# nico-bohlinger/RL-X

Measured on AMD Instinct MI355X. Metric: env-steps/sec (whole node) PPO 4096 envs at 1/2/4/8 MI355X, higher is better.
Workload: dtype f32

## Files before the change

rl-x_amd/csrc/common.h:

```cpp
#pragma once
#include <hip/hip_runtime.h>
#include <hip/hip_ext.h>
#include <stdint.h>
#include <cstring>
#include <cmath>
#include <string>
#include <vector>
#include <functional>
#include "../../include/rlx_hip.h"

namespace rlx {

void set_error(const std::string& msg);

#define RLX_HIP_TRY(expr)                                                                      \
  do {                                                                                         \
    hipError_t e_ = (expr);                                                                    \
    if (e_ != hipSuccess) {                                                                    \
      ::rlx::set_error(std::string(#expr) + " failed: " + hipGetErrorString(e_) + " (" __FILE__ \
                       ":" + std::to_string(__LINE__) + ")");                                  \
      return RLX_EHIP;                                                                         \
    }                                                                                          \
  } while (0)

#define RLX_REQUIRE(cond, code, msg)                 \
  do {                                               \
    if (!(cond)) {                                   \
      ::rlx::set_error(std::string(msg));            \
      return (code);                                 \
    }                                                \
  } while (0)

#define RLX_LAUNCH_CHECK()                           \
  RLX_HIP_TRY(hipGetLastError())

constexpr int WAVE = 64;

struct Scratch {
  void* ptr = nullptr;
  size_t bytes = 0;
};

enum ScratchSlot {
  SL_SORT_KEYS_A = 0, SL_SORT_KEYS_B, SL_SORT_VALS_B, SL_SORT_TMP, SL_PERM,
  SL_MB_X, SL_MB_XC, SL_MB_AUX, SL_STATS,
  SL_ACT_P0, SL_ACT_P1, SL_ACT_P2, SL_ACT_C0, SL_ACT_C1, SL_ACT_C2,
  SL_DACT_0, SL_DACT_1, SL_LN_P, SL_LN_C,
  SL_PARTIAL, SL_HEAD_PART, SL_NORM, SL_NORM2, SL_FWD_A, SL_FWD_B, SL_KEYS, SL_GRAD_P, SL_GRAD_C, SL_MEAN, SL_VALUE, SL_RO_NETS, SL_SAC, SL_LSTM, SL_LSTM_IDX, SL_STAGE, SL_OPT_A, SL_OPT_B, SL_STATS_ALL, SL_ZEROS, SL_STAT_PART, SL_LIDX, SL_COUNTS, SL_DIST_STATS, SL_OVERFLOW, SL_SCHED, SL_NV_ROWS, SL_WFRAG, SL_WFRAG_RO, SL_XMAX, SL_MB_GROUP_X, SL_MB_GROUP_AUX, SL_DZ0, SL_WFRAG_SAC, SL_ROW_REC,
  SL_COUNT
};

enum ProfKernel { PK_GEMM_FWD = 0, PK_GEMM_DX, PK_GEMM_DW, PK_DX_L1BWD,
                  PK_L1FWD, PK_HEAD_LOSS, PK_REDUCE,
                  PK_L12FWD,
                  PK_TAIL,
                  PK_FWD2H,
                  PK_COUNT };
constexpr int PROF_ENGINE_HBM = 2;
struct ProfRec {
  int kid, row;
  double flops, bytes;
  hipEvent_t e0, e1;
};
struct ProfRow {
  int kid, engine;
  int64_t M;
  int N, K;
  int64_t launches, timed;
  double ms, flops, bytes;
};
struct Twin { const void* p[4] = {nullptr, nullptr, nullptr, nullptr}; };

}

struct AttrOnce {
  uint64_t mask = 0;
  static int dev() { int d = 0; (void)hipGetDevice(&d); return d & 63; }
  bool done() const { return (mask >> dev()) & 1; }
  void mark() { mask |= 1ull << dev(); }
};

struct rlx_ctx {
  int device = 0;
  rlx::Scratch slots[3][rlx::SL_COUNT];
  int bank = 0;
  int opt_flip = 0;
  hipStream_t side = nullptr;
  hipEvent_t ev_fork = nullptr, ev_join = nullptr;
  hipEvent_t ev_rows[2] = {nullptr, nullptr};
  hipEvent_t ev_cdone[2] = {nullptr, nullptr};
  const float* dbg_sac_eps[2] = {nullptr, nullptr};
  bool l1fwd_mfma = true;
  bool pipeline_updates = true;
  bool pf_valid = false;
  uint32_t pf_key_in[2] = {0, 0}, pf_key_out[2] = {0, 0};
  int pf_E = 0, pf_scheme = 0;
  int64_t pf_B = 0;
  hipEvent_t pf_done = nullptr;
  hipEvent_t ev_perm_free = nullptr;
  bool perm_free_recorded = false;
  bool two_streams = true;
  const uint32_t* l1_xmax = nullptr;
  const uint32_t* xmax_slot[2] = {nullptr, nullptr};
  int lf_idle_cus = 0;
  bool dw_recompute = false;
  float* l12_stats = nullptr;
  bool l12_ran = false;
  bool dw_merge = true;
  void* dbg_stamps = nullptr;
  bool fwd2h = true;
  int gather_group_rows = 524288;
  bool gather_records = true;
  bool l12_fused = true;
  int ppo_tail = -1;
  int ppo_twin = -1;
  bool fused_recurrent_act = true;
  int num_cus = 256;
  void* defer = nullptr;
  bool prof_on = false;
  int prof_sample = 1;
  hipEvent_t prof_ref = nullptr;
  double prof_union_ms = 0.0;
  std::vector<rlx::ProfRec> prof_recs;
  std::vector<rlx::ProfRow> prof_rows;
  std::vector<hipEvent_t> prof_pool;
  bool gemm_bx = true;
  float bx_gscale = 1.f;
  bool adam_emit = true;
  bool bx_keep[3] = {false, false, false};
  struct RoImages { bool valid = false; const float* params[2] = {nullptr, nullptr}; const void* img[2][3] = {}; int nt[2][3] = {}; } ro_img;
  int bx_force_mi = 0;
  int bx_debug = 0;
  struct BxImage { const float* W; int trans, K, N; const void* img; };
  BxImage bx_img[3][32];
  int bx_n[3] = {0, 0, 0};
  bool disable_l1fused = false;
  std::vector<char> ro_nets_shadow;
  int rank = 0, world = 1;
  void* comm = nullptr;
  hipStream_t comm_stream = nullptr;
  hipEvent_t comm_ev[32] = {};
  int comm_ev_pos = 0;
  rlx_allreduce_fn ar_hook = nullptr;
  void* ar_hook_user = nullptr;
  int ro_exit = 0;
  int64_t bx_window_fallbacks = 0;
  int64_t ar_calls = 0;
  hipStream_t sac_st[2] = {nullptr, nullptr};
  hipEvent_t sac_ev[6] = {nullptr, nullptr, nullptr, nullptr, nullptr, nullptr};
  struct SacImages {
    bool valid = false; const float *pp = nullptr, *qp = nullptr, *qt = nullptr; rlx_mlp_desc pd{}, qd{}; int64_t np = 0, nq2 = 0;
    void written(const float* p, int64_t n) {
      if (!valid) return;
      auto hit = [&](const float* b, int64_t m) { return b && p < b + m && b < p + n; };
      if (hit(pp, np) || hit(qp, nq2) || hit(qt, nq2)) valid = false;
    }
  } sac_img;
  const void* sac_img_arena = nullptr;
  int sac_twin = 1;
  float* sched_host[4] = {nullptr, nullptr, nullptr, nullptr};
  hipEvent_t sched_ev[4] = {nullptr, nullptr, nullptr, nullptr};
  size_t sched_cap = 0;
  int sched_pos = 0;
  bool pf_dist = false;
  int pf_T = 0, pf_nl = 0, pf_ng = 0, pf_off = 0, pf_mb = 0;
};

namespace rlx {

struct ProfScope {
  rlx_ctx* ctx;
  hipStream_t st;
  int idx = -1;
  ProfScope(rlx_ctx* c, int kid, double flops, hipStream_t s, double bytes = 0.0, int64_t M = 0, int N = 0, int K = 0,
            int engine = 0);
  hipEvent_t ev0() const;
  hipEvent_t ev1() const;
};
#define RLX_PLAUNCH(KERNEL, GRID, BLOCK, LDS, ST, ...)                                                              \
  do {                                                                                                            \
    if (prof.idx >= 0) hipExtLaunchKernelGGL(KERNEL, GRID, BLOCK, LDS, ST, prof.ev0(), prof.ev1(), 0, __VA_ARGS__); \
    else hipLaunchKernelGGL(KERNEL, GRID, BLOCK, LDS, ST, __VA_ARGS__);                                           \
  } while (0)

inline double gemm_bytes(double M, double N, double K, int c_rw = 0) { return 4.0 * (M * K + K * N + M * N * (1 + c_rw)); }

const float* zeros_f32(rlx_ctx* ctx, size_t n);
int ctx_side_stream(rlx_ctx* ctx);
int ctx_sac_streams(rlx_ctx* ctx);
__host__ __device__ __forceinline__ float x_pow2_inv(float m) {
  union { float f; uint32_t u; } c;
  c.f = m;
  const int e = (int)((c.u >> 23) & 0xffu);
  if (e == 0 || e == 0xff) return 1.f;
  int se = 254 - e;
  se = se < 27 ? 27 : (se > 227 ? 227 : se);
  c.u = (uint32_t)se << 23;
  return c.f;
}
struct GradScaleScope {
  rlx_ctx* c;
  float prev;
  GradScaleScope(rlx_ctx* ctx, float s) : c(ctx), prev(ctx->bx_gscale) { ctx->bx_gscale = s; }
  ~GradScaleScope() { c->bx_gscale = prev; }
};
void* scratch(rlx_ctx* ctx, ScratchSlot s, size_t bytes);
int x_max_update(rlx_ctx* ctx, const float* x, int64_t n, int which, hipStream_t st, const uint32_t** out);
struct XmaxScope {
  rlx_ctx* c;
  const uint32_t* prev;
  XmaxScope(rlx_ctx* ctx, const uint32_t* p) : c(ctx), prev(ctx->l1_xmax) { ctx->l1_xmax = p; }
  ~XmaxScope() { c->l1_xmax = prev; }
};
__host__ __device__ __forceinline__ float x_scale_from_max(uint32_t mbits, float fallback) {
  const int e = (int)((mbits >> 23) & 0xffu);
  if (e == 0 || e == 0xff) return fallback;
  int se = 127 + 10 - (e - 127);
  se = se < 27 ? 27 : (se > 227 ? 227 : se);
  union { uint32_t u; float f; } c;
  c.u = (uint32_t)se << 23;
  return c.f;
}

struct LayerOff {
  int in, out;
  int64_t W, b, g, be;
};
struct MlpLayout {
  int n_hidden;
  LayerOff layer[4];
  LayerOff head;
  int64_t logstd;
  int64_t n_params;
};
inline MlpLayout make_layout(const rlx_mlp_desc& d) {
  MlpLayout L{};
  L.n_hidden = d.n_hidden;
  int64_t off = 0;
  int in = d.in_dim;
  for (int l = 0; l < d.n_hidden; ++l) {
    LayerOff& o = L.layer[l];
    o.in = in;
    o.out = d.hidden[l];
    o.W = off; off += (int64_t)in * o.out;
    o.b = off; off += o.out;
    o.g = o.be = -1;
    if (d.ln_first && l == 0) {
      o.g = off; off += o.out;
      o.be = off; off += o.out;
    }
    in = o.out;
  }
  L.head.in = in;
  L.head.out = d.out_dim;
  L.head.W = off; off += (int64_t)in * d.out_dim;
  L.head.b = off; off += d.out_dim;
  L.head.g = L.head.be = -1;
  L.logstd = -1;
  if (d.has_logstd) { L.logstd = off; off += d.out_dim; }
  L.n_params = off;
  return L;
// ... 232 lines not shown
```

rl-x_amd/csrc/core.hip:

```cpp
#include "common.h"
#include <algorithm>
#include <cstdio>
#include <cstdlib>
#include <utility>

namespace rlx {

static thread_local std::string g_last_error;

void set_error(const std::string& msg) { g_last_error = msg; }

void* scratch(rlx_ctx* ctx, ScratchSlot s, size_t bytes) {
  Scratch& sl = ctx->slots[ctx->bank][s];
  if (sl.bytes >= bytes && sl.ptr) return sl.ptr;
  if (sl.ptr) {
    if (hipDeviceSynchronize() != hipSuccess) { set_error("hipDeviceSynchronize failed in scratch()"); return nullptr; }
    (void)hipFree(sl.ptr);
    sl.ptr = nullptr;
    sl.bytes = 0;
  }
  size_t want = ((bytes > (size_t(1) << 20) ? bytes + bytes / 8 : bytes) + 255) & ~size_t(255);
  void* p = nullptr;
  hipError_t e = hipMalloc(&p, want);
  if (e != hipSuccess) {
// ... 48 lines not shown
  hipEvent_t e = nullptr;
  (void)hipEventCreate(&e);
  return e;
}

ProfScope::ProfScope(rlx_ctx* c, int kid, double flops, hipStream_t s, double bytes, int64_t M, int N, int K, int engine)
    : ctx(c), st(s) {
  if (!c || !c->prof_on) return;
  int row = -1;
  for (size_t i = 0; i < c->prof_rows.size(); ++i) {
    const ProfRow& q = c->prof_rows[i];
    if (q.kid == kid && q.engine == engine && q.M == M && q.N == N && q.K == K) { row = (int)i; break; }
  }
  if (row < 0) {
    row = (int)c->prof_rows.size();
    c->prof_rows.push_back(ProfRow{kid, engine, M, N, K, 0, 0, 0.0, 0.0, 0.0});
  }
  const int64_t seq = c->prof_rows[row].launches++;
  if (c->prof_sample > 1 && (seq % c->prof_sample) != 0) return;
  ProfRec r{kid, row, flops, bytes, prof_event(c), prof_event(c)};
  idx = (int)c->prof_recs.size();
  c->prof_recs.push_back(r);
}

__global__ __launch_bounds__(256) void k_abs_max(const float* __restrict__ x, int64_t n, uint32_t* __restrict__ out) {
  __shared__ float s_m[4];
  float m = 0.f;
  const int64_t stride = (int64_t)gridDim.x * 256 * 4;
  for (int64_t i = ((int64_t)blockIdx.x * 256 + threadIdx.x) * 4; i < n; i += stride) {
    if (i + 4 <= n && (reinterpret_cast<uintptr_t>(x + i) & 15) == 0) {
      const float4 v = *reinterpret_cast<const float4*>(x + i);
      m = fmaxf(fmaxf(m, fabsf(v.x)), fmaxf(fabsf(v.y), fmaxf(fabsf(v.z), fabsf(v.w))));
    } else {
      for (int j = 0; j < 4 && i + j < n; ++j) m = fmaxf(m, fabsf(x[i + j]));
    }
  }
  m = wave_max(m);
  if ((threadIdx.x & 63) == 0) s_m[threadIdx.x >> 6] = m;
  __syncthreads();
  if (threadIdx.x == 0) {
    m = fmaxf(fmaxf(s_m[0], s_m[1]), fmaxf(s_m[2], s_m[3]));
    if (m > 0.f) atomicMax(out, __float_as_uint(m));
  }
}

int x_max_update(rlx_ctx* ctx, const float* x, int64_t n, int which, hipStream_t st, const uint32_t** out) {
  const int bank = ctx->bank;
  ctx->bank = 0;
  uint32_t* slot = (uint32_t*)scratch(ctx, SL_XMAX, 4 * sizeof(uint32_t));
  ctx->bank = bank;
  if (!slot) return RLX_ENOMEM;
  slot += which & 3;
  RLX_HIP_TRY(hipMemsetAsync(slot, 0, sizeof(uint32_t), st));
  int grid = div_up(n, 256 * 4 * 8);
  grid = grid < 1 ? 1 : (grid > 512 ? 512 : grid);
  hipLaunchKernelGGL(k_abs_max, dim3(grid), dim3(256), 0, st, x, n, slot);
  RLX_LAUNCH_CHECK();
  *out = slot;
  return RLX_OK;
}

hipEvent_t ProfScope::ev0() const { return idx >= 0 ? ctx->prof_recs[idx].e0 : nullptr; }
hipEvent_t ProfScope::ev1() const { return idx >= 0 ? ctx->prof_recs[idx].e1 : nullptr; }

}

extern "C" {

int rlx_prof_begin(rlx_ctx* ctx) {
  RLX_REQUIRE(ctx, RLX_EINVAL, "rlx_prof_begin: ctx is NULL");
  if (!ctx->prof_ref) RLX_HIP_TRY(hipEventCreate(&ctx->prof_ref));
  RLX_HIP_TRY(hipDeviceSynchronize());
  RLX_HIP_TRY(hipEventRecord(ctx->prof_ref, 0));
  ctx->prof_rows.clear();
  ctx->prof_on = true;
  return RLX_OK;
}

int rlx_prof_kernel_count(void) { return rlx::PK_COUNT; }

const char* rlx_prof_kernel_name(int k) {
  static const char* names[rlx::PK_COUNT] = {"k_gemm_fwd", "k_gemm_dx", "k_gemm_dw", "k_dx_l1bwd",
                                              "k_l1fwd_mfma", "k_head_loss", "k_reduce_segments", "k_l12fwd", "k_tail", "k_fwd2h"};
  return (k >= 0 && k < rlx::PK_COUNT) ? names[k] : nullptr;
}

int rlx_prof_end(rlx_ctx* ctx, double* ms_out, double* flops_out, double* bytes_out, int64_t* count_out) {
  RLX_REQUIRE(ctx && ms_out && flops_out && bytes_out && count_out, RLX_EINVAL, "rlx_prof_end: NULL pointer");
  ctx->prof_on = false;
  RLX_HIP_TRY(hipDeviceSynchronize());
  for (int k = 0; k < rlx::PK_COUNT; ++k) { ms_out[k] = 0.0; flops_out[k] = 0.0; bytes_out[k] = 0.0; count_out[k] = 0; }
  std::vector<std::pair<float, float>> iv;
  iv.reserve(ctx->prof_recs.size());
  for (auto& r : ctx->prof_recs) {
    float ms = 0.f, t0 = 0.f;
    if (hipEventElapsedTime(&ms, r.e0, r.e1) == hipSuccess) {
      ms_out[r.kid] += ms;
      flops_out[r.kid] += r.flops;
      bytes_out[r.kid] += r.bytes;
      count_out[r.kid] += 1;
      rlx::ProfRow& q = ctx->prof_rows[r.row];
      q.timed += 1;
      q.ms += ms;
      q.flops += r.flops;
      q.bytes += r.bytes;
      if (q.engine != rlx::PROF_ENGINE_HBM && ctx->prof_ref && hipEventElapsedTime(&t0, ctx->prof_ref, r.e0) == hipSuccess)
        iv.emplace_back(t0, t0 + ms);
    }
    ctx->prof_pool.push_back(r.e0);
    ctx->prof_pool.push_back(r.e1);
  }
  ctx->prof_recs.clear();
  std::sort(iv.begin(), iv.end());
  double uni = 0.0;
  float cs = 0.f, ce = -1.f;
  for (auto& p : iv) {
    if (ce < 0.f || p.first > ce) { if (ce >= 0.f) uni += ce - cs; cs = p.first; ce = p.second; }
    else if (p.second > ce) ce = p.second;
  }
  if (ce >= 0.f) uni += ce - cs;
  ctx->prof_union_ms = uni;
  return RLX_OK;
}

int rlx_prof_rows(rlx_ctx* ctx, rlx_prof_row* rows, int capacity, int* n_out) {
  RLX_REQUIRE(ctx && n_out && (rows || capacity == 0), RLX_EINVAL, "rlx_prof_rows: NULL pointer");
  const int n = (int)ctx->prof_rows.size();
  *n_out = n;
  for (int i = 0; i < n && i < capacity; ++i) {
    const rlx::ProfRow& q = ctx->prof_rows[i];
    rows[i] = rlx_prof_row{q.kid, q.engine, q.N, q.K, q.M, q.launches, q.timed, q.ms, q.flops, q.bytes};
  }
  return RLX_OK;
}

int rlx_prof_union_ms(rlx_ctx* ctx, double* out) {
  RLX_REQUIRE(ctx && out, RLX_EINVAL, "rlx_prof_union_ms: NULL pointer");
  *out = ctx->prof_union_ms;
  return RLX_OK;
}

int rlx_dbg_set_option(rlx_ctx* ctx, const char* name, int value) {
  RLX_REQUIRE(ctx && name, RLX_EINVAL, "rlx_dbg_set_option: NULL");
  if (std::string(name) == "sac_twin") { ctx->sac_twin = value; return RLX_OK; }
  if (std::string(name) == "disable_l1fused") { ctx->disable_l1fused = value != 0; return RLX_OK; }
  if (std::string(name) == "l1fwd_mfma") { ctx->l1fwd_mfma = value != 0; return RLX_OK; }
  if (std::string(name) == "pipeline_updates") { ctx->pipeline_updates = value != 0; return RLX_OK; }
  if (std::string(name) == "two_streams") { ctx->two_streams = value != 0; return RLX_OK; }
  if (std::string(name) == "ppo_twin") { ctx->ppo_twin = value; return RLX_OK; }
  if (std::string(name) == "ro_exit") { ctx->ro_exit = value; return RLX_OK; }
  if (std::string(name) == "lf_idle_cus") { ctx->lf_idle_cus = value < 0 ? 0 : value; return RLX_OK; }
  if (std::string(name) == "dw_recompute") { ctx->dw_recompute = value != 0; return RLX_OK; }
  if (std::string(name) == "dw_merge") { ctx->dw_merge = value != 0; return RLX_OK; }
  if (std::string(name) == "fwd2h") { ctx->fwd2h = value != 0; return RLX_OK; }
  if (std::string(name) == "l12_fused") { ctx->l12_fused = value != 0; return RLX_OK; }
  if (std::string(name) == "gather_group_rows") { ctx->gather_group_rows = value; return RLX_OK; }
  if (std::string(name) == "gather_records") { ctx->gather_records = value != 0; return RLX_OK; }
  if (std::string(name) == "ppo_tail") { ctx->ppo_tail = value < 0 ? -1 : (value > 2 ? 2 : value); return RLX_OK; }
  if (std::string(name) == "bx_force_mi") { ctx->bx_force_mi = value; return RLX_OK; }
  if (std::string(name) == "adam_emit") { ctx->adam_emit = value != 0; return RLX_OK; }
  if (std::string(name) == "bx_debug") { ctx->bx_debug = value; return RLX_OK; }
  if (std::string(name) == "bx_gscale_log2") { ctx->bx_gscale = ldexpf(1.f, value < 0 ? 0 : (value > 40 ? 40 : value)); return RLX_OK; }
  if (std::string(name) == "gemm_bx") { ctx->gemm_bx = value != 0; return RLX_OK; }
  if (std::string(name) == "prof_sample") { ctx->prof_sample = value < 1 ? 1 : value; return RLX_OK; }
  if (std::string(name) == "fused_recurrent_act") { ctx->fused_recurrent_act = value != 0; return RLX_OK; }
  RLX_REQUIRE(false, RLX_EINVAL, "rlx_dbg_set_option: unknown option");
}

int rlx_dbg_get_counter(rlx_ctx* ctx, const char* name, int64_t* out) {
  RLX_REQUIRE(ctx && name && out, RLX_EINVAL, "rlx_dbg_get_counter: NULL");
  int bank = 0, slot = 0;
  if (sscanf(name, "scratch_ptr:%d:%d", &bank, &slot) == 2 && bank >= 0 && bank < 3 && slot >= 0 && slot < rlx::SL_COUNT) {
    *out = (int64_t)reinterpret_cast<uintptr_t>(ctx->slots[bank][slot].ptr);
    return RLX_OK;
  }
  if (sscanf(name, "scratch_bytes:%d:%d", &bank, &slot) == 2 && bank >= 0 && bank < 3 && slot >= 0 && slot < rlx::SL_COUNT) {
    *out = (int64_t)ctx->slots[bank][slot].bytes;
    return RLX_OK;
  }
  if (std::string(name) == "allreduce_calls") { *out = ctx->ar_calls; return RLX_OK; }
  if (std::string(name) == "bx_window_fallbacks") { *out = ctx->bx_window_fallbacks; return RLX_OK; }
  if (std::string(name) == "gemm_bx") { *out = ctx->gemm_bx ? 1 : 0; return RLX_OK; }
  RLX_REQUIRE(false, RLX_EINVAL, "rlx_dbg_get_counter: unknown counter");
}

int rlx_version(void) { return 200; }

const char* rlx_last_error(void) { return rlx::g_last_error.c_str(); }

int rlx_ctx_create(int device, rlx_ctx** out) {
  RLX_REQUIRE(out != nullptr, RLX_EINVAL, "rlx_ctx_create: out is NULL");
  int count = 0;
  RLX_HIP_TRY(hipGetDeviceCount(&count));
  RLX_REQUIRE(device >= 0 && device < count, RLX_EINVAL, "rlx_ctx_create: no such HIP device");
  RLX_HIP_TRY(hipSetDevice(device));
  hipDeviceProp_t prop;
  RLX_HIP_TRY(hipGetDeviceProperties(&prop, device));
  rlx_ctx* c = new rlx_ctx();
  c->device = device;
  c->num_cus = prop.multiProcessorCount;
  if (const char* e = getenv("RLX_GEMM_BX")) c->gemm_bx = atoi(e) != 0;
  if (const char* e = getenv("RLX_BX_DEBUG")) c->bx_debug = atoi(e);
  *out = c;
  return RLX_OK;
}

int rlx_dist_release(rlx_ctx* ctx);

int rlx_ctx_destroy(rlx_ctx* ctx) {
  if (!ctx) return RLX_OK;
  (void)hipSetDevice(ctx->device);
  (void)hipDeviceSynchronize();
  (void)rlx_dist_release(ctx);
  for (int i = 0; i < 2; ++i)
    if (ctx->sac_st[i]) (void)hipStreamDestroy(ctx->sac_st[i]);
  for (int i = 0; i < 6; ++i)
    if (ctx->sac_ev[i]) (void)hipEventDestroy(ctx->sac_ev[i]);
  for (int i = 0; i < 4; ++i) {
    if (ctx->sched_host[i]) (void)hipHostFree(ctx->sched_host[i]);
    if (ctx->sched_ev[i]) (void)hipEventDestroy(ctx->sched_ev[i]);
  }
  for (int b = 0; b < 3; ++b)
    for (int i = 0; i < rlx::SL_COUNT; ++i)
      if (ctx->slots[b][i].ptr) (void)hipFree(ctx->slots[b][i].ptr);
  if (ctx->ev_fork) (void)hipEventDestroy(ctx->ev_fork);
  if (ctx->ev_join) (void)hipEventDestroy(ctx->ev_join);
  for (int p = 0; p < 2; ++p) {
    if (ctx->ev_rows[p]) (void)hipEventDestroy(ctx->ev_rows[p]);
    if (ctx->ev_cdone[p]) (void)hipEventDestroy(ctx->ev_cdone[p]);
  }
  if (ctx->side) (void)hipStreamDestroy(ctx->side);
  for (auto& r : ctx->prof_recs) { (void)hipEventDestroy(r.e0); (void)hipEventDestroy(r.e1); }
  for (auto e : ctx->prof_pool) (void)hipEventDestroy(e);
  if (ctx->prof_ref) (void)hipEventDestroy(ctx->prof_ref);
  if (ctx->pf_done) (void)hipEventDestroy(ctx->pf_done);
  if (ctx->ev_perm_free) (void)hipEventDestroy(ctx->ev_perm_free);
  delete ctx;
  return RLX_OK;
}

int64_t rlx_mlp_param_count(const rlx_mlp_desc* desc) {
  if (!desc || desc->n_hidden < 1 || desc->n_hidden > 3) return -1;
  return rlx::make_layout(*desc).n_params;
}

}
```

rl-x_amd/csrc/gemm_bx.hip:

```cpp
#include "gemm_bx.h"
#ifndef RLX_WS_MIN_WAVES
#define RLX_WS_MIN_WAVES 2
#endif
#include "mlp.h"

namespace rlx {

__global__ __launch_bounds__(256) void k_bx_wfrag(BxJobs jobs) {
  int ji = 0;
#pragma unroll
  for (int q = 1; q < BX_MAX_JOBS; ++q)
    if (q < jobs.n && (int)blockIdx.x >= jobs.job[q].first_block) ji = q;
  const BxJob& jb = jobs.job[ji];
  const int idx = ((int)blockIdx.x - jb.first_block) * 256 + threadIdx.x;
  if (idx >= jb.KB * jb.NT * 64) return;
  const int lane = idx & 63, blk = idx >> 6, nt = blk % jb.NT, kb = blk / jb.NT;
  const int j = nt * 32 + (lane & 31), k0 = kb * 16 + 8 * (lane >> 5);
  float v[8];
#pragma unroll
  for (int e = 0; e < 8; ++e) {
    const int k = k0 + e;
    v[e] = (k < jb.K && j < jb.N) ? (jb.trans ? jb.W[(int64_t)j * jb.ldw + k] : jb.W[(int64_t)k * jb.ldw + j]) : 0.f;
  }
  u32x4 pl[X_NP];
#pragma unroll
  for (int e = 0; e < 4; ++e) {
    uint32_t p0, p1;
    bx_split2(v[2 * e] * X_WSCALE, v[2 * e + 1] * X_WSCALE, p0, p1);
    pl[0][e] = p0;
    pl[1][e] = p1;
  }
  u32x4* o = jb.out + ((int64_t)blk * X_NP) * 64 + lane;
  o[0] = pl[0];
  o[64] = pl[1];
}

template <int MODE, int ACT, bool APPLY, int MI, bool WS = false, bool TWIN = false>
__global__ __launch_bounds__(WS ? 2 * G_THREADS : G_THREADS, WS ? RLX_WS_MIN_WAVES : 2) void k_gemm_bx(const float* __restrict__ A, const u32x4* __restrict__ Wf,
                                                          const float* __restrict__ bias, float* __restrict__ C,
                                                          int64_t M, int N, int K, int lda, int ldc, int ntn,
                                                          const int32_t* __restrict__ m_dev, Twin tw, float sa, float so,
                                                          const float* __restrict__ Hsrc) {
  constexpr int BM = 64 * MI;
  if (TWIN && blockIdx.y) {
    A = static_cast<const float*>(tw.p[0]);
    Wf = static_cast<const u32x4*>(tw.p[1]);
    bias = static_cast<const float*>(tw.p[2]);
    C = const_cast<float*>(static_cast<const float*>(tw.p[3]));
    if (MODE == 1) Hsrc = Hsrc ? static_cast<const float*>(tw.p[2]) : nullptr;
  }
  __shared__ __attribute__((aligned(16))) char lds[2 * X_OPER];
  const int tile = xcd_remap(blockIdx.x, gridDim.x);
  const int64_t m0 = (int64_t)(tile / ntn) * BM;
  if (m_dev) {
    const int64_t mv = *m_dev;
    if (mv < M) M = mv;
    if (m0 >= M) return;
  }
  const int n0 = (tile % ntn) * G_BN;
  const int t = threadIdx.x, lane = t & 63, wv = t >> 6, wm = (wv >> 1) & 1, wn = wv & 1;
  const int a_r = (t & 255) >> 3, a_c = (t & 7) * 4;
  const int NT = ntn * 4, nt0 = (n0 >> 5) + wn * 2;
  if (WS && wv >= 4) {
    const int nkp = (K + X_BK - 1) / X_BK;
    const bool plain = m0 + BM <= M && K % X_BK == 0;
    const float* ap = A + (m0 + a_r) * lda + a_c;
    float4 ra[2 * MI];
    auto load = [&](int kt) {
      const int kk = kt * X_BK;
#pragma unroll
      for (int p = 0; p < 2 * MI; ++p)
        ra[p] = plain ? *reinterpret_cast<const float4*>(ap + (int64_t)(32 * p) * lda + kk)
                      : ld4(A, m0 + a_r + 32 * p, kk + a_c, M, K, lda);
    };
    load(0);
#pragma unroll
    for (int p = 0; p < 2 * MI; ++p) bx_stage_k4(lds, a_r + 32 * p, a_c, ra[p], sa);
    if (nkp > 1) load(1);
    __syncthreads();
    for (int kt = 0; kt < nkp; ++kt) {
      if (kt + 1 < nkp) {
        char* nxt = lds + ((kt + 1) & 1) * X_OPER;
#pragma unroll
        for (int p = 0; p < 2 * MI; ++p) bx_stage_k4(nxt, a_r + 32 * p, a_c, ra[p], sa);
        if (kt + 2 < nkp) load(kt + 2);
      }
      __syncthreads();
    }
    return;
  }
  f32x16 acc[MI][2];
#pragma unroll
  for (int i = 0; i < MI; ++i)
#pragma unroll
    for (int j = 0; j < 2; ++j)
#pragma unroll
      for (int r = 0; r < 16; ++r) acc[i][j][r] = 0.f;
  const int nk = (K + X_BK - 1) / X_BK;
  float bv[2] = {0.f, 0.f};
  if (MODE == 0) {
#pragma unroll
    for (int j = 0; j < 2; ++j) {
      const int col = n0 + acc_col(wn, j, lane);
      bv[j] = col < N ? bias[col] : 0.f;
    }
  }
  if (WS) {
    u32x4 fb0[2][X_NP], fb1[2][X_NP], fa0[MI][X_NP], fa1[MI][X_NP];
    bx_load_b(Wf, 0, NT, nt0, lane, fb0);
    __syncthreads();
    for (int kt = 0; kt < nk; ++kt) {
      const char* cur = lds + (kt & 1) * X_OPER;
      bx_load_frag<MI>(cur, wm * 32 * MI, lane, 0, fa0);
      bx_load_b(Wf, 2 * kt + 1, NT, nt0, lane, fb1);
      bx_load_frag<MI>(cur, wm * 32 * MI, lane, 1, fa1);
      bx_mma<MI>(fa0, fb0, acc);
      bx_load_b(Wf, 2 * kt + 2 < 2 * nk ? 2 * kt + 2 : 2 * nk - 1, NT, nt0, lane, fb0);
      bx_mma<MI>(fa1, fb1, acc);
      __syncthreads();
    }
  } else
  if (m0 + BM <= M && K % X_BK == 0) {
    const float* ap = A + (m0 + a_r) * lda + a_c;
    auto load = [&](int kt, float4 (&r)[2 * MI]) {
      const int kk = (kt < nk ? kt : nk - 1) * X_BK;
#pragma unroll
      for (int p = 0; p < 2 * MI; ++p) r[p] = *reinterpret_cast<const float4*>(ap + (int64_t)(32 * p) * lda + kk);
    };
    bx_kloop<MI>(lds, Wf, nk, NT, nt0, wm, lane, a_r, a_c, load, acc, sa);
  } else {
    auto load = [&](int kt, float4 (&r)[2 * MI]) {
      const int kk = (kt < nk ? kt : nk - 1) * X_BK;
#pragma unroll
      for (int p = 0; p < 2 * MI; ++p) r[p] = ld4(A, m0 + a_r + 32 * p, kk + a_c, M, K, lda);
    };
    bx_kloop<MI>(lds, Wf, nk, NT, nt0, wm, lane, a_r, a_c, load, acc, sa);
  }
  if (m0 + BM <= M && n0 + G_BN <= N) {
    float* cb = C + (m0 + wm * 32 * MI + 4 * (lane >> 5)) * ldc + n0 + wn * 64 + (lane & 31);
    if (MODE == 0) {
#pragma unroll
      for (int i = 0; i < MI; ++i)
#pragma unroll
        for (int j = 0; j < 2; ++j)
#pragma unroll
          for (int r = 0; r < 16; ++r)
            cb[(i * 32 + (r & 3) + 8 * (r >> 2)) * ldc + j * 32] = act_fwd_t<ACT>(fmaf(acc[i][j][r], so, bv[j]));
    } else if (APPLY) {
      const float* hsb = (Hsrc ? Hsrc : C) + (m0 + wm * 32 * MI + 4 * (lane >> 5)) * ldc + n0 + wn * 64 + (lane & 31);
#pragma unroll
      for (int i = 0; i < MI; ++i) {
        float h[2][16];
#pragma unroll
        for (int j = 0; j < 2; ++j)
#pragma unroll
          for (int r = 0; r < 16; ++r) h[j][r] = hsb[(i * 32 + (r & 3) + 8 * (r >> 2)) * ldc + j * 32];
#pragma unroll
        for (int j = 0; j < 2; ++j)
#pragma unroll
          for (int r = 0; r < 16; ++r)
            cb[(i * 32 + (r & 3) + 8 * (r >> 2)) * ldc + j * 32] = acc[i][j][r] * so * act_grad_t<ACT>(h[j][r]);
      }
    } else {
#pragma unroll
      for (int i = 0; i < MI; ++i)
#pragma unroll
        for (int j = 0; j < 2; ++j)
#pragma unroll
          for (int r = 0; r < 16; ++r) cb[(i * 32 + (r & 3) + 8 * (r >> 2)) * ldc + j * 32] = acc[i][j][r] * so;
    }
    return;
  }
#pragma unroll
  for (int j = 0; j < 2; ++j) {
    const int col = n0 + acc_col(wn, j, lane);
    if (col >= N) continue;
#pragma unroll
    for (int i = 0; i < MI; ++i)
#pragma unroll
      for (int r = 0; r < 16; ++r) {
        const int64_t row = m0 + wm * 32 * MI + i * 32 + (r & 3) + 8 * (r >> 2) + 4 * (lane >> 5);
        if (row < M) {
          const int64_t o = row * ldc + col;
          float v = acc[i][j][r] * so;
          if (MODE == 0) v = act_fwd_t<ACT>(v + bv[j]);
          else if (APPLY) v *= act_grad_t<ACT>((Hsrc ? Hsrc : C)[o]);
          C[o] = v;
        }
      }
  }
}

constexpr int XW_THREADS = 512;
struct DwArgs {
  const float* Hp;
  const float* dZ;
  float* partW;
  float* partB;
  const float *Hp1, *dZ1;
  float *partW1, *partB1;
  int64_t M, Mc;
  int Kd, ldh, N, ntk, ntn;
  BxDwRecompute rc;
};
template <bool TWIN, bool REC = false>
__global__ __launch_bounds__(XW_THREADS, 2) void k_gemm_dw_bx(DwArgs a, DwArgs b, int nb0, float sg, float so) {
  extern __shared__ __attribute__((aligned(16))) char lds[];
  int bid = blockIdx.x, nblk = nb0;
  if (bid >= nb0) {
    a = b;
    bid -= nb0;
    nblk = gridDim.x - nb0;
  }
  const float* __restrict__ Hp = a.Hp;
  const float* __restrict__ dZ = a.dZ;
  float* __restrict__ partW = a.partW;
  float* __restrict__ partB = a.partB;
  if (TWIN && blockIdx.y) {
    Hp = a.Hp1;
    dZ = a.dZ1;
    partW = a.partW1;
    partB = a.partB1;
  }
  const int64_t M = a.M, Mc = a.Mc;
  const int Kd = a.Kd, ldh = a.ldh, N = a.N, ntk = a.ntk, ntn = a.ntn;
  const int ntiles = ntk * ntn;
  const int lb = xcd_remap(bid, nblk);
  const int s = lb / ntiles, tile = lb % ntiles;
  const int k0d = (tile / ntn) * G_BM;
  const int n0 = (tile % ntn) * G_BN;
  const int64_t mbeg = (int64_t)s * Mc;
  int64_t mend = mbeg + Mc;
  if (mend > M) mend = M;
  const int t = threadIdx.x, lane = t & 63, wv = t >> 6;
  const int nk = (int)((mend - mbeg + X_BK - 1) / X_BK);
  const bool interior = k0d + G_BM <= Kd && n0 + G_BN <= N;
  float colsum[4] = {0.f, 0.f, 0.f, 0.f};
  const int pt = t & 255, op = pt >> 7, tt = pt & 127, cg = tt & 31, mg = tt >> 5;
  const bool rec = REC && a.rc.X != nullptr;
  if (REC && wv >= 4 && rec && op == 0) {
    const BxDwRecompute& R = a.rc;
    const int wh = wv - 4, li = lane & 31, lh = lane >> 5;
    const int O = R.O;
    const int64_t pdelta = (TWIN && blockIdx.y) ? R.pdelta1 : 0;
    const float* __restrict__ stats = (TWIN && blockIdx.y) ? R.stats1 : R.stats;
    const u32x4* __restrict__ W1x = reinterpret_cast<const u32x4*>((TWIN && blockIdx.y) ? R.W1x1 : R.W1x);
    const float xs = R.xmax ? x_scale_from_max(*R.xmax, X_ASCALE) : X_ASCALE;
    const float xinv = 1.0f / xs;
    u32x4 w1f[2][2][X_NP];
    float bias[2], gam[2], bet[2];
#pragma unroll
    for (int j = 0; j < 2; ++j) {
      const int ctg = (k0d >> 5) + 2 * wh + j;
#pragma unroll
      for (int kb = 0; kb < 2; ++kb)
#pragma unroll
        for (int p = 0; p < X_NP; ++p) w1f[kb][j][p] = W1x[((int64_t)(kb * R.NT1 + ctg) * X_NP + p) * 64 + lane];
      const int col = k0d + 32 * (2 * wh + j) + li;
      bias[j] = R.b1[pdelta + col];
      gam[j] = R.g[pdelta + col];
      bet[j] = R.be[pdelta + col];
    }
    char* xa = lds + 4 * X_OPER + wh * (X_NP * 2048 + 256);
    float* st_l = reinterpret_cast<float*>(xa + X_NP * 2048);
    for (int i = lane; i < X_NP * 2048 / 16; i += 64) reinterpret_cast<u32x4*>(xa)[i] = u32x4{0u, 0u, 0u, 0u};
    constexpr int XC = 9;
    int xr_[XC], xk_[XC];
#pragma unroll
    for (int c = 0; c < XC; ++c) {
      const int e = lane + 64 * c;
      xr_[c] = e / O;
      xk_[c] = e - xr_[c] * O;
    }
    float xv[XC], smean = 0.f, srstd = 0.f;
    auto xload = [&](int kt) {
      const int64_t m0 = mbeg + (int64_t)kt * X_BK;
      const float* xb = R.X + m0 * O;
      const int nvalid = (int)((mend - m0 < X_BK ? mend - m0 : X_BK)) * O;
#pragma unroll
      for (int c = 0; c < XC; ++c) {
        const int e = lane + 64 * c;
        xv[c] = e < nvalid ? xb[e] : 0.f;
      }
      const bool rv = lane < 32 && m0 + lane < mend;
      smean = rv ? stats[m0 + lane] : 0.f;
      srstd = rv ? stats[M + m0 + lane] : 0.f;
    };
    auto produce = [&](int buf) {
#pragma unroll
      for (int c = 0; c < XC; ++c) {
        if (lane + 64 * c < 32 * O) {
          uint32_t p0, p1;
          bx_split2(xv[c] * xs, 0.f, p0, p1);
          char* da = xa + bx_off(xr_[c], xk_[c] >> 3) + (xk_[c] & 7) * 2;
          *reinterpret_cast<uint16_t*>(da) = (uint16_t)p0;
          *reinterpret_cast<uint16_t*>(da + 2048) = (uint16_t)p1;
        }
      }
      if (lane < 32) { st_l[lane] = smean; st_l[32 + lane] = srstd; }
      f32x16 z[2];
#pragma unroll
      for (int j = 0; j < 2; ++j)
#pragma unroll
        for (int r = 0; r < 16; ++r) z[j][r] = bias[j] * (xs * X_WSCALE);
      const int nks = O > 16 ? 2 : 1;
      for (int kb = 0; kb < nks; ++kb) {
        u32x4 xf[X_NP];
#pragma unroll
        for (int p = 0; p < X_NP; ++p) xf[p] = *reinterpret_cast<const u32x4*>(xa + p * 2048 + bx_off(li, 2 * kb + lh));
#pragma unroll
        for (int j = 0; j < 2; ++j) {
          z[j] = __builtin_amdgcn_mfma_f32_32x32x16_f16(__builtin_bit_cast(f16x8, xf[0]), __builtin_bit_cast(f16x8, w1f[kb][j][1]), z[j], 0, 0, 0);
          z[j] = __builtin_amdgcn_mfma_f32_32x32x16_f16(__builtin_bit_cast(f16x8, xf[1]), __builtin_bit_cast(f16x8, w1f[kb][j][0]), z[j], 0, 0, 0);
          z[j] = __builtin_amdgcn_mfma_f32_32x32x16_f16(__builtin_bit_cast(f16x8, xf[0]), __builtin_bit_cast(f16x8, w1f[kb][j][0]), z[j], 0, 0, 0);
        }
      }
      const float zs = xinv * X_WINV;
      char* dst = lds + buf * 2 * X_OPER;
#pragma unroll
      for (int s8 = 0; s8 < 2; ++s8) {
        float4 mv[2], rv[2];
#pragma unroll
        for (int h2 = 0; h2 < 2; ++h2) {
          mv[h2] = *reinterpret_cast<const float4*>(st_l + 16 * s8 + 8 * h2 + 4 * lh);
          rv[h2] = *reinterpret_cast<const float4*>(st_l + 32 + 16 * s8 + 8 * h2 + 4 * lh);
        }
#pragma unroll
        for (int j = 0; j < 2; ++j) {
          float v[8];
#pragma unroll
          for (int e = 0; e < 8; ++e) {
            const float mean = e < 4 ? (&mv[0].x)[e & 3] : (&mv[1].x)[e & 3];
            const float rs = e < 4 ? (&rv[0].x)[e & 3] : (&rv[1].x)[e & 3];
            const float y = fmaf((z[j][8 * s8 + e] * zs - mean) * rs, gam[j], bet[j]);
            v[e] = y > 0.f ? y : __expf(fminf(y, 0.f)) - 1.0f;
          }
          bx_stage_k8<true>(dst, 32 * (2 * wh + j) + li, 2 * s8 + lh, v, X_ASCALE);
        }
      }
    };
    xload(0);
    produce(0);
    if (nk > 1) xload(1);
    __syncthreads();
    for (int kt = 0; kt < nk; ++kt) {
      if (kt + 1 < nk) {
        produce((kt + 1) & 1);
        if (kt + 2 < nk) xload(kt + 2);
      }
      __syncthreads();
    }
    if (k0d == 0 && partB) {
      const float* red = reinterpret_cast<const float*>(lds);
      __syncthreads();
      if (pt < 128 && n0 + pt < N) partB[(int64_t)s * N + n0 + pt] = (red[pt] + red[128 + pt]) + (red[256 + pt] + red[384 + pt]);
    }
    return;
  }
  if (wv >= 4) {
    const float* __restrict__ src = op ? dZ : Hp;
    const int ld = op ? N : ldh, c0 = (op ? n0 : k0d) + cg * 4, ncols = op ? N : Kd;
    const bool plain = interior && (mend - mbeg) % X_BK == 0;
    float4 rra[8];
    const int rbase = rec ? 16 * (mg >> 1) + 4 * (mg & 1) : mg * 8;
    const float* sp = src + (mbeg + rbase) * ld + c0;
// ... 303 lines not shown
  }

#define RLX_BX_LAUNCH_WS_TWIN(MODE, ACTV, APPLYV, GRID, ST, ...)                                                                          \
  if ((MODE) == 0) {                                                                                                              \
    switch (ACTV) {                                                                                                               \
      case RLX_ACT_TANH: RLX_PLAUNCH((k_gemm_bx<0, RLX_ACT_TANH, false, 2, true, true>), GRID, dim3(2 * G_THREADS), 0, ST, __VA_ARGS__); break; \
      case RLX_ACT_ELU: RLX_PLAUNCH((k_gemm_bx<0, RLX_ACT_ELU, false, 2, true, true>), GRID, dim3(2 * G_THREADS), 0, ST, __VA_ARGS__); break;   \
      case RLX_ACT_RELU: RLX_PLAUNCH((k_gemm_bx<0, RLX_ACT_RELU, false, 2, true, true>), GRID, dim3(2 * G_THREADS), 0, ST, __VA_ARGS__); break; \
      default: RLX_PLAUNCH((k_gemm_bx<0, RLX_ACT_NONE, false, 2, true, true>), GRID, dim3(2 * G_THREADS), 0, ST, __VA_ARGS__); break;           \
    }                                                                                                                             \
  } else if (!(APPLYV)) {                                                                                                         \
    RLX_PLAUNCH((k_gemm_bx<1, RLX_ACT_NONE, false, 2, true, true>), GRID, dim3(2 * G_THREADS), 0, ST, __VA_ARGS__);                     \
  } else {                                                                                                                        \
    switch (ACTV) {                                                                                                               \
      case RLX_ACT_TANH: RLX_PLAUNCH((k_gemm_bx<1, RLX_ACT_TANH, true, 2, true, true>), GRID, dim3(2 * G_THREADS), 0, ST, __VA_ARGS__); break;  \
      case RLX_ACT_ELU: RLX_PLAUNCH((k_gemm_bx<1, RLX_ACT_ELU, true, 2, true, true>), GRID, dim3(2 * G_THREADS), 0, ST, __VA_ARGS__); break;    \
      case RLX_ACT_RELU: RLX_PLAUNCH((k_gemm_bx<1, RLX_ACT_RELU, true, 2, true, true>), GRID, dim3(2 * G_THREADS), 0, ST, __VA_ARGS__); break;  \
      default: RLX_PLAUNCH((k_gemm_bx<1, RLX_ACT_NONE, false, 2, true, true>), GRID, dim3(2 * G_THREADS), 0, ST, __VA_ARGS__); break;           \
    }                                                                                                                             \
  }

#define RLX_BX_LAUNCH_MI(MIV, MODE, ACTV, APPLYV, GRID, ST, ...)                                                                   \
  if ((MODE) == 0) {                                                                                                              \
    switch (ACTV) {                                                                                                               \
      case RLX_ACT_TANH: RLX_PLAUNCH((k_gemm_bx<0, RLX_ACT_TANH, false, MIV>), GRID, dim3(G_THREADS), 0, ST, __VA_ARGS__); break; \
      case RLX_ACT_ELU: RLX_PLAUNCH((k_gemm_bx<0, RLX_ACT_ELU, false, MIV>), GRID, dim3(G_THREADS), 0, ST, __VA_ARGS__); break;   \
      case RLX_ACT_RELU: RLX_PLAUNCH((k_gemm_bx<0, RLX_ACT_RELU, false, MIV>), GRID, dim3(G_THREADS), 0, ST, __VA_ARGS__); break; \
      default: RLX_PLAUNCH((k_gemm_bx<0, RLX_ACT_NONE, false, MIV>), GRID, dim3(G_THREADS), 0, ST, __VA_ARGS__); break;           \
    }                                                                                                                             \
  } else if (!(APPLYV)) {                                                                                                         \
    RLX_PLAUNCH((k_gemm_bx<1, RLX_ACT_NONE, false, MIV>), GRID, dim3(G_THREADS), 0, ST, __VA_ARGS__);                             \
  } else {                                                                                                                        \
    switch (ACTV) {                                                                                                               \
      case RLX_ACT_TANH: RLX_PLAUNCH((k_gemm_bx<1, RLX_ACT_TANH, true, MIV>), GRID, dim3(G_THREADS), 0, ST, __VA_ARGS__); break;  \
      case RLX_ACT_ELU: RLX_PLAUNCH((k_gemm_bx<1, RLX_ACT_ELU, true, MIV>), GRID, dim3(G_THREADS), 0, ST, __VA_ARGS__); break;    \
      case RLX_ACT_RELU: RLX_PLAUNCH((k_gemm_bx<1, RLX_ACT_RELU, true, MIV>), GRID, dim3(G_THREADS), 0, ST, __VA_ARGS__); break;  \
      default: RLX_PLAUNCH((k_gemm_bx<1, RLX_ACT_NONE, false, MIV>), GRID, dim3(G_THREADS), 0, ST, __VA_ARGS__); break;           \
    }                                                                                                                             \
  }

#define RLX_BX_LAUNCH_TWIN(MODE, ACTV, APPLYV, GRID, ST, ...)                                                                       \
  if ((MODE) == 0) {                                                                                                              \
    switch (ACTV) {                                                                                                               \
      case RLX_ACT_TANH: RLX_PLAUNCH((k_gemm_bx<0, RLX_ACT_TANH, false, 1, false, true>), GRID, dim3(G_THREADS), 0, ST, __VA_ARGS__); break; \
      case RLX_ACT_ELU: RLX_PLAUNCH((k_gemm_bx<0, RLX_ACT_ELU, false, 1, false, true>), GRID, dim3(G_THREADS), 0, ST, __VA_ARGS__); break;   \
      case RLX_ACT_RELU: RLX_PLAUNCH((k_gemm_bx<0, RLX_ACT_RELU, false, 1, false, true>), GRID, dim3(G_THREADS), 0, ST, __VA_ARGS__); break; \
      default: RLX_PLAUNCH((k_gemm_bx<0, RLX_ACT_NONE, false, 1, false, true>), GRID, dim3(G_THREADS), 0, ST, __VA_ARGS__); break;           \
    }                                                                                                                             \
  } else if (!(APPLYV)) {                                                                                                         \
    RLX_PLAUNCH((k_gemm_bx<1, RLX_ACT_NONE, false, 1, false, true>), GRID, dim3(G_THREADS), 0, ST, __VA_ARGS__);                  \
  } else {                                                                                                                        \
    switch (ACTV) {                                                                                                               \
      case RLX_ACT_TANH: RLX_PLAUNCH((k_gemm_bx<1, RLX_ACT_TANH, true, 1, false, true>), GRID, dim3(G_THREADS), 0, ST, __VA_ARGS__); break;  \
      case RLX_ACT_ELU: RLX_PLAUNCH((k_gemm_bx<1, RLX_ACT_ELU, true, 1, false, true>), GRID, dim3(G_THREADS), 0, ST, __VA_ARGS__); break;    \
      case RLX_ACT_RELU: RLX_PLAUNCH((k_gemm_bx<1, RLX_ACT_RELU, true, 1, false, true>), GRID, dim3(G_THREADS), 0, ST, __VA_ARGS__); break;  \
      default: RLX_PLAUNCH((k_gemm_bx<1, RLX_ACT_NONE, false, 1, false, true>), GRID, dim3(G_THREADS), 0, ST, __VA_ARGS__); break;           \
    }                                                                                                                             \
  }

static inline int bx_row_tiles(const rlx_ctx* ctx, int64_t M, int ntn) {
  if (ctx->bx_force_mi == 1 || ctx->bx_force_mi == 2) return ctx->bx_force_mi;
  return (div_up(M, G_BM) * ntn < 2 * ctx->num_cus) ? 1 : 2;
}

bool bx_twin_usable(const rlx_ctx* ctx, int64_t M, int N) { return bx_row_tiles(ctx, M, div_up(N, G_BN)) == 1; }

int bx_launch_fwd(rlx_ctx* ctx, const float* A, const void* img, const float* bias, float* C, int64_t M, int N, int K,
                  int act, hipStream_t st, int lda, const int32_t* m_dev, const Twin* tw) {
  ProfScope prof(m_dev ? nullptr : ctx, PK_GEMM_FWD, (tw ? 4.0 : 2.0) * (double)M * N * K, st, (tw ? 2.0 : 1.0) * gemm_bytes(M, N, K), M, N, K, 1);
  const int ntn = div_up(N, G_BN);
  if (tw && bx_row_tiles(ctx, M, ntn) != 1) {
    RLX_BX_LAUNCH_WS_TWIN(0, act, 0, dim3(div_up(M, G_BM) * ntn, 2), st, A, (const u32x4*)img, bias, C, M, N, K, lda > 0 ? lda : K, N,
                          ntn, m_dev, *tw, X_ASCALE, X_AINV * X_WINV, (const float*)nullptr);
  } else if (tw) {
    RLX_BX_LAUNCH_TWIN(0, act, 0, dim3(div_up(M, 64) * ntn, 2), st, A, (const u32x4*)img, bias, C, M, N, K, lda > 0 ? lda : K, N,
                       ntn, m_dev, *tw, X_ASCALE, X_AINV * X_WINV, (const float*)nullptr);
  } else if (bx_row_tiles(ctx, M, ntn) == 1) {
    RLX_BX_LAUNCH_MI(1, 0, act, 0, dim3(div_up(M, 64) * ntn), st, A, (const u32x4*)img, bias, C, M, N, K, lda > 0 ? lda : K, N,
                     ntn, m_dev, Twin{}, X_ASCALE, X_AINV * X_WINV, (const float*)nullptr);
  } else {
    RLX_BX_LAUNCH_WS(0, act, 0, dim3(div_up(M, G_BM) * ntn), st, A, (const u32x4*)img, bias, C, M, N, K, lda > 0 ? lda : K, N,
                     ntn, m_dev, Twin{}, X_ASCALE, X_AINV * X_WINV, (const float*)nullptr);
  }
  RLX_LAUNCH_CHECK();
  return RLX_OK;
}

int bx_launch_dx(rlx_ctx* ctx, const float* dZ, const void* img, float* HD, int64_t M, int N, int Kd, int ldo, int act,
                 int apply, hipStream_t st, const Twin* tw, const float* hsrc) {
  RLX_REQUIRE(!tw || (hsrc != nullptr) == (tw->p[2] != nullptr), RLX_EINVAL, "bx_launch_dx: a twin launch is out of place for both problems or for neither");
  const float gs = ctx->bx_gscale;
  ProfScope prof(ctx, PK_GEMM_DX, (tw ? 4.0 : 2.0) * (double)M * N * Kd, st, (tw ? 2.0 : 1.0) * gemm_bytes(M, Kd, N, apply), M, Kd, N, 1);
  const int ntn = div_up(Kd, G_BN);
  if (tw && bx_row_tiles(ctx, M, ntn) != 1) {
    RLX_BX_LAUNCH_WS_TWIN(1, act, apply, dim3(div_up(M, G_BM) * ntn, 2), st, dZ, (const u32x4*)img, (const float*)nullptr, HD, M, Kd,
                          N, N, ldo, ntn, (const int32_t*)nullptr, *tw, gs, X_WINV / gs, hsrc);
  } else if (tw) {
    RLX_BX_LAUNCH_TWIN(1, act, apply, dim3(div_up(M, 64) * ntn, 2), st, dZ, (const u32x4*)img, (const float*)nullptr, HD, M, Kd,
                       N, N, ldo, ntn, (const int32_t*)nullptr, *tw, gs, X_WINV / gs, hsrc);
  } else if (bx_row_tiles(ctx, M, ntn) == 1) {
    RLX_BX_LAUNCH_MI(1, 1, act, apply, dim3(div_up(M, 64) * ntn), st, dZ, (const u32x4*)img, (const float*)nullptr, HD, M, Kd, N,
                     N, ldo, ntn, (const int32_t*)nullptr, Twin{}, gs, X_WINV / gs, hsrc);
  } else {
    RLX_BX_LAUNCH_WS(1, act, apply, dim3(div_up(M, G_BM) * ntn), st, dZ, (const u32x4*)img, (const float*)nullptr, HD, M, Kd,
                     N, N, ldo, ntn, (const int32_t*)nullptr, Twin{}, gs, X_WINV / gs, hsrc);
  }
  RLX_LAUNCH_CHECK();
  return RLX_OK;
}

bool bx_dw_usable(const rlx_ctx* ctx, int64_t M, int Kd, int ldh, int N) {
  return !(ctx->bx_debug & 64) && ctx->gemm_bx && M >= 4096 && N % 4 == 0 && ldh % 4 == 0 && ldh >= ((Kd + 3) & ~3);
}

static int dw_attr() {
  static AttrOnce attr_set;      
  if (!attr_set.done()) {
    RLX_HIP_TRY(hipFuncSetAttribute(reinterpret_cast<const void*>(k_gemm_dw_bx<false>), hipFuncAttributeMaxDynamicSharedMemorySize,
                                    4 * X_OPER + 16384));
    RLX_HIP_TRY(hipFuncSetAttribute(reinterpret_cast<const void*>(k_gemm_dw_bx<true>), hipFuncAttributeMaxDynamicSharedMemorySize,
                                    4 * X_OPER + 16384));
    RLX_HIP_TRY(hipFuncSetAttribute(reinterpret_cast<const void*>(k_gemm_dw_bx<false, true>), hipFuncAttributeMaxDynamicSharedMemorySize,
                                    4 * X_OPER + 16384));
    RLX_HIP_TRY(hipFuncSetAttribute(reinterpret_cast<const void*>(k_gemm_dw_bx<true, true>), hipFuncAttributeMaxDynamicSharedMemorySize,
                                    4 * X_OPER + 16384));
    attr_set.mark();  
  }
  return RLX_OK;
}

static DwArgs dw_args(const float* Hp, const float* dZ, float* pW, float* pB, int64_t M, int Kd, int ldh, int N, int64_t Mc, int ntk,
                      int ntn, const Twin* tw) {
  DwArgs a;
  a.Hp = Hp; a.dZ = dZ; a.partW = pW; a.partB = pB;
  a.Hp1 = tw ? static_cast<const float*>(tw->p[0]) : nullptr;
  a.dZ1 = tw ? static_cast<const float*>(tw->p[1]) : nullptr;
  a.partW1 = tw ? const_cast<float*>(static_cast<const float*>(tw->p[2])) : nullptr;
  a.partB1 = tw ? const_cast<float*>(static_cast<const float*>(tw->p[3])) : nullptr;
  a.M = M; a.Mc = Mc; a.Kd = Kd; a.ldh = ldh; a.N = N; a.ntk = ntk; a.ntn = ntn;
  a.rc = BxDwRecompute{};
  return a;
}
constexpr size_t DW_REC_LDS = 2 * (X_NP * 2048 + 256);

int bx_launch_dw(rlx_ctx* ctx, const float* Hp, const float* dZ, float* pW, float* pB, int64_t M, int Kd, int ldh, int N,
                 int64_t Mc, int S, int ntk, int ntn, hipStream_t st, const Twin* tw) {
  int rc = dw_attr();
  if (rc) return rc;
  const float gs = ctx->bx_gscale;
  ProfScope prof(ctx, PK_GEMM_DW, (tw ? 4.0 : 2.0) * (double)M * Kd * N, st, (tw ? 2.0 : 1.0) * gemm_bytes(Kd, N, M), Kd, N, (int)M, 1);
  const DwArgs a = dw_args(Hp, dZ, pW, pB, M, Kd, ldh, N, Mc, ntk, ntn, tw);
  const int nb = S * ntk * ntn;
  if (tw) {
    RLX_PLAUNCH(k_gemm_dw_bx<true>, dim3(nb, 2), dim3(XW_THREADS), 4 * X_OPER, st, a, a, nb, gs, X_AINV / gs);
  } else {
    RLX_PLAUNCH(k_gemm_dw_bx<false>, dim3(nb), dim3(XW_THREADS), 4 * X_OPER, st, a, a, nb, gs, X_AINV / gs);
  }
  RLX_LAUNCH_CHECK();
  return RLX_OK;
}

int bx_launch_dw2(rlx_ctx* ctx, const BxDwJob& j0, const BxDwJob& j1, int64_t M, hipStream_t st, const Twin* tw0, const Twin* tw1) {
  int rc = dw_attr();
  if (rc) return rc;
  RLX_REQUIRE((tw0 == nullptr) == (tw1 == nullptr), RLX_EINVAL, "bx_launch_dw2: both jobs or neither must have a twin");
  const float gs = ctx->bx_gscale;
  const double nets = tw0 ? 2.0 : 1.0;
  ProfScope prof(ctx, PK_GEMM_DW, nets * 2.0 * (double)M * ((double)j0.Kd * j0.N + (double)j1.Kd * j1.N), st,
                 nets * (gemm_bytes(j0.Kd, j0.N, M) + gemm_bytes(j1.Kd, j1.N, M)), j0.Kd + j1.Kd, j0.N + j1.N, (int)M, 1);
  DwArgs a = dw_args(j0.Hp, j0.dZ, j0.pW, j0.pB, M, j0.Kd, j0.ldh, j0.N, j0.Mc, j0.ntk, j0.ntn, tw0);
  const DwArgs b = dw_args(j1.Hp, j1.dZ, j1.pW, j1.pB, M, j1.Kd, j1.ldh, j1.N, j1.Mc, j1.ntk, j1.ntn, tw1);
  if (j0.rc) {
    RLX_REQUIRE(j0.rc->X && j0.rc->W1x && j0.rc->stats && j0.Kd == 512 && j0.rc->O <= 32 && (!tw0 || (j0.rc->W1x1 && j0.rc->stats1)),
                RLX_EINVAL, "bx_launch_dw2: incomplete recompute description");
    a.rc = *j0.rc;
  }
  const int nb0 = j0.S * j0.ntk * j0.ntn, nb1 = j1.S * j1.ntk * j1.ntn;
  const size_t lds = 4 * X_OPER + (j0.rc ? DW_REC_LDS : 0);
  if (j0.rc) {
    if (tw0) { RLX_PLAUNCH((k_gemm_dw_bx<true, true>), dim3(nb0 + nb1, 2), dim3(XW_THREADS), lds, st, a, b, nb0, gs, X_AINV / gs); }
    else { RLX_PLAUNCH((k_gemm_dw_bx<false, true>), dim3(nb0 + nb1), dim3(XW_THREADS), lds, st, a, b, nb0, gs, X_AINV / gs); }
  } else if (tw0) {
    RLX_PLAUNCH(k_gemm_dw_bx<true>, dim3(nb0 + nb1, 2), dim3(XW_THREADS), lds, st, a, b, nb0, gs, X_AINV / gs);
  } else {
    RLX_PLAUNCH(k_gemm_dw_bx<false>, dim3(nb0 + nb1), dim3(XW_THREADS), lds, st, a, b, nb0, gs, X_AINV / gs);
  }
  RLX_LAUNCH_CHECK();
  return RLX_OK;
}

}
```

rl-x_amd/csrc/mlp.h:

```cpp
#pragma once
#include "gemm.h"

namespace rlx {

constexpr int REDUCE_MAX_SEGS = 48;
constexpr int REDUCE_MAX_BLOCKS = 4096;

struct ReduceSeg {
  const float* src;
  float* dst;
  int64_t len;
  int64_t stride;
  int S;
  int nblocks;
  float scale;
  float bias;
  int in_norm;
  int vec;
};
struct ReduceTable {
  int n;
  ReduceSeg seg[REDUCE_MAX_SEGS];
};

struct TrunkOpts {
  int ldx = 0;
  bool gemm_l0 = false;
  float* dx_out = nullptr;
  int dx_c0 = 0, dx_nc = 0, dx_ld = 0;
  const float* dz_below_last = nullptr;
};

int mlp_check_desc(const rlx_mlp_desc& d);
int launch_gemm_fwd(rlx_ctx* ctx, const float* A, const float* W, const float* bias, float* C, int64_t M, int N, int K,
                    int act, hipStream_t st, int lda, const int32_t* m_dev = nullptr);
int launch_head_fwd(const float* H, const float* W, const float* b, float* out, int64_t M, int K, int A,
                    hipStream_t st, const int32_t* m_dev = nullptr, const Twin* tw = nullptr);
bool dx_cols_ok(int K, int nc);
int launch_dx_cols(const float* dZ, const float* Wblk, float* dX, int64_t M, int K, int nc, int ldo, hipStream_t st,
                   const Twin* tw = nullptr);
int64_t choose_mc(int64_t M, int tiles, int num_cus, int* S_out);
int64_t choose_mc_fit(int64_t M, int tiles, int num_cus, int* S_out);
int launch_reduce_segments(ReduceTable& tab, float* sumsq_partials, int* n_blocks_out, hipStream_t st, rlx_ctx* prof_ctx = nullptr);
int mlp_trunk_fwd(rlx_ctx* ctx, const rlx_mlp_desc& d, const MlpLayout& L, const float* params, const float* x,
                  float* const* acts, int64_t M, hipStream_t st, int ldx = 0, bool gemm_l0 = false,
                  const int32_t* m_dev = nullptr, int n_layers = -1);
int mlp_trunk_bwd(rlx_ctx* ctx, const rlx_mlp_desc& d, const MlpLayout& L, const float* params, const float* x,
                  float* const* acts, float* grads, int64_t M, const ReduceSeg* extra, int n_extra,
                  float* sumsq_partials, int* n_sumsq_blocks, hipStream_t st, const TrunkOpts* opt = nullptr);

int stage_reduce(rlx_ctx* ctx, ReduceTable& tab, float* sumsq, int* nsq, hipStream_t st);
int stage_l1_fwd2(rlx_ctx* ctx, const float* x, const float* W, const float* b, const float* g, const float* be, float* H,
                  const float* W2, const float* b2, const float* g2, const float* be2, float* H2, int64_t M, int O, int Hd,
                  int act, int ln, hipStream_t st);
int stage_l1_bwd2(rlx_ctx* ctx, const float* x, const float* W, const float* b, const float* g, const float* be, float* H,
                  const float* W2, const float* b2, const float* g2, const float* be2, float* H2, int64_t M, int O, int Hd, int act,
                  int ln, float* gW, float* gb, float* gg, float* gbe, float* gW2, float* gb2, float* gg2, float* gbe2, float* sumsq,
                  int* nsq, hipStream_t st);
struct ReduceDefer {
  ReduceTable tab;
  float* base = nullptr;
  size_t cap = 0, off = 0;
};
float* stage_alloc(rlx_ctx* ctx, size_t floats);
size_t stage_dw_floats(const rlx_ctx* ctx, int64_t M, int Kd, int N);
size_t stage_l1_bwd_floats(const rlx_ctx* ctx, int64_t M, int O, int Hd);
int stage_reduce_flush(rlx_ctx* ctx, float* sumsq, int* nsq, hipStream_t st);
int stage_dw(rlx_ctx* ctx, const float* Hp, int ldh, const float* dZ, int64_t M, int Kd, int N, float* gW, float* gB,
             float* sumsq, int* nsq, hipStream_t st);
int stage_dx(rlx_ctx* ctx, const float* dZ, const float* W, float* out, int64_t M, int N, int Kd, int ldo, int act,
             int apply_act, hipStream_t st, const float* hsrc = nullptr);
int stage_l1_fwd(rlx_ctx* ctx, const float* x, const float* W, const float* b, const float* g, const float* be, float* H,
                 int64_t M, int O, int Hd, int act, int ln, hipStream_t st);
int stage_l1_bwd(rlx_ctx* ctx, const float* x, const float* W, const float* b, const float* g, const float* be, float* H,
                 int64_t M, int O, int Hd, int act, int ln, float* gW, float* gb, float* gg, float* gbe, float* sumsq,
                 int* nsq, hipStream_t st);

bool l1fused_supported(const rlx_mlp_desc& d);
bool l1fwd_mfma_supported(const rlx_mlp_desc& d);
int launch_l1fwd_mfma(const rlx_mlp_desc& d, const MlpLayout& L, const float* params, const float* x, float* h1, int64_t M,
                      int num_cus, hipStream_t st, const int32_t* m_dev = nullptr, rlx_ctx* prof_ctx = nullptr,
                      const float* params1 = nullptr, float* h1_1 = nullptr);
struct L12Twin {
  const float* params;
  float *h1, *h2;
  const void *w1x, *w2x;
  float* stats = nullptr;
};
bool l12fwd_supported(const rlx_mlp_desc& d);
int launch_l12fwd(rlx_ctx* ctx, const rlx_mlp_desc& d, const MlpLayout& L, const float* params, const float* x, float* h1, float* h2,
                  const void* w1x, const void* w2x, int64_t M, hipStream_t st, const L12Twin* tw = nullptr, float* stats = nullptr);
struct Fwd2hTwin {
  const float* params;
  const void *w1x, *w2x;
  float *h1, *h2, *out;
};
bool fwd2h_supported(const rlx_ctx* ctx, const rlx_mlp_desc& d, const MlpLayout& L, const float* params, int64_t M, int ldx,
                     const void** w1x, const void** w2x);
int launch_fwd2h(rlx_ctx* ctx, const rlx_mlp_desc& d, const MlpLayout& L, const float* params, const void* w1x, const void* w2x,
                 const float* x, int ldx, float* h1, float* h2, float* out, int64_t M, hipStream_t st, const Fwd2hTwin* tw = nullptr);
struct Fwd3hTwin {
  const float* params;
  const void* wx[3];
  float *z1, *h1, *h2, *h3, *out;
};
bool fwd3h_supported(const rlx_ctx* ctx, const rlx_mlp_desc& d, const MlpLayout& L, const float* params, int64_t M, int ldx, const void** wx);
int launch_fwd3h(rlx_ctx* ctx, const rlx_mlp_desc& d, const MlpLayout& L, const float* params, const void* const* wx, const float* x, int ldx,
                 float* z1, float* h1, float* h2, float* h3, float* out, int64_t M, hipStream_t st, const Fwd3hTwin* tw = nullptr);
struct Dxa2hTwin {
  const float* params;
  const void* w2t;
  const float *h1, *h2, *dq;
  float* da;
};
bool dxa2h_supported(const rlx_ctx* ctx, const rlx_mlp_desc& d, int64_t M, int nc);
int launch_dxa2h(rlx_ctx* ctx, const rlx_mlp_desc& d, const MlpLayout& L, const float* params, const void* w2t, const float* h1,
                 const float* h2, const float* dq, float* da, int c0, int nc, int ld_da, int64_t M, hipStream_t st,
                 const Dxa2hTwin* tw = nullptr);
bool dw_merge_ok(const rlx_ctx* ctx, const rlx_mlp_desc& d, const MlpLayout& L, int64_t M);
size_t l1fused_partial_floats(const rlx_mlp_desc& d, int grid);
int l1fused_grid(int64_t M, int num_cus);
struct L1FusedTwin {
  const float* params;
  const float* dZ2;
  float* arena;
  float* grads;
  const void *w2x, *w1x;
  ReduceTable* tab;
};
bool l1fused_bx_images(const rlx_ctx* ctx, const MlpLayout& L, const float* params, const void** w2x, const void** w1x);
int launch_l1fused(rlx_ctx* ctx, const rlx_mlp_desc& d, const MlpLayout& L, const float* params, const float* x,
                   const float* dZ2, float* arena, int grid, float* grads, int64_t M, ReduceTable* tab, hipStream_t st,
                   const L1FusedTwin* tw = nullptr);

int bx_prepare_mlp(rlx_ctx* ctx, const rlx_mlp_desc& d, const MlpLayout& L, const float* params, bool with_bwd, hipStream_t st);
void bx_release(rlx_ctx* ctx);
struct BxNetSpec {
  const rlx_mlp_desc* d;
  const float* params;
  bool with_bwd;
  bool first_layer;
};
int bx_prepare_nets(rlx_ctx* ctx, const BxNetSpec* nets, int n_nets, hipStream_t st, ScratchSlot slot = SL_WFRAG, bool launch = true);
struct BxMat {
  const float* W;
  int K, N;
  bool fwd, trans;
};
int bx_prepare_mats(rlx_ctx* ctx, const BxMat* mats, int n, hipStream_t st);
void bx_release_all(rlx_ctx* ctx);
const void* bx_lookup(const rlx_ctx* ctx, const float* W, int trans, int K, int N);
bool bx_twin_usable(const rlx_ctx* ctx, int64_t M, int N);
int bx_launch_fwd(rlx_ctx* ctx, const float* A, const void* img, const float* bias, float* C, int64_t M, int N, int K, int act,
                  hipStream_t st, int lda, const int32_t* m_dev, const Twin* tw = nullptr);
int bx_launch_dx(rlx_ctx* ctx, const float* dZ, const void* img, float* HD, int64_t M, int N, int Kd, int ldo, int act, int apply,
                 hipStream_t st, const Twin* tw = nullptr, const float* hsrc = nullptr);
bool bx_dw_usable(const rlx_ctx* ctx, int64_t M, int Kd, int ldh, int N);
int bx_launch_dw(rlx_ctx* ctx, const float* Hp, const float* dZ, float* pW, float* pB, int64_t M, int Kd, int ldh, int N,
                 int64_t Mc, int S, int ntk, int ntn, hipStream_t st, const Twin* tw = nullptr);
struct BxDwRecompute {
  const float* X = nullptr;
  const void* W1x = nullptr;
  const float* b1 = nullptr;
  const float* g = nullptr;
  const float* be = nullptr;
  const float* stats = nullptr;
  const uint32_t* xmax = nullptr;
  const void* W1x1 = nullptr;
  const float* stats1 = nullptr;
  int64_t pdelta1 = 0;
  int O = 0, NT1 = 16;
};
struct BxDwJob {
  const float* Hp;
  const float* dZ;
  float *pW, *pB;
  int Kd, ldh, N;
  int64_t Mc;
  int S, ntk, ntn;
  const BxDwRecompute* rc = nullptr;
};
int bx_launch_dw2(rlx_ctx* ctx, const BxDwJob& j0, const BxDwJob& j1, int64_t M, hipStream_t st, const Twin* tw0 = nullptr,
                  const Twin* tw1 = nullptr);


struct BxEmitLayer {
  int64_t w_off;
  int in, out;
  void* nn;
  void* tt;
  int nt_nn, nt_tt;
};
struct BxEmit {
  int n;
  BxEmitLayer l[3];
};
BxEmit bx_emit_table(const rlx_ctx* ctx, const rlx_mlp_desc& d, const float* params);
int launch_clip_adam(float* params, const float* grads, float* m, float* v, int64_t n, const float* sumsq_partials,
                     int n_partials, int64_t step, float lr, float max_norm, float b1, float b2, float eps,
                     float* norm_out, hipStream_t st, const float* sched_dev = nullptr, const BxEmit* emit = nullptr,
                     float* polyak_target = nullptr, float tau = 0.f,
                     float weight_decay = 0.f,
                     int clip_mode = 0);
int launch_clip_adam2(float* p0, const float* g0, float* m0, float* v0, int64_t n0, const float* part0, int np0, float* norm0,
                      const BxEmit* e0, float* p1, const float* g1, float* m1, float* v1, int64_t n1, const float* part1, int np1,
                      float* norm1, const BxEmit* e1, int64_t step, float lr, float max_norm, float b1, float b2, float eps,
                      hipStream_t st, const float* sched_dev = nullptr);
int launch_sumsq_partials2(const float* g0, int64_t n0, float* part0, int* np0, const float* g1, int64_t n1, float* part1, int* np1,
                           hipStream_t st);
int clip_adam_step(rlx_ctx* ctx, float* params, const float* grads, float* m, float* v, int64_t n_params, int64_t step, float lr,
                   float max_grad_norm, float b1, float b2, float eps, float* grad_norm_out, hipStream_t st, const BxEmit* emit);
void adam_schedule_entry(float* out3, int64_t step, float lr, float b1, float b2);
int launch_sumsq_partials(const float* g, int64_t n, float* partials, hipStream_t st);

}
```

rl-x_amd/csrc/mlp.hip:

```cpp
#include "mlp.h"
#include "ln_kernels.h"

namespace rlx {

constexpr int L1_R_FWD = 4, L1_R_BWD = 2;
constexpr int L1_MAXJ = 8;
constexpr int L1_THREADS = 512;

__device__ __forceinline__ float readlane_f(float v, int lane) {
  return __int_as_float(__builtin_amdgcn_readlane(__float_as_int(v), lane));
}

struct L1Args {
  const float* X;
  float* H;
  int64_t M;
  int O, Hd, NJ;
};

template <bool BWD, int ACT, bool LN, int L1R>
__device__ __forceinline__ void l1_rows(const L1Args& a, const float* __restrict__ Ws, const float* __restrict__ bs,
                                        const float* __restrict__ gs, const float* __restrict__ bes,
                                        float (&dg)[L1_MAXJ], float (&dbe)[L1_MAXJ], int lane, int64_t wave_g,
                                        int64_t nwaves) {
  const float invH = 1.0f / (float)a.Hd;
  const int NJ = a.NJ;
  float xv[L1R], dh[L1R][L1_MAXJ];
  int64_t row0 = wave_g * L1R;
#pragma unroll
  for (int r = 0; r < L1R; ++r) {
    xv[r] = (lane < a.O && row0 + r < a.M) ? a.X[(row0 + r) * a.O + lane] : 0.f;
    if (BWD) {
#pragma unroll
      for (int j = 0; j < L1_MAXJ; ++j)
        dh[r][j] = (j < NJ && row0 + r < a.M) ? a.H[(row0 + r) * a.Hd + lane + 64 * j] : 0.f;
    }
  }
  for (; row0 < a.M; row0 += nwaves * L1R) {
    float xc[L1R], dc[L1R][L1_MAXJ];
#pragma unroll
    for (int r = 0; r < L1R; ++r) {
      xc[r] = xv[r];
      if (BWD) {
#pragma unroll
        for (int j = 0; j < L1_MAXJ; ++j) dc[r][j] = dh[r][j];
      }
    }
    const int64_t nrow0 = row0 + nwaves * L1R;
#pragma unroll
    for (int r = 0; r < L1R; ++r) {
      xv[r] = (lane < a.O && nrow0 + r < a.M) ? a.X[(nrow0 + r) * a.O + lane] : 0.f;
      if (BWD) {
#pragma unroll
        for (int j = 0; j < L1_MAXJ; ++j)
          dh[r][j] = (j < NJ && nrow0 + r < a.M) ? a.H[(nrow0 + r) * a.Hd + lane + 64 * j] : 0.f;
      }
    }
    float z[L1R][L1_MAXJ];
#pragma unroll
    for (int r = 0; r < L1R; ++r)
#pragma unroll
      for (int j = 0; j < L1_MAXJ; ++j) z[r][j] = 0.f;
    for (int k = 0; k < a.O; ++k) {
      float xs[L1R];
#pragma unroll
      for (int r = 0; r < L1R; ++r) xs[r] = readlane_f(xc[r], k);
#pragma unroll
      for (int j = 0; j < L1_MAXJ; ++j) {
        if (j < NJ) {
          const float wv = Ws[k * a.Hd + lane + 64 * j];
#pragma unroll
          for (int r = 0; r < L1R; ++r) z[r][j] = fmaf(xs[r], wv, z[r][j]);
        }
      }
    }
#pragma unroll
    for (int r = 0; r < L1R; ++r) {
      const int64_t row = row0 + r;
      if (row >= a.M) break;
      float s = 0.f, ss = 0.f;
#pragma unroll
      for (int j = 0; j < L1_MAXJ; ++j)
        if (j < NJ) {
          z[r][j] += bs[lane + 64 * j];
          s += z[r][j];
          ss += z[r][j] * z[r][j];
        }
      float mean = 0.f, rstd = 1.f;
      if (LN) {
        s = wave_sum(s);
        ss = wave_sum(ss);
        mean = s * invH;
        const float var = fmaxf(0.f, ss * invH - mean * mean);
        rstd = rsqrtf(var + 1e-6f);
      }
      if (!BWD) {
#pragma unroll
        for (int j = 0; j < L1_MAXJ; ++j)
          if (j < NJ) {
            const int c = lane + 64 * j;
            float y = z[r][j];
            if (LN) y = (y - mean) * rstd * gs[c] + bes[c];
            a.H[row * a.Hd + c] = act_fwd_t<ACT>(y);
          }
      } else {
        float m1 = 0.f, m2 = 0.f;
#pragma unroll
        for (int j = 0; j < L1_MAXJ; ++j)
          if (j < NJ) {
            const int c = lane + 64 * j;
            const float gam = LN ? gs[c] : 1.f;
            const float xh = (z[r][j] - mean) * rstd;
            const float y = LN ? xh * gam + bes[c] : z[r][j];
            const float h = act_fwd_t<ACT>(y);
            const float dy = dc[r][j] * act_grad_t<ACT>(h);
            dg[j] += dy * xh;
            dbe[j] += dy;
            const float dxh = dy * gam;
            z[r][j] = xh;
            dc[r][j] = dxh;
            m1 += dxh;
            m2 += dxh * xh;
          }
        if (LN) {
          m1 = wave_sum(m1) * invH;
          m2 = wave_sum(m2) * invH;
        }
#pragma unroll
        for (int j = 0; j < L1_MAXJ; ++j)
          if (j < NJ) a.H[row * a.Hd + lane + 64 * j] = LN ? rstd * (dc[r][j] - m1 - z[r][j] * m2) : dc[r][j];
      }
    }
  }
}

struct L1Twin { const float *W = nullptr, *b = nullptr, *g = nullptr, *be = nullptr; float *H = nullptr, *lnp = nullptr; };

template <bool BWD>
__global__ __launch_bounds__(L1_THREADS) void k_l1(const float* __restrict__ X, const float* __restrict__ W,
                                                   const float* __restrict__ b, const float* __restrict__ g,
                                                   const float* __restrict__ be, float* __restrict__ H,
                                                   float* __restrict__ ln_partials ,
                                                   int64_t M, int O, int Hd, int act, int ln,
                                                   const int32_t* __restrict__ m_dev ,
                                                   L1Twin tw = L1Twin()) {
  extern __shared__ __attribute__((aligned(16))) float smem[];
  if (m_dev && (int64_t)*m_dev < M) M = *m_dev;
  if (blockIdx.y) { W = tw.W; b = tw.b; g = tw.g; be = tw.be; H = tw.H; ln_partials = tw.lnp; }
  float* Ws = smem;
  float* bs = Ws + O * Hd;
  float* gs = bs + Hd;
  float* bes = gs + Hd;
  lds_stage<L1_THREADS>(Ws, W, O * Hd);
// ... 415 lines not shown
    red[b_r * 128 + b_c + 3] = colsum[3];
    __syncthreads();
    if (t < 128 && n0 + t < N) {
      float v = 0.f;
#pragma unroll
      for (int q = 0; q < 8; ++q) v += red[q * 128 + t];
      partB[(int64_t)s * N + n0 + t] = v;
    }
  }
}

constexpr int head_fwd_lds_floats(int rows, int K, int A) { return rows * (K + 4) + K * A; }
template <int ROWS, int NQA>
__global__ __launch_bounds__(256) void k_head_fwd(const float* __restrict__ H, const float* __restrict__ W,
                                                  const float* __restrict__ b, float* __restrict__ out, int64_t M,
                                                  int K, int A, const int32_t* __restrict__ m_dev, int w_trans, int ldo,
                                                  Twin tw) {
  extern __shared__ __attribute__((aligned(16))) float smem[];
  constexpr int NG = 256 / ROWS;
  static_assert(NQA >= 1 && NQA * NG <= 64, "at most 64 output columns");
  if (blockIdx.y) {
    H = static_cast<const float*>(tw.p[0]);
    W = static_cast<const float*>(tw.p[1]);
    b = static_cast<const float*>(tw.p[2]);
    out = const_cast<float*>(static_cast<const float*>(tw.p[3]));
  }
  const int HS = K + 4;
  float* Hs = smem;
  float* Ws = Hs + ROWS * HS;
  const int64_t r0 = (int64_t)blockIdx.x * ROWS;
  if (m_dev) {
    const int64_t mv = *m_dev;
    if (mv < M) M = mv;
    if (r0 >= M) return;
  }
  const int K4 = K >> 2, KA = K * A;
  constexpr int HB = ROWS / 16;
  constexpr int WB = 36;
  float4 hreg[HB][4];
  {
    const int c4 = threadIdx.x & 15;
#pragma unroll
    for (int q = 0; q < HB; ++q) {
      const int r = (threadIdx.x >> 4) + 16 * q;
      const float4* src = reinterpret_cast<const float4*>(H + (r0 + r) * K);
#pragma unroll
      for (int j = 0; j < 4; ++j)
        hreg[q][j] = (r0 + r < M && c4 + 16 * j < K4) ? src[c4 + 16 * j] : make_float4(0.f, 0.f, 0.f, 0.f);
    }
  }
  float wreg[WB];
#pragma unroll
  for (int j = 0; j < WB; ++j) {
    const int i = threadIdx.x + 256 * j;
    wreg[j] = i < KA ? W[i] : 0.f;
  }
  {
    const int c4 = threadIdx.x & 15;
#pragma unroll
    for (int q = 0; q < HB; ++q) {
      const int r = (threadIdx.x >> 4) + 16 * q;
#pragma unroll
      for (int j = 0; j < 4; ++j)
        if (c4 + 16 * j < K4) *reinterpret_cast<float4*>(&Hs[r * HS + 4 * (c4 + 16 * j)]) = hreg[q][j];
    }
    for (int c = c4 + 64; c < K4; c += 16) {
#pragma unroll
      for (int q = 0; q < HB; ++q) {
        const int r = (threadIdx.x >> 4) + 16 * q;
        *reinterpret_cast<float4*>(&Hs[r * HS + 4 * c]) =
            r0 + r < M ? reinterpret_cast<const float4*>(H + (r0 + r) * K)[c] : make_float4(0.f, 0.f, 0.f, 0.f);
      }
    }
  }
  for (int base = 0; base < KA; base += 256 * WB) {
    if (base) {
#pragma unroll
      for (int j = 0; j < WB; ++j) {
        const int i = base + threadIdx.x + 256 * j;
        wreg[j] = i < KA ? W[i] : 0.f;
      }
    }
#pragma unroll
    for (int j = 0; j < WB; ++j) {
      const int i = base + threadIdx.x + 256 * j;
      if (i < KA) {
        if (w_trans) {
          const int a = i / K, k = i - a * K;
          Ws[k * A + a] = wreg[j];
        } else {
          Ws[i] = wreg[j];
        }
      }
    }
  }
  __syncthreads();
  const int r = threadIdx.x % ROWS, g = threadIdx.x / ROWS;
  float acc[NQA];
  int ac[NQA];
#pragma unroll
  for (int q = 0; q < NQA; ++q) {
    acc[q] = 0.f;
    ac[q] = g + q * NG < A ? g + q * NG : A - 1;
  }
#pragma unroll 2
  for (int k = 0; k < K; k += 4) {
    const float4 h = *reinterpret_cast<const float4*>(&Hs[r * HS + k]);
    const float* wk = Ws + k * A;
#pragma unroll
    for (int q = 0; q < NQA; ++q) {
      acc[q] = fmaf(h.x, wk[ac[q]], acc[q]);
      acc[q] = fmaf(h.y, wk[A + ac[q]], acc[q]);
      acc[q] = fmaf(h.z, wk[2 * A + ac[q]], acc[q]);
      acc[q] = fmaf(h.w, wk[3 * A + ac[q]], acc[q]);
    }
  }
  if (r0 + r < M) {
#pragma unroll
    for (int q = 0; q < NQA; ++q) {
      const int a = g + q * NG;
      if (a < A) out[(r0 + r) * ldo + a] = acc[q] + (b ? b[a] : 0.f);
    }
  }
}

constexpr size_t HEAD_FWD_MAX_LDS = 128 * 1024;
static void head_fwd16_allow_large_lds() {
  static AttrOnce done;
  if (done.done()) return;
  (void)hipFuncSetAttribute(reinterpret_cast<const void*>(k_head_fwd<16, 1>), hipFuncAttributeMaxDynamicSharedMemorySize, (int)HEAD_FWD_MAX_LDS);
  (void)hipFuncSetAttribute(reinterpret_cast<const void*>(k_head_fwd<16, 2>), hipFuncAttributeMaxDynamicSharedMemorySize, (int)HEAD_FWD_MAX_LDS);
  (void)hipFuncSetAttribute(reinterpret_cast<const void*>(k_head_fwd<16, 3>), hipFuncAttributeMaxDynamicSharedMemorySize, (int)HEAD_FWD_MAX_LDS);
  (void)hipFuncSetAttribute(reinterpret_cast<const void*>(k_head_fwd<16, 4>), hipFuncAttributeMaxDynamicSharedMemorySize, (int)HEAD_FWD_MAX_LDS);
  done.mark();
}
#define RLX_HEAD_FWD_16(A_, GRID, LDS, ST, ...)                                                                   \
  if ((LDS) > 64 * 1024) head_fwd16_allow_large_lds();                                                            \
  switch (div_up((A_), 16)) {                                                                                     \
    case 1: hipLaunchKernelGGL((k_head_fwd<16, 1>), GRID, dim3(256), LDS, ST, __VA_ARGS__); break;                \
    case 2: hipLaunchKernelGGL((k_head_fwd<16, 2>), GRID, dim3(256), LDS, ST, __VA_ARGS__); break;                \
    case 3: hipLaunchKernelGGL((k_head_fwd<16, 3>), GRID, dim3(256), LDS, ST, __VA_ARGS__); break;                \
    default: hipLaunchKernelGGL((k_head_fwd<16, 4>), GRID, dim3(256), LDS, ST, __VA_ARGS__); break;               \
  }
#define RLX_HEAD_FWD_64(A_, GRID, LDS, ST, ...)                                                                   \
  do {                                                                                                            \
    const int nq_ = div_up((A_), 4);                                                                              \
    if (nq_ <= 2) hipLaunchKernelGGL((k_head_fwd<64, 2>), GRID, dim3(256), LDS, ST, __VA_ARGS__);                 \
    else if (nq_ <= 4) hipLaunchKernelGGL((k_head_fwd<64, 4>), GRID, dim3(256), LDS, ST, __VA_ARGS__);            \
    else if (nq_ <= 8) hipLaunchKernelGGL((k_head_fwd<64, 8>), GRID, dim3(256), LDS, ST, __VA_ARGS__);            \
    else hipLaunchKernelGGL((k_head_fwd<64, 16>), GRID, dim3(256), LDS, ST, __VA_ARGS__);                         \
  } while (0)

__global__ __launch_bounds__(256) void k_reduce_segments(ReduceTable tab, float* __restrict__ sumsq_partials) {
  __shared__ float4 s_acc[4][64];
  __shared__ float s_buf[4];
  int seg = 0;
  int blk = blockIdx.x;
  while (seg < tab.n - 1 && blk >= tab.seg[seg].nblocks) {
    blk -= tab.seg[seg].nblocks;
    ++seg;
  }
  const ReduceSeg sg = tab.seg[seg];
  float sq = 0.f;
  if (sg.vec == 2) {
    const int x = threadIdx.x & 15, y = threadIdx.x >> 4;
    const int64_t i = (int64_t)blk * 64 + 4 * x;
    float4 a = make_float4(0.f, 0.f, 0.f, 0.f);
    if (i < sg.len) {
      const float* p = sg.src + i;
      int sidx = y;
      for (; sidx + 240 < sg.S; sidx += 256) {
        float4 v[16];
#pragma unroll
        for (int q = 0; q < 16; ++q) v[q] = *reinterpret_cast<const float4*>(p + (int64_t)(sidx + 16 * q) * sg.stride);
#pragma unroll
        for (int q = 0; q < 16; q += 4) {
          a.x += (v[q].x + v[q + 1].x) + (v[q + 2].x + v[q + 3].x);
          a.y += (v[q].y + v[q + 1].y) + (v[q + 2].y + v[q + 3].y);
          a.z += (v[q].z + v[q + 1].z) + (v[q + 2].z + v[q + 3].z);
          a.w += (v[q].w + v[q + 1].w) + (v[q + 2].w + v[q + 3].w);
        }
      }
      for (; sidx < sg.S; sidx += 64) {
        float4 r[4];
#pragma unroll
        for (int q = 0; q < 4; ++q) {
          const int si = sidx + 16 * q;
          r[q] = *reinterpret_cast<const float4*>(p + (int64_t)(si < sg.S ? si : sg.S - 1) * sg.stride);
        }
#pragma unroll
        for (int q = 0; q < 4; ++q)
          if (sidx + 16 * q < sg.S) { a.x += r[q].x; a.y += r[q].y; a.z += r[q].z; a.w += r[q].w; }
      }
    }
    float4* sred4 = &s_acc[0][0];
    sred4[y * 16 + x] = a;
    __syncthreads();
    if (y == 0 && i < sg.len) {
      float4 v = a;
#pragma unroll
      for (int q = 1; q < 16; ++q) {
        const float4 b = sred4[q * 16 + x];
        v.x += b.x; v.y += b.y; v.z += b.z; v.w += b.w;
      }
      v.x = v.x * sg.scale + sg.bias;
      v.y = v.y * sg.scale + sg.bias;
      v.z = v.z * sg.scale + sg.bias;
      v.w = v.w * sg.scale + sg.bias;
      sg.dst[i] = v.x; sg.dst[i + 1] = v.y; sg.dst[i + 2] = v.z; sg.dst[i + 3] = v.w;
      if (sg.in_norm) sq = v.x * v.x + v.y * v.y + v.z * v.z + v.w * v.w;
    }
  } else if (sg.vec) {
    const int x = threadIdx.x & 63, y = threadIdx.x >> 6;
    const int64_t i = (int64_t)blk * 256 + 4 * x;
    float4 a = make_float4(0.f, 0.f, 0.f, 0.f);
    if (i < sg.len) {
      const float* p = sg.src + i;
      int sidx = y;
      for (; sidx + 60 < sg.S; sidx += 64) {
        float4 v[16];
#pragma unroll
        for (int q = 0; q < 16; ++q) v[q] = *reinterpret_cast<const float4*>(p + (int64_t)(sidx + 4 * q) * sg.stride);
#pragma unroll
        for (int q = 0; q < 16; q += 4) {
          a.x += (v[q].x + v[q + 1].x) + (v[q + 2].x + v[q + 3].x);
          a.y += (v[q].y + v[q + 1].y) + (v[q + 2].y + v[q + 3].y);
          a.z += (v[q].z + v[q + 1].z) + (v[q + 2].z + v[q + 3].z);
          a.w += (v[q].w + v[q + 1].w) + (v[q + 2].w + v[q + 3].w);
        }
      }
      for (; sidx + 12 < sg.S; sidx += 16) {
        const float4 v0 = *reinterpret_cast<const float4*>(p + (int64_t)sidx * sg.stride);
        const float4 v1 = *reinterpret_cast<const float4*>(p + (int64_t)(sidx + 4) * sg.stride);
        const float4 v2 = *reinterpret_cast<const float4*>(p + (int64_t)(sidx + 8) * sg.stride);
        const float4 v3 = *reinterpret_cast<const float4*>(p + (int64_t)(sidx + 12) * sg.stride);
        a.x += (v0.x + v1.x) + (v2.x + v3.x);
        a.y += (v0.y + v1.y) + (v2.y + v3.y);
        a.z += (v0.z + v1.z) + (v2.z + v3.z);
        a.w += (v0.w + v1.w) + (v2.w + v3.w);
      }
      {
        float4 r[3];
#pragma unroll
        for (int q = 0; q < 3; ++q) {
          const int si = sidx + 4 * q;
          r[q] = *reinterpret_cast<const float4*>(p + (int64_t)(si < sg.S ? si : sg.S - 1) * sg.stride);
        }
#pragma unroll
        for (int q = 0; q < 3; ++q) {
          if (sidx + 4 * q < sg.S) { a.x += r[q].x; a.y += r[q].y; a.z += r[q].z; a.w += r[q].w; }
        }
      }
    }
    s_acc[y][x] = a;
    __syncthreads();
    if (y == 0 && i < sg.len) {
      const float4 b1 = s_acc[1][x], b2 = s_acc[2][x], b3 = s_acc[3][x];
      float4 v;
      v.x = ((a.x + b1.x) + (b2.x + b3.x)) * sg.scale + sg.bias;
      v.y = ((a.y + b1.y) + (b2.y + b3.y)) * sg.scale + sg.bias;
      v.z = ((a.z + b1.z) + (b2.z + b3.z)) * sg.scale + sg.bias;
      v.w = ((a.w + b1.w) + (b2.w + b3.w)) * sg.scale + sg.bias;
      sg.dst[i] = v.x; sg.dst[i + 1] = v.y; sg.dst[i + 2] = v.z; sg.dst[i + 3] = v.w;
      if (sg.in_norm) sq = v.x * v.x + v.y * v.y + v.z * v.z + v.w * v.w;
    }
  } else {
    const int x = threadIdx.x & 15, y = threadIdx.x >> 4;
    const int64_t i = (int64_t)blk * 16 + x;
    float a = 0.f;
    if (i < sg.len) {
      const float* p = sg.src + i;
      int sidx = y;
      for (; sidx + 48 < sg.S; sidx += 64) {
        const float v0 = p[(int64_t)sidx * sg.stride], v1 = p[(int64_t)(sidx + 16) * sg.stride];
        const float v2 = p[(int64_t)(sidx + 32) * sg.stride], v3 = p[(int64_t)(sidx + 48) * sg.stride];
        a += (v0 + v1) + (v2 + v3);
      }
      for (; sidx < sg.S; sidx += 16) a += p[(int64_t)sidx * sg.stride];
    }
    float* sred = reinterpret_cast<float*>(&s_acc[0][0]);
    sred[y * 16 + x] = a;
    __syncthreads();
    if (y == 0 && i < sg.len) {
      float v = 0.f;
#pragma unroll
      for (int q = 0; q < 16; ++q) v += sred[q * 16 + x];
      v = v * sg.scale + sg.bias;
      sg.dst[i] = v;
      if (sg.in_norm) sq = v * v;
    }
  }
  sq = wave_sum(sq);
  if ((threadIdx.x & 63) == 0) s_buf[threadIdx.x >> 6] = sq;
  __syncthreads();
  if (threadIdx.x == 0 && sumsq_partials) sumsq_partials[blockIdx.x] = s_buf[0] + s_buf[1] + s_buf[2] + s_buf[3];
}

static int check_desc(const rlx_mlp_desc& d) {
  RLX_REQUIRE(d.n_hidden >= 1 && d.n_hidden <= 3, RLX_EUNSUP, "mlp: n_hidden must be 1..3");
  RLX_REQUIRE(d.in_dim >= 1 && d.in_dim <= 8192, RLX_EUNSUP, "mlp: in_dim must be 1..8192");
  RLX_REQUIRE(d.in_dim <= 32 || !d.ln_first || d.n_hidden >= 2, RLX_EUNSUP,
              "mlp: LayerNorm after a wide first layer needs at least two hidden layers");
  RLX_REQUIRE(d.hidden[0] % 64 == 0 && d.hidden[0] >= 64 && d.hidden[0] <= 512, RLX_EUNSUP,
              "mlp: hidden[0] must be a multiple of 64 in [64, 512]");
  for (int l = 1; l < d.n_hidden; ++l)
    RLX_REQUIRE(d.hidden[l] % 4 == 0 && d.hidden[l] >= 4, RLX_EUNSUP, "mlp: hidden dims must be multiples of 4");
  RLX_REQUIRE(d.out_dim >= 1 && d.out_dim <= 64, RLX_EUNSUP, "mlp: out_dim must be 1..64");
  RLX_REQUIRE(d.act >= 0 && d.act <= 2, RLX_EINVAL, "mlp: unknown activation");
  return RLX_OK;
}

int mlp_check_desc(const rlx_mlp_desc& d) { return check_desc(d); }

int launch_l1_fwd(const rlx_mlp_desc& d, const MlpLayout& L, const float* params, const float* x, float* h1,
                  int64_t M, int num_cus, hipStream_t st, bool allow_mfma, const int32_t* m_dev = nullptr, rlx_ctx* prof_ctx = nullptr) {
  if (allow_mfma && M >= 1024 && l1fwd_mfma_supported(d)) return launch_l1fwd_mfma(d, L, params, x, h1, M, num_cus, st, m_dev, prof_ctx);
  const LayerOff& o = L.layer[0];
  const int grid = l1_grid(M, num_cus);
  return launch_l1<false>(x, params + o.W, params + o.b, o.g >= 0 ? params + o.g : nullptr,
                          o.be >= 0 ? params + o.be : nullptr, h1, nullptr, M, o.in, o.out, d.act,
                          d.ln_first ? 1 : 0, grid, st, m_dev);
}

int launch_gemm_fwd(rlx_ctx* ctx, const float* A, const float* W, const float* bias, float* C, int64_t M, int N, int K,
                    int act, hipStream_t st, int lda, const int32_t* m_dev) {
  if (const void* img = bx_lookup(ctx, W, 0, K, N)) return bx_launch_fwd(ctx, A, img, bias, C, M, N, K, act, st, lda, m_dev);
  ProfScope prof(m_dev ? nullptr : ctx, PK_GEMM_FWD, 2.0 * (double)M * N * K, st, gemm_bytes(M, N, K), M, N, K);
  const int ntn = div_up(N, G_BN);
  const int grid = div_up(M, G_BM) * ntn;
  RLX_GEMM_FWD_LAUNCH(act, dim3(grid), st, A, W, bias, C, M, N, K, lda > 0 ? lda : K, ntn, m_dev);
  RLX_LAUNCH_CHECK();
  return RLX_OK;
}


__global__ __launch_bounds__(256) void k_head_fwd_narrow(const float* __restrict__ H, const float* __restrict__ W,
                                                         const float* __restrict__ b, float* __restrict__ out, int64_t M,
                                                         int K, int A, const int32_t* __restrict__ m_dev, Twin tw) {
  if (blockIdx.y) {
    H = static_cast<const float*>(tw.p[0]);
    W = static_cast<const float*>(tw.p[1]);
    b = static_cast<const float*>(tw.p[2]);
    out = const_cast<float*>(static_cast<const float*>(tw.p[3]));
  }
  if (m_dev) {
    const int64_t mv = *m_dev;
    if (mv < M) M = mv;
  }
  const int lane = threadIdx.x & 63, wv = threadIdx.x >> 6;
  const int64_t nw = (int64_t)gridDim.x * 4;
  for (int64_t row = (int64_t)blockIdx.x * 4 + wv; row < M; row += nw) {
    float acc[4] = {0.f, 0.f, 0.f, 0.f};
    for (int k = lane; k < K; k += 64) {
      const float h = H[row * K + k];
#pragma unroll
      for (int a = 0; a < 4; ++a)
        if (a < A) acc[a] = fmaf(h, W[k * A + a], acc[a]);
    }
#pragma unroll
    for (int a = 0; a < 4; ++a)
      if (a < A) {
        const float v = wave_sum(acc[a]);
        if (lane == 0) out[row * A + a] = v + b[a];
      }
  }
}

int launch_head_fwd(const float* H, const float* W, const float* b, float* out, int64_t M, int K, int A,
                    hipStream_t st, const int32_t* m_dev, const Twin* tw) {
  const unsigned gy = tw ? 2 : 1;
  const Twin t2 = tw ? *tw : Twin{};
  static AttrOnce lds_opt_in;
  if (!lds_opt_in.done()) {
#define RLX_HEAD_ATTR(R, Q)                                                                                                     \
  RLX_HIP_TRY(hipFuncSetAttribute(reinterpret_cast<const void*>(k_head_fwd<R, Q>), hipFuncAttributeMaxDynamicSharedMemorySize, 160 * 1024))
    RLX_HEAD_ATTR(16, 1); RLX_HEAD_ATTR(16, 2); RLX_HEAD_ATTR(16, 3); RLX_HEAD_ATTR(16, 4);
    RLX_HEAD_ATTR(64, 2); RLX_HEAD_ATTR(64, 4); RLX_HEAD_ATTR(64, 8); RLX_HEAD_ATTR(64, 16);
#undef RLX_HEAD_ATTR
    lds_opt_in.mark();
  }
  if (A <= 4) {
    int grid = div_up(M, 4);
    if (grid > 4096) grid = 4096;
    hipLaunchKernelGGL(k_head_fwd_narrow, dim3(grid, gy), dim3(256), 0, st, H, W, b, out, M, K, A, m_dev, t2);
  } else if (M < 65536) {
    const size_t lds = (size_t)head_fwd_lds_floats(16, K, A) * sizeof(float);
    RLX_REQUIRE(K % 4 == 0 && A <= 64 && lds <= 160 * 1024, RLX_EUNSUP, "head forward: K % 4 == 0, A <= 64, tile within the LDS");
    RLX_HEAD_FWD_16(A, dim3(div_up(M, 16), gy), lds, st, H, W, b, out, M, K, A, m_dev, 0, A, t2);
  } else {
    const size_t lds = (size_t)head_fwd_lds_floats(64, K, A) * sizeof(float);
    RLX_REQUIRE(K % 4 == 0 && A <= 64 && lds <= 160 * 1024, RLX_EUNSUP, "head forward: K % 4 == 0, A <= 64, tile within the LDS");
    RLX_HEAD_FWD_64(A, dim3(div_up(M, 64), gy), lds, st, H, W, b, out, M, K, A, m_dev, 0, A, t2);
  }
  RLX_LAUNCH_CHECK();
  return RLX_OK;
}

bool dx_cols_ok(int K, int nc) {
  return nc >= 1 && nc <= 64 && K % 4 == 0 && (size_t)head_fwd_lds_floats(16, K, nc) * sizeof(float) <= HEAD_FWD_MAX_LDS;
}

int launch_dx_cols(const float* dZ, const float* Wblk, float* dX, int64_t M, int K, int nc, int ldo, hipStream_t st,
                   const Twin* tw) {
  const size_t lds = (size_t)head_fwd_lds_floats(16, K, nc) * sizeof(float);
  RLX_REQUIRE(nc <= 64 && K % 4 == 0 && lds <= HEAD_FWD_MAX_LDS, RLX_EUNSUP, "launch_dx_cols: at most 64 columns, tile within 128 KB of LDS");
  RLX_HEAD_FWD_16(nc, dim3(div_up(M, 16), tw ? 2 : 1), lds, st, dZ, Wblk, (const float*)nullptr, dX, M, K, nc,
                  (const int32_t*)nullptr, 1, ldo, tw ? *tw : Twin{});
  RLX_LAUNCH_CHECK();
  return RLX_OK;
}

int mlp_trunk_fwd(rlx_ctx* ctx, const rlx_mlp_desc& d, const MlpLayout& L, const float* params, const float* x,
                  float* const* acts, int64_t M, hipStream_t st, int ldx, bool gemm_l0, const int32_t* m_dev, int n_layers) {
  int rc;
  const int nl = (n_layers >= 1 && n_layers <= d.n_hidden) ? n_layers : d.n_hidden;
  int l_next = 1;
  if (ctx->l12_fused && d.in_dim <= 32 && !gemm_l0 && !m_dev && nl >= 2 && M >= 4096 && (ldx <= 0 || ldx == d.in_dim) &&
      l12fwd_supported(d)) {
    const LayerOff &o0 = L.layer[0], &o1 = L.layer[1];
    const void* w1x = bx_lookup(ctx, params + o0.W, 0, o0.in, o0.out);
    const void* w2x = w1x ? bx_lookup(ctx, params + o1.W, 0, o1.in, o1.out) : nullptr;
    if (w1x && w2x) {
      rc = launch_l12fwd(ctx, d, L, params, x, acts[0], acts[1], w1x, w2x, M, st, nullptr, ctx->l12_stats);
      if (rc) return rc;
      l_next = 2;
      ctx->l12_ran = ctx->l12_stats != nullptr;
    }
  }
  if (l_next == 2) {
  } else if (d.in_dim <= 32 && !gemm_l0) {
    RLX_REQUIRE(ldx <= 0 || ldx == d.in_dim, RLX_EUNSUP, "mlp: padded input rows need in_dim > 32");
    rc = launch_l1_fwd(d, L, params, x, acts[0], M, ctx->num_cus, st, ctx->l1fwd_mfma, m_dev, ctx);
  } else {
    const LayerOff& o = L.layer[0];
    const int ld = ldx > 0 ? ldx : d.in_dim;
    RLX_REQUIRE(ld % 4 == 0 && ld >= d.in_dim, RLX_EUNSUP, "mlp: wide inputs need a row stride that is a multiple of 4");
    if (d.ln_first) {
      RLX_REQUIRE(acts[3] != nullptr && d.n_hidden >= 2, RLX_EUNSUP, "mlp: wide LayerNorm layer without its pre-activation buffer");
      rc = launch_gemm_fwd(ctx, x, params + o.W, params + o.b, acts[3], M, o.out, o.in, RLX_ACT_NONE, st, ld, m_dev);
      if (rc) return rc;
      int grid = div_up(M, 4);
      if (grid > ctx->num_cus * 8) grid = ctx->num_cus * 8;
      hipLaunchKernelGGL(k_ln_act<false>, dim3(grid), dim3(256), 0, st, acts[3], acts[0], params + o.g, params + o.be,
                         (float*)nullptr, M, o.out, d.act);
      RLX_LAUNCH_CHECK();
      rc = RLX_OK;
    } else {
      rc = launch_gemm_fwd(ctx, x, params + o.W, params + o.b, acts[0], M, o.out, o.in, d.act, st, ld, m_dev);
    }
  }
  if (rc) return rc;
  for (int l = l_next; l < nl; ++l) {
    const LayerOff& o = L.layer[l];
    rc = launch_gemm_fwd(ctx, acts[l - 1], params + o.W, params + o.b, acts[l], M, o.out, o.in, d.act, st, 0, m_dev);
    if (rc) return rc;
  }
  return RLX_OK;
}

int64_t choose_mc(int64_t M, int tiles, int num_cus, int* S_out) {
  int S = (num_cus + tiles - 1) / tiles;
  if (S < 1) S = 1;
  int64_t Mc = (M + S - 1) / S;
  Mc = ((Mc + G_BK - 1) / G_BK) * G_BK;
  if (Mc < G_BK) Mc = G_BK;
  S = (int)((M + Mc - 1) / Mc);
  if (S < 1) S = 1;
  *S_out = S;
  return Mc;
}

bool dw_merge_ok(const rlx_ctx* ctx, const rlx_mlp_desc& d, const MlpLayout& L, int64_t M) {
  return ctx->dw_merge && d.n_hidden == 3 && bx_dw_usable(ctx, M, L.layer[2].in, L.layer[2].in, L.layer[2].out) &&
         bx_dw_usable(ctx, M, L.layer[1].in, L.layer[1].in, L.layer[1].out);
}

int64_t choose_mc_fit(int64_t M, int tiles, int num_cus, int* S_out) {
  int S = num_cus / tiles;
  if (S < 1) S = 1;
  int64_t Mc = (M + S - 1) / S;
  Mc = ((Mc + G_BK - 1) / G_BK) * G_BK;
  if (Mc < G_BK) Mc = G_BK;
  S = (int)((M + Mc - 1) / Mc);
  *S_out = S < 1 ? 1 : S;
  return Mc;
}

int mlp_trunk_bwd(rlx_ctx* ctx, const rlx_mlp_desc& d, const MlpLayout& L, const float* params, const float* x,
                  float* const* acts, float* grads, int64_t M, const ReduceSeg* extra, int n_extra,
                  float* sumsq_partials, int* n_sumsq_blocks, hipStream_t st, const TrunkOpts* opt) {
  ReduceTable tab;
  tab.n = 0;
  const bool wide = d.in_dim > 32 || (opt && opt->gemm_l0);
  const bool wide_ln = wide && d.ln_first;
  RLX_REQUIRE(!wide_ln || (d.n_hidden >= 2 && acts[3] != nullptr), RLX_EUNSUP,
              "mlp: wide LayerNorm layer needs two hidden layers and its pre-activation buffer");
  const bool pgrads = grads != nullptr;
  const int ldx = (opt && opt->ldx > 0) ? opt->ldx : d.in_dim;
  size_t need = 0;
  int S_l[4];
  int64_t Mc_l[4];
  for (int l = d.n_hidden - 1; l >= 0; --l) {
    const LayerOff& o = L.layer[l];
    const int tiles = (l == 0 && !wide) ? div_up(o.out, G_BN) : div_up(o.in, G_BM) * div_up(o.out, G_BN);
    Mc_l[l] = choose_mc(M, tiles, ctx->num_cus, &S_l[l]);
  }
  const bool dw_merge = pgrads && opt && opt->dz_below_last && dw_merge_ok(ctx, d, L, M);
  RLX_REQUIRE(dw_merge || !ctx->l12_ran, RLX_EUNSUP, "mlp bwd: the first-layer activations were not stored but cannot be recomputed here");
  if (dw_merge) {
    const int tiles = div_up(L.layer[2].in, G_BM) * div_up(L.layer[2].out, G_BN) + div_up(L.layer[1].in, G_BM) * div_up(L.layer[1].out, G_BN);
    Mc_l[2] = Mc_l[1] = choose_mc_fit(M, tiles, ctx->num_cus, &S_l[2]);
    S_l[1] = S_l[2];
  }
  for (int l = d.n_hidden - 1; l >= 0; --l) need += (size_t)S_l[l] * ((size_t)L.layer[l].in * L.layer[l].out + L.layer[l].out);
  const LayerOff& o0 = L.layer[0];
  const int l1_grid = rlx::l1_grid(M, ctx->num_cus);
  int ln_grid = div_up(M, 16);
  if (ln_grid > ctx->num_cus * 4) ln_grid = ctx->num_cus * 4;
  if (d.ln_first) need += (size_t)(wide_ln ? ln_grid : l1_grid) * 2 * o0.out;
  const bool fuse_l1 = pgrads && !wide && l1fused_supported(d) && !ctx->disable_l1fused;
  const int lf_grid = l1fused_grid(M, ctx->num_cus - ctx->lf_idle_cus > 8 ? ctx->num_cus - ctx->lf_idle_cus : 8);
  if (fuse_l1) need += l1fused_partial_floats(d, lf_grid);
  float* arena = (float*)scratch(ctx, SL_PARTIAL, need * sizeof(float));
  if (!arena) return RLX_ENOMEM;
  float* cur = arena;
  const float* dz[4] = {acts[0], acts[1], acts[2], acts[3]};
  const int pre = d.n_hidden - 2;
  const bool dz_ready = opt && opt->dz_below_last && pre >= 1;
  if (dz_ready) dz[pre] = opt->dz_below_last;

  const bool merge2 = pgrads && ctx->dw_merge && d.n_hidden == 2 && wide && !d.ln_first && !dz_ready && !fuse_l1 &&
                      bx_lookup(ctx, params + L.layer[1].W, 1, L.layer[1].out, L.layer[1].in) != nullptr &&
                      bx_dw_usable(ctx, M, L.layer[1].in, L.layer[1].in, L.layer[1].out) && bx_dw_usable(ctx, M, o0.in, ldx, o0.out);
  if (merge2) {
    const LayerOff& o1 = L.layer[1];
    float* dz0 = (float*)scratch(ctx, SL_DZ0, (size_t)M * o0.out * sizeof(float));
    if (!dz0) return RLX_ENOMEM;
    int rcm = bx_launch_dx(ctx, acts[1], bx_lookup(ctx, params + o1.W, 1, o1.out, o1.in), dz0, M, o1.out, o1.in, o1.in, d.act, 1, st,
                           nullptr, acts[0]);
    if (rcm) return rcm;
    const int tiles = div_up(o1.in, G_BM) * div_up(o1.out, G_BN) + div_up(o0.in, G_BM) * div_up(o0.out, G_BN);
    int Sm = 0;
    const int64_t Mcm = choose_mc_fit(M, tiles, ctx->num_cus, &Sm);
    RLX_REQUIRE(Sm <= S_l[0] && Sm <= S_l[1], RLX_EUNSUP, "mlp bwd: merged weight-gradient slabs exceed the arena");
    float* pW1 = cur; cur += (size_t)S_l[1] * o1.in * o1.out;
    float* pB1 = cur; cur += (size_t)S_l[1] * o1.out;
    float* pW0 = cur; cur += (size_t)S_l[0] * o0.in * o0.out;
    float* pB0 = cur; cur += (size_t)S_l[0] * o0.out;
    const BxDwJob j0{x, dz0, pW0, pB0, o0.in, ldx, o0.out, Mcm, Sm, div_up(o0.in, G_BM), div_up(o0.out, G_BN)};
    const BxDwJob j1{acts[0], acts[1], pW1, pB1, o1.in, o1.in, o1.out, Mcm, Sm, div_up(o1.in, G_BM), div_up(o1.out, G_BN)};
    rcm = bx_launch_dw2(ctx, j0, j1, M, st);
    if (rcm) return rcm;
    tab.seg[tab.n++] = ReduceSeg{pW1, grads + o1.W, (int64_t)o1.in * o1.out, (int64_t)o1.in * o1.out, Sm, 0, 1.f, 0.f, 1};
    tab.seg[tab.n++] = ReduceSeg{pB1, grads + o1.b, (int64_t)o1.out, (int64_t)o1.out, Sm, 0, 1.f, 0.f, 1};
    tab.seg[tab.n++] = ReduceSeg{pW0, grads + o0.W, (int64_t)o0.in * o0.out, (int64_t)o0.in * o0.out, Sm, 0, 1.f, 0.f, 1};
    tab.seg[tab.n++] = ReduceSeg{pB0, grads + o0.b, (int64_t)o0.out, (int64_t)o0.out, Sm, 0, 1.f, 0.f, 1};
    if (opt && opt->dx_out) RLX_REQUIRE(false, RLX_EUNSUP, "mlp bwd: input-gradient columns with parameter gradients");
    for (int e = 0; e < n_extra; ++e) tab.seg[tab.n++] = extra[e];
    return launch_reduce_segments(tab, sumsq_partials, n_sumsq_blocks, st, ctx);
  }
  BxDwJob dw_job3{};
  bool l1_done = false;
  if (dw_merge && fuse_l1 && dz_ready) {
    float* lf_arena = arena + need - l1fused_partial_floats(d, lf_grid);
    const int rcf = launch_l1fused(ctx, d, L, params, x, dz[1], lf_arena, lf_grid, grads, M, &tab, st);
    if (rcf) return rcf;
    l1_done = true;
  }
  for (int l = d.n_hidden - 1; l >= 1; --l) {
    const LayerOff& o = L.layer[l];
    float* pW = cur; cur += (size_t)S_l[l] * o.in * o.out;
    float* pB = cur; cur += (size_t)S_l[l] * o.out;
    const int ntk = div_up(o.in, G_BM), ntn = div_up(o.out, G_BN);
    if (dw_merge) {
      BxDwJob job{acts[l - 1], dz[l], pW, pB, o.in, o.in, o.out, Mc_l[l], S_l[l], ntk, ntn};
      if (l == 2) dw_job3 = job;
      else {
        BxDwRecompute rcd;
        if (ctx->l12_ran) {
          rcd.X = x; rcd.W1x = bx_lookup(ctx, params + o0.W, 0, o0.in, o0.out); rcd.b1 = params + o0.b; rcd.g = params + o0.g;
          rcd.be = params + o0.be; rcd.stats = ctx->l12_stats; rcd.xmax = ctx->l1_xmax; rcd.O = o0.in; rcd.NT1 = o0.out / 32;
          job.rc = &rcd;
        }
        const int rcw = bx_launch_dw2(ctx, job, dw_job3, M, st);
        if (rcw) return rcw;
      }
      tab.seg[tab.n++] = ReduceSeg{pW, grads + o.W, (int64_t)o.in * o.out, (int64_t)o.in * o.out, S_l[l], 0, 1.f, 0.f, 1};
      tab.seg[tab.n++] = ReduceSeg{pB, grads + o.b, (int64_t)o.out, (int64_t)o.out, S_l[l], 0, 1.f, 0.f, 1};
    } else if (pgrads) {
      hipStream_t sw = st;
      if (bx_dw_usable(ctx, M, o.in, o.in, o.out)) {
        const int rcw = bx_launch_dw(ctx, acts[l - 1], dz[l], pW, pB, M, o.in, o.in, o.out, Mc_l[l], S_l[l], ntk, ntn, sw);
        if (rcw) return rcw;
      } else {
        ProfScope prof(ctx, PK_GEMM_DW, 2.0 * (double)M * o.in * o.out, sw, gemm_bytes(o.in, o.out, M), o.in, o.out, (int)M);
        RLX_PLAUNCH(k_gemm_dw, dim3(S_l[l] * ntk * ntn), dim3(G_THREADS), 0, sw, (const float*)acts[l - 1], dz[l], pW, pB, M,
                           o.in, o.in, o.out, Mc_l[l], ntk, ntn);
      }
      RLX_LAUNCH_CHECK();
      tab.seg[tab.n++] = ReduceSeg{pW, grads + o.W, (int64_t)o.in * o.out, (int64_t)o.in * o.out, S_l[l], 0, 1.f, 0.f, 1};
      tab.seg[tab.n++] = ReduceSeg{pB, grads + o.b, (int64_t)o.out, (int64_t)o.out, S_l[l], 0, 1.f, 0.f, 1};
    }
    if (l == 1 && fuse_l1) continue;
    if (dz_ready && l == d.n_hidden - 1) continue;
    const int ntn2 = div_up(o.in, G_BN);
    const int apply = (l - 1 == 0 && (!wide || wide_ln)) ? 0 : 1;
    if (const void* img = bx_lookup(ctx, params + o.W, 1, o.out, o.in)) {
      const int rcx = bx_launch_dx(ctx, dz[l], img, acts[l - 1], M, o.out, o.in, o.in, d.act, apply, st);
      if (rcx) return rcx;
    } else {
      ProfScope prof(ctx, PK_GEMM_DX, 2.0 * (double)M * o.in * o.out, st, gemm_bytes(M, o.in, o.out, apply), M, o.in, o.out);
      RLX_GEMM_DX_LAUNCH(d.act, apply, dim3(div_up(M, G_BM) * ntn2), st, dz[l], params + o.W, acts[l - 1], M, o.out, o.in,
                         o.in, ntn2, (const float*)nullptr);
      RLX_LAUNCH_CHECK();
    }
  }
  if (fuse_l1 && !l1_done) {
    float* lf_arena = cur; cur += l1fused_partial_floats(d, lf_grid);
    const int rcf = launch_l1fused(ctx, d, L, params, x, dz[1], lf_arena, lf_grid, grads, M, &tab, st);
    if (rcf) return rcf;
  }
  if (wide_ln) {
    float* pLNw = cur; cur += (size_t)ln_grid * 2 * o0.out;
    hipLaunchKernelGGL(k_ln_act<true>, dim3(ln_grid), dim3(256), (size_t)8 * o0.out * sizeof(float), st, acts[3], acts[0],
                       params + o0.g, params + o0.be, pLNw, M, o0.out, d.act);
    RLX_LAUNCH_CHECK();
    if (pgrads) {
      tab.seg[tab.n++] = ReduceSeg{pLNw, grads + o0.g, (int64_t)o0.out, (int64_t)2 * o0.out, ln_grid, 0, 1.f, 0.f, 1};
      tab.seg[tab.n++] = ReduceSeg{pLNw + o0.out, grads + o0.be, (int64_t)o0.out, (int64_t)2 * o0.out, ln_grid, 0, 1.f, 0.f, 1};
    }
  }
  if (wide) {
    if (pgrads) {
      float* pW = cur; cur += (size_t)S_l[0] * o0.in * o0.out;
      float* pB = cur; cur += (size_t)S_l[0] * o0.out;
      const int ntk = div_up(o0.in, G_BM), ntn = div_up(o0.out, G_BN);
      if (bx_dw_usable(ctx, M, o0.in, ldx, o0.out)) {
        const int rcw = bx_launch_dw(ctx, x, acts[0], pW, pB, M, o0.in, ldx, o0.out, Mc_l[0], S_l[0], ntk, ntn, st);
        if (rcw) return rcw;
      } else {
        ProfScope prof(ctx, PK_GEMM_DW, 2.0 * (double)M * o0.in * o0.out, st, gemm_bytes(o0.in, o0.out, M), o0.in, o0.out, (int)M);
        RLX_PLAUNCH(k_gemm_dw, dim3(S_l[0] * ntk * ntn), dim3(G_THREADS), 0, st, x, acts[0], pW, pB, M, o0.in, ldx,
                           o0.out, Mc_l[0], ntk, ntn);
      }
      RLX_LAUNCH_CHECK();
      tab.seg[tab.n++] = ReduceSeg{pW, grads + o0.W, (int64_t)o0.in * o0.out, (int64_t)o0.in * o0.out, S_l[0], 0, 1.f, 0.f, 1};
      tab.seg[tab.n++] = ReduceSeg{pB, grads + o0.b, (int64_t)o0.out, (int64_t)o0.out, S_l[0], 0, 1.f, 0.f, 1};
    }
    if (opt && opt->dx_out) {
      RLX_REQUIRE(opt->dx_nc > 0 && opt->dx_c0 >= 0 && opt->dx_c0 + opt->dx_nc <= o0.in && opt->dx_ld >= opt->dx_nc,
                  RLX_EINVAL, "mlp bwd: bad input-gradient column range");
      if (opt->dx_nc <= 64 && (size_t)head_fwd_lds_floats(16, o0.out, opt->dx_nc) * sizeof(float) <= HEAD_FWD_MAX_LDS) {
        const size_t lds = (size_t)head_fwd_lds_floats(16, o0.out, opt->dx_nc) * sizeof(float);
        RLX_HEAD_FWD_16(opt->dx_nc, dim3(div_up(M, 16)), lds, st, (const float*)acts[0],
                        params + o0.W + (int64_t)opt->dx_c0 * o0.out, (const float*)nullptr, opt->dx_out, M, o0.out,
                        opt->dx_nc, (const int32_t*)nullptr, 1, opt->dx_ld, Twin{});
        RLX_LAUNCH_CHECK();
      } else {
      const int ntn2 = div_up(opt->dx_nc, G_BN);
      ProfScope prof(ctx, PK_GEMM_DX, 2.0 * (double)M * opt->dx_nc * o0.out, st, gemm_bytes(M, opt->dx_nc, o0.out), M, opt->dx_nc, o0.out);
      RLX_GEMM_DX_LAUNCH(d.act, 0, dim3(div_up(M, G_BM) * ntn2), st, acts[0],
                         params + o0.W + (int64_t)opt->dx_c0 * o0.out, opt->dx_out, M, o0.out, opt->dx_nc, opt->dx_ld, ntn2,
                         (const float*)nullptr);
      RLX_LAUNCH_CHECK();
      }
    }
  }
  float* pLN = nullptr;
  if (!fuse_l1 && !wide) {
    RLX_REQUIRE(pgrads, RLX_EUNSUP, "mlp bwd: input-gradient-only mode needs in_dim > 32");
    if (d.ln_first) { pLN = cur; cur += (size_t)l1_grid * 2 * o0.out; }
    int rc1 = launch_l1<true>(x, params + o0.W, params + o0.b, o0.g >= 0 ? params + o0.g : nullptr,
                              o0.be >= 0 ? params + o0.be : nullptr, acts[0], pLN, M, o0.in, o0.out, d.act,
                              d.ln_first ? 1 : 0, l1_grid, st);
    if (rc1) return rc1;
    if (d.ln_first) {
      tab.seg[tab.n++] = ReduceSeg{pLN, grads + o0.g, (int64_t)o0.out, (int64_t)2 * o0.out, l1_grid, 0, 1.f, 0.f, 1};
      tab.seg[tab.n++] = ReduceSeg{pLN + o0.out, grads + o0.be, (int64_t)o0.out, (int64_t)2 * o0.out, l1_grid, 0, 1.f, 0.f, 1};
    }
    float* pW = cur; cur += (size_t)S_l[0] * o0.in * o0.out;
    float* pB = cur; cur += (size_t)S_l[0] * o0.out;
    const int ntn = div_up(o0.out, G_BN);
    RLX_REQUIRE(o0.in <= 32, RLX_EUNSUP, "mlp bwd: in_dim > 32 not supported by the skinny dW1 kernel yet");
    hipLaunchKernelGGL(k_gemm_dw_skinny, dim3(S_l[0] * ntn), dim3(G_THREADS), 0, st, x, acts[0], pW, pB, M, o0.in,
                       o0.out, Mc_l[0], ntn);
    RLX_LAUNCH_CHECK();
    tab.seg[tab.n++] = ReduceSeg{pW, grads + o0.W, (int64_t)o0.in * o0.out, (int64_t)o0.in * o0.out, S_l[0], 0, 1.f, 0.f, 1};
    tab.seg[tab.n++] = ReduceSeg{pB, grads + o0.b, (int64_t)o0.out, (int64_t)o0.out, S_l[0], 0, 1.f, 0.f, 1};
  }
  if (!pgrads) {
    if (n_sumsq_blocks) *n_sumsq_blocks = 0;
    return RLX_OK;
  }
  for (int e = 0; e < n_extra; ++e) tab.seg[tab.n++] = extra[e];
  return launch_reduce_segments(tab, sumsq_partials, n_sumsq_blocks, st, ctx);
}

int launch_reduce_segments(ReduceTable& tab, float* sumsq_partials, int* n_blocks_out, hipStream_t st, rlx_ctx* prof_ctx) {
  int total_blocks = 0;
  double bytes = 0.0;
  int64_t outputs = 0;
  for (int i = 0; i < tab.n; ++i) {
    bytes += 4.0 * (double)tab.seg[i].len * (tab.seg[i].S + 1);
    outputs += tab.seg[i].len;
  }
  ProfScope prof(prof_ctx, PK_REDUCE, 0.0, st, bytes, outputs, tab.n, 0, PROF_ENGINE_HBM);
  for (int i = 0; i < tab.n; ++i) {
    ReduceSeg& g = tab.seg[i];
    g.vec = (g.len % 4 == 0 && g.stride % 4 == 0 && (reinterpret_cast<uintptr_t>(g.src) & 15) == 0 && g.len >= 256)
                ? 1 : 0;
    if (g.vec && g.S >= 128) g.vec = 2;
    g.nblocks = g.vec == 2 ? div_up(g.len, 64) : (g.vec ? div_up(g.len, 256) : div_up(g.len, 16));
    total_blocks += g.nblocks;
  }
  RLX_REQUIRE(total_blocks <= REDUCE_MAX_BLOCKS, RLX_EUNSUP, "mlp bwd: too many reduction blocks");
  RLX_PLAUNCH(k_reduce_segments, dim3(total_blocks), dim3(256), 0, st, tab, sumsq_partials);
  RLX_LAUNCH_CHECK();
  if (n_blocks_out) *n_blocks_out = total_blocks;
  return RLX_OK;
}

static inline size_t align64(size_t n) { return (n + 63) & ~size_t(63); }

float* stage_alloc(rlx_ctx* ctx, size_t floats) {
  ReduceDefer* D = static_cast<ReduceDefer*>(ctx->defer);
  if (!D) return (float*)scratch(ctx, SL_STAGE, floats * sizeof(float));
  if (D->off + align64(floats) > D->cap) {
    set_error("stage_alloc: the deferred-reduction arena is too small (stage_*_floats out of step with the stages)");
    return nullptr;
  }
  float* p = D->base + D->off;
  D->off += align64(floats);
  return p;
}

size_t stage_dw_floats(const rlx_ctx* ctx, int64_t M, int Kd, int N) {
  int S = 1;
  (void)choose_mc(M, div_up(Kd, G_BM) * div_up(N, G_BN), ctx->num_cus, &S);
  return align64((size_t)S * Kd * N + (size_t)S * N);
}

size_t stage_l1_bwd_floats(const rlx_ctx* ctx, int64_t M, int O, int Hd) {
  int S = 1;
  (void)choose_mc(M, div_up(Hd, G_BN), ctx->num_cus, &S);
  return align64((size_t)l1_grid(M, ctx->num_cus) * 2 * Hd + (size_t)S * (O + 1) * Hd);
}

static int reduce_launch(rlx_ctx* ctx, ReduceTable& tab, float* sumsq, int* nsq, hipStream_t st);

int stage_reduce_flush(rlx_ctx* ctx, float* sumsq, int* nsq, hipStream_t st) {
  ReduceDefer* D = static_cast<ReduceDefer*>(ctx->defer);
  ctx->defer = nullptr;
  if (!D || D->tab.n == 0) return RLX_OK;
  return reduce_launch(ctx, D->tab, sumsq, nsq, st);
}

static int reduce_now(rlx_ctx* ctx, ReduceTable& tab, float* sumsq, int* nsq, hipStream_t st) {
  if (ReduceDefer* D = static_cast<ReduceDefer*>(ctx->defer)) {
    RLX_REQUIRE(D->tab.n + tab.n <= REDUCE_MAX_SEGS, RLX_EUNSUP, "deferred reduction: too many segments");
    for (int i = 0; i < tab.n; ++i) D->tab.seg[D->tab.n++] = tab.seg[i];
    return RLX_OK;
  }
  return reduce_launch(ctx, tab, sumsq, nsq, st);
}

static int reduce_launch(rlx_ctx* ctx, ReduceTable& tab, float* sumsq, int* nsq, hipStream_t st) {
  int total = 0;
  for (int i = 0; i < tab.n; ++i) {
    ReduceSeg& g = tab.seg[i];
    g.vec = (g.len % 4 == 0 && g.stride % 4 == 0 && (reinterpret_cast<uintptr_t>(g.src) & 15) == 0 && g.len >= 256) ? 1 : 0;
    if (g.vec && g.S >= 128) g.vec = 2;
    g.nblocks = g.vec == 2 ? div_up(g.len, 64) : (g.vec ? div_up(g.len, 256) : div_up(g.len, 16));
    total += g.nblocks;
  }
  RLX_REQUIRE(!nsq || *nsq + total <= REDUCE_MAX_BLOCKS, RLX_EUNSUP, "stage reduce: norm partial array exhausted");
  hipLaunchKernelGGL(k_reduce_segments, dim3(total), dim3(256), 0, st, tab, sumsq ? sumsq + (nsq ? *nsq : 0) : nullptr);
  RLX_LAUNCH_CHECK();
  if (nsq) *nsq += total;
  return RLX_OK;
}

int stage_reduce(rlx_ctx* ctx, ReduceTable& tab, float* sumsq, int* nsq, hipStream_t st) {
  return reduce_now(ctx, tab, sumsq, nsq, st);
}

int stage_dw(rlx_ctx* ctx, const float* Hp, int ldh, const float* dZ, int64_t M, int Kd, int N, float* gW, float* gB,
             float* sumsq, int* nsq, hipStream_t st) {
  const int ntk = div_up(Kd, G_BM), ntn = div_up(N, G_BN);
  int S = 1;
  const int64_t Mc = choose_mc(M, ntk * ntn, ctx->num_cus, &S);
  float* pW = stage_alloc(ctx, (size_t)S * Kd * N + (size_t)S * N);
  if (!pW) return RLX_ENOMEM;
  float* pB = pW + (size_t)S * Kd * N;
  if (bx_dw_usable(ctx, M, Kd, ldh, N)) {
    const int rcw = bx_launch_dw(ctx, Hp, dZ, pW, pB, M, Kd, ldh, N, Mc, S, ntk, ntn, st);
    if (rcw) return rcw;
  } else {
    ProfScope prof(ctx, PK_GEMM_DW, 2.0 * (double)M * Kd * N, st, gemm_bytes(Kd, N, M), Kd, N, (int)M);
    RLX_PLAUNCH(k_gemm_dw, dim3(S * ntk * ntn), dim3(G_THREADS), 0, st, Hp, dZ, pW, pB, M, Kd, ldh, N, Mc, ntk, ntn);
  }
  RLX_LAUNCH_CHECK();
  ReduceTable tab;
  tab.n = 0;
  tab.seg[tab.n++] = ReduceSeg{pW, gW, (int64_t)Kd * N, (int64_t)Kd * N, S, 0, 1.f, 0.f, 1};
  if (gB) tab.seg[tab.n++] = ReduceSeg{pB, gB, (int64_t)N, (int64_t)N, S, 0, 1.f, 0.f, 1};
  return reduce_now(ctx, tab, sumsq, nsq, st);
}

int stage_dx(rlx_ctx* ctx, const float* dZ, const float* W, float* out, int64_t M, int N, int Kd, int ldo, int act,
             int apply_act, hipStream_t st, const float* hsrc) {
  if (const void* img = bx_lookup(ctx, W, 1, N, Kd)) return bx_launch_dx(ctx, dZ, img, out, M, N, Kd, ldo, act, apply_act, st, nullptr, hsrc);
  const int ntn = div_up(Kd, G_BN);
  ProfScope prof(ctx, PK_GEMM_DX, 2.0 * (double)M * N * Kd, st, gemm_bytes(M, Kd, N, apply_act), M, Kd, N);
  RLX_GEMM_DX_LAUNCH(act, apply_act, dim3(div_up(M, G_BM) * ntn), st, dZ, W, out, M, N, Kd, ldo, ntn, hsrc);
  RLX_LAUNCH_CHECK();
  return RLX_OK;
}

int stage_l1_fwd(rlx_ctx* ctx, const float* x, const float* W, const float* b, const float* g, const float* be, float* H,
                 int64_t M, int O, int Hd, int act, int ln, hipStream_t st) {
  return launch_l1<false>(x, W, b, g, be, H, nullptr, M, O, Hd, act, ln, l1_grid(M, ctx->num_cus), st);
}

int stage_l1_fwd2(rlx_ctx* ctx, const float* x, const float* W, const float* b, const float* g, const float* be, float* H,
                  const float* W2, const float* b2, const float* g2, const float* be2, float* H2, int64_t M, int O, int Hd,
                  int act, int ln, hipStream_t st) {
  L1Twin tw;
  tw.W = W2; tw.b = b2; tw.g = g2; tw.be = be2; tw.H = H2;
  return launch_l1<false>(x, W, b, g, be, H, nullptr, M, O, Hd, act, ln, l1_grid(M, ctx->num_cus), st, nullptr, &tw);
}

int stage_l1_bwd(rlx_ctx* ctx, const float* x, const float* W, const float* b, const float* g, const float* be, float* H,
                 int64_t M, int O, int Hd, int act, int ln, float* gW, float* gb, float* gg, float* gbe, float* sumsq,
                 int* nsq, hipStream_t st) {
  RLX_REQUIRE(O <= 32, RLX_EUNSUP, "stage_l1_bwd: in_dim must be <= 32");
  const int grid = l1_grid(M, ctx->num_cus);
  const int ntn = div_up(Hd, G_BN);
  int S = 1;
  const int64_t Mc = choose_mc(M, ntn, ctx->num_cus, &S);
  float* arena = stage_alloc(ctx, (size_t)grid * 2 * Hd + (size_t)S * (O + 1) * Hd);
  if (!arena) return RLX_ENOMEM;
  float* pLN = arena;
  float* pW = arena + (size_t)grid * 2 * Hd;
  float* pB = pW + (size_t)S * O * Hd;
  int rc = launch_l1<true>(x, W, b, g, be, H, ln ? pLN : nullptr, M, O, Hd, act, ln, grid, st);
  if (rc) return rc;
  hipLaunchKernelGGL(k_gemm_dw_skinny, dim3(S * ntn), dim3(G_THREADS), 0, st, x, H, pW, pB, M, O, Hd, Mc, ntn);
  RLX_LAUNCH_CHECK();
  ReduceTable tab;
  tab.n = 0;
  tab.seg[tab.n++] = ReduceSeg{pW, gW, (int64_t)O * Hd, (int64_t)O * Hd, S, 0, 1.f, 0.f, 1};
  tab.seg[tab.n++] = ReduceSeg{pB, gb, (int64_t)Hd, (int64_t)Hd, S, 0, 1.f, 0.f, 1};
  if (ln) {
    tab.seg[tab.n++] = ReduceSeg{pLN, gg, (int64_t)Hd, (int64_t)2 * Hd, grid, 0, 1.f, 0.f, 1};
    tab.seg[tab.n++] = ReduceSeg{pLN + Hd, gbe, (int64_t)Hd, (int64_t)2 * Hd, grid, 0, 1.f, 0.f, 1};
  }
  return reduce_now(ctx, tab, sumsq, nsq, st);
}

int stage_l1_bwd2(rlx_ctx* ctx, const float* x, const float* W, const float* b, const float* g, const float* be, float* H,
                  const float* W2, const float* b2, const float* g2, const float* be2, float* H2, int64_t M, int O, int Hd, int act,
                  int ln, float* gW, float* gb, float* gg, float* gbe, float* gW2, float* gb2, float* gg2, float* gbe2, float* sumsq,
                  int* nsq, hipStream_t st) {
  RLX_REQUIRE(O <= 32, RLX_EUNSUP, "stage_l1_bwd2: in_dim must be <= 32");
  const int grid = l1_grid(M, ctx->num_cus);
  const int ntn = div_up(Hd, G_BN);
  int S = 1;
  const int64_t Mc = choose_mc(M, ntn, ctx->num_cus, &S);
  float* arena[2];
  for (int k = 0; k < 2; ++k) {
    arena[k] = stage_alloc(ctx, (size_t)grid * 2 * Hd + (size_t)S * (O + 1) * Hd);
    if (!arena[k]) return RLX_ENOMEM;
  }
  RLX_REQUIRE(ctx->defer || arena[0] != arena[1], RLX_EUNSUP, "stage_l1_bwd2 needs the deferred-reduction arena (two live partial sets)");
  L1Twin tw;
  tw.W = W2; tw.b = b2; tw.g = g2; tw.be = be2; tw.H = H2; tw.lnp = ln ? arena[1] : nullptr;
  int rc = launch_l1<true>(x, W, b, g, be, H, ln ? arena[0] : nullptr, M, O, Hd, act, ln, grid, st, nullptr, &tw);
  if (rc) return rc;
  ReduceTable tab;
  tab.n = 0;
  float* Hs[2] = {H, H2};
  float* gWs[2] = {gW, gW2};
  float* gbs[2] = {gb, gb2};
  float* ggs[2] = {gg, gg2};
  float* gbes[2] = {gbe, gbe2};
  for (int k = 0; k < 2; ++k) {
    float* pLN = arena[k];
    float* pW = arena[k] + (size_t)grid * 2 * Hd;
    float* pB = pW + (size_t)S * O * Hd;
    hipLaunchKernelGGL(k_gemm_dw_skinny, dim3(S * ntn), dim3(G_THREADS), 0, st, x, Hs[k], pW, pB, M, O, Hd, Mc, ntn);
    RLX_LAUNCH_CHECK();
    tab.seg[tab.n++] = ReduceSeg{pW, gWs[k], (int64_t)O * Hd, (int64_t)O * Hd, S, 0, 1.f, 0.f, 1};
    tab.seg[tab.n++] = ReduceSeg{pB, gbs[k], (int64_t)Hd, (int64_t)Hd, S, 0, 1.f, 0.f, 1};
    if (ln) {
      tab.seg[tab.n++] = ReduceSeg{pLN, ggs[k], (int64_t)Hd, (int64_t)2 * Hd, grid, 0, 1.f, 0.f, 1};
      tab.seg[tab.n++] = ReduceSeg{pLN + Hd, gbes[k], (int64_t)Hd, (int64_t)2 * Hd, grid, 0, 1.f, 0.f, 1};
    }
  }
  return reduce_now(ctx, tab, sumsq, nsq, st);
}

}

using namespace rlx;

extern "C" int rlx_dbg_gemm_f32(rlx_ctx* ctx, int mode, const float* A, const float* B, float* C, float* aux,
                                int64_t M, int N, int K, int act, void* stream) {
  RLX_REQUIRE(ctx && A && B && C && M > 0 && N > 0 && K > 0, RLX_EINVAL, "rlx_dbg_gemm_f32: bad args");
  RLX_REQUIRE(N % 4 == 0 && K % 4 == 0, RLX_EUNSUP, "rlx_dbg_gemm_f32: N and K must be multiples of 4");
  hipStream_t st = (hipStream_t)stream;
  if (mode == 0) {
    RLX_REQUIRE(aux, RLX_EINVAL, "rlx_dbg_gemm_f32: mode 0 needs bias");
    return launch_gemm_fwd(ctx, A, B, aux, C, M, N, K, act, st, 0, nullptr);
  }
  if (mode == 1) {
    const int ntn = div_up(K, G_BN);
    ProfScope prof(ctx, PK_GEMM_DX, 2.0 * (double)M * N * K, st, gemm_bytes(M, K, N, act >= 0 ? 1 : 0));
    RLX_GEMM_DX_LAUNCH(act >= 0 ? act : 0, act >= 0 ? 1 : 0, dim3(div_up(M, G_BM) * ntn), st, A, B, C, M, N, K, K, ntn, (const float*)nullptr);
    RLX_LAUNCH_CHECK();
    return RLX_OK;
  }
  if (mode == 2 || mode == 5) {
    const int ntk = div_up(K, G_BM), ntn = div_up(N, G_BN);
    int S = 1;
    const int64_t Mc = choose_mc(M, ntk * ntn, ctx->num_cus, &S);
    float* pW = (float*)scratch(ctx, SL_PARTIAL, ((size_t)S * K * N + (size_t)S * N) * sizeof(float));
    if (!pW) return RLX_ENOMEM;
    float* pB = pW + (size_t)S * K * N;
    if (mode == 5) {
      const int rcw = bx_launch_dw(ctx, A, B, pW, pB, M, K, K, N, Mc, S, ntk, ntn, st);
      if (rcw) return rcw;
    } else {
      ProfScope prof(ctx, PK_GEMM_DW, 2.0 * (double)M * N * K, st, gemm_bytes(K, N, M));
      RLX_PLAUNCH(k_gemm_dw, dim3(S * ntk * ntn), dim3(G_THREADS), 0, st, A, B, pW, pB, M, K, K, N, Mc, ntk, ntn);
    }
    RLX_LAUNCH_CHECK();
    ReduceTable tab;
    tab.n = 0;
    tab.seg[tab.n++] = ReduceSeg{pW, C, (int64_t)K * N, (int64_t)K * N, S, 0, 1.f, 0.f, 0};
    if (aux) tab.seg[tab.n++] = ReduceSeg{pB, aux, (int64_t)N, (int64_t)N, S, 0, 1.f, 0.f, 0};
    int total = 0;
    for (int i = 0; i < tab.n; ++i) {
      ReduceSeg& g = tab.seg[i];
      g.vec = (g.len % 4 == 0 && g.stride % 4 == 0 && (reinterpret_cast<uintptr_t>(g.src) & 15) == 0 && g.len >= 256) ? 1 : 0;
      if (g.vec && g.S >= 128) g.vec = 2;
      g.nblocks = g.vec == 2 ? div_up(g.len, 64) : (g.vec ? div_up(g.len, 256) : div_up(g.len, 16));
      total += g.nblocks;
    }
    hipLaunchKernelGGL(k_reduce_segments, dim3(total), dim3(256), 0, st, tab, (float*)nullptr);
    RLX_LAUNCH_CHECK();
    return RLX_OK;
  }
  if (mode == 3 || mode == 4) {
    rlx_mlp_desc d{};
    MlpLayout L{};
    d.n_hidden = 2;
    L.n_hidden = 2;
    LayerOff& o = L.layer[1];
    o.W = 0;
    o.in = K;
    o.out = N;
    const bool was = ctx->gemm_bx;
    ctx->gemm_bx = true;
    int rc = bx_prepare_mlp(ctx, d, L, B, mode == 4, st);
    if (!rc) {
      if (mode == 3) {
        RLX_REQUIRE(aux, RLX_EINVAL, "rlx_dbg_gemm_f32: mode 3 needs bias");
        const void* img = bx_lookup(ctx, B, 0, K, N);
        rc = img ? bx_launch_fwd(ctx, A, img, aux, C, M, N, K, act, st, 0, nullptr) : RLX_EUNSUP;
      } else {
        const void* img = bx_lookup(ctx, B, 1, N, K);
        rc = img ? bx_launch_dx(ctx, A, img, C, M, N, K, K, act >= 0 ? act : 0, act >= 0 ? 1 : 0, st) : RLX_EUNSUP;
      }
    }
    bx_release(ctx);
    ctx->gemm_bx = was;
    return rc;
  }
  RLX_REQUIRE(false, RLX_EINVAL, "rlx_dbg_gemm_f32: mode must be 0 .. 5");
}

extern "C" int rlx_dbg_l1_f32(rlx_ctx* ctx, int bwd, const float* X, const float* W, const float* b, const float* g,
                              const float* be, float* H, float* ln_partials, int64_t M, int O, int Hd, int act, int ln,
                              int grid, void* stream) {
  RLX_REQUIRE(ctx && X && W && b && H && M > 0 && O >= 1 && O <= 32 && Hd % 64 == 0 && Hd <= 512 && grid > 0,
              RLX_EINVAL, "rlx_dbg_l1_f32: bad args");
  if (bwd) return launch_l1<true>(X, W, b, g, be, H, ln_partials, M, O, Hd, act, ln, grid, (hipStream_t)stream);
  return launch_l1<false>(X, W, b, g, be, H, nullptr, M, O, Hd, act, ln, grid, (hipStream_t)stream);
}

extern "C" int rlx_mlp_fwd_f32(rlx_ctx* ctx, const rlx_mlp_desc* desc, const float* params, const float* x, float* out,
                               int64_t n, void* stream) {
  RLX_REQUIRE(ctx && desc && params && x && out && n >= 0, RLX_EINVAL, "rlx_mlp_fwd_f32: bad args");
  if (n == 0) return RLX_OK;
  int rc = mlp_check_desc(*desc);
  if (rc) return rc;
  const MlpLayout L = make_layout(*desc);
  hipStream_t st = (hipStream_t)stream;
  int maxh = 0;
  for (int l = 0; l < desc->n_hidden; ++l) maxh = desc->hidden[l] > maxh ? desc->hidden[l] : maxh;
  float* bufA = (float*)scratch(ctx, SL_FWD_A, (size_t)n * maxh * sizeof(float));
  float* bufB = (float*)scratch(ctx, SL_FWD_B, (size_t)n * maxh * sizeof(float));
  if (!bufA || !bufB) return RLX_ENOMEM;
  float* acts[4] = {bufA, bufB, bufA, bufB};
  int ldx = 0;
  if (desc->in_dim > 32 && desc->in_dim % 4 != 0) {
    ldx = (desc->in_dim + 3) & ~3;
    float* xp = (float*)scratch(ctx, SL_STAGE, (size_t)n * ldx * sizeof(float));
    if (!xp) return RLX_ENOMEM;
    RLX_HIP_TRY(hipMemcpy2DAsync(xp, (size_t)ldx * sizeof(float), x, (size_t)desc->in_dim * sizeof(float),
                                 (size_t)desc->in_dim * sizeof(float), (size_t)n, hipMemcpyDeviceToDevice, st));
    x = xp;
  }
  const bool own_images = n >= 4096 && ctx->gemm_bx && ctx->bx_n[0] == 0 && ctx->bx_n[1] == 0;
  struct BxOwn { rlx_ctx* c; bool on; ~BxOwn() { if (on) bx_release_all(c); } } bx_own{ctx, own_images};
  if (own_images) {
    const BxNetSpec net = {desc, params, false, desc->in_dim > 32};
    rc = bx_prepare_nets(ctx, &net, 1, st);
    if (rc) return rc;
  }
  {
    const void *w1x = nullptr, *w2x = nullptr;
    if (fwd2h_supported(ctx, *desc, L, params, n, ldx, &w1x, &w2x))
      return launch_fwd2h(ctx, *desc, L, params, w1x, w2x, x, ldx, nullptr, nullptr, out, n, st);
    const void* wx[3];
    if (fwd3h_supported(ctx, *desc, L, params, n, ldx, wx))
      return launch_fwd3h(ctx, *desc, L, params, wx, x, ldx, nullptr, nullptr, nullptr, nullptr, out, n, st);
  }
  rc = mlp_trunk_fwd(ctx, *desc, L, params, x, acts, n, st, ldx);
  if (rc) return rc;
  return launch_head_fwd(acts[desc->n_hidden - 1], params + L.head.W, params + L.head.b, out, n, L.head.in,
                         L.head.out, st);
}
```

rl-x_amd/csrc/ppo.hip:

```cpp
#include "ppo_internal.h"
#include "gemm_bx.h"
#include "dist.h"

namespace rlx {

constexpr float LOG_2PI = 1.8378770664093453f;
constexpr float HALF_LOG_2PIE = 1.4189385332046727f;
constexpr int HEAD_ROWS = 64;

__global__ __launch_bounds__(256) void k_gather(const float* __restrict__ states, const float* __restrict__ actions,
                                                const float* __restrict__ logp, const float* __restrict__ returns,
                                                const float* __restrict__ adv, const int32_t* __restrict__ idx,
                                                float* __restrict__ mb_x, float* __restrict__ mb_a,
                                                float* __restrict__ aux, const int32_t* __restrict__ valid_rows,
                                                int64_t mb, int O, int A, const float* __restrict__ cstates,
                                                float* __restrict__ mb_xc, int Oc) {
  const int64_t nv = valid_rows ? (int64_t)*valid_rows : mb;
  const int64_t nx = mb * O, na = mb * A, nxc = cstates ? mb * Oc : 0;
  const int64_t total = nx + na + mb + nxc;
  for (int64_t e = (int64_t)blockIdx.x * 256 + threadIdx.x; e < total; e += (int64_t)gridDim.x * 256) {
    if (e >= nx + na + mb) {
      const int64_t f = e - nx - na - mb;
      const int64_t r = f / Oc;
      const int d = (int)(f - r * Oc);
// ... 1216 lines not shown
  const int both = (p && c) ? 1 : 0, which = p ? 0 : 1;
  const float gs = bx_grad_scale(mb_global);
  const float inv_mb = 1.0f / (float)mb_global;
  const size_t lds = 2 * X_OPER + (size_t)HEAD_ROWS * TL_TS * sizeof(float);
  const double nets = both ? 2.0 : 1.0;
  ProfScope prof(s.valid_rows ? nullptr : ctx, PK_TAIL, nets * 4.0 * (double)mb * N2 * TL_K3, st,
                 nets * 4.0 * ((double)mb * (2 * N2 + TL_K3) + 2.0 * N2 * TL_K3), mb, TL_K3, N2, 1);
  if (tail_rows(ctx, N2, act, mb) == T32_ROWS) {
    constexpr int HPL = T32_ROWS * (2 * 256 + 16), DPL = T32_ROWS * (2 * TL_K3 + 16);
    constexpr int TREG = (T32_ROWS * TL_TS * 4 > 2 * DPL) ? T32_ROWS * TL_TS * 4 : 2 * DPL;
    const size_t lds32 = 2 * HPL + TREG + ((size_t)TL_K3 * 8 + 2 * T32_ROWS * 8 + 16 + 2 * TL_K3 * 8) * sizeof(float);
    static AttrOnce attr32;
    if (!attr32.done()) {
      RLX_HIP_TRY(hipFuncSetAttribute(reinterpret_cast<const void*>(k_tail32_bx<RLX_ACT_ELU, 256>),
                                      hipFuncAttributeMaxDynamicSharedMemorySize, 160 * 1024));
      attr32.mark();
    }
    RLX_PLAUNCH((k_tail32_bx<RLX_ACT_ELU, 256>), dim3((unsigned)(mb / T32_ROWS), both ? 2 : 1), dim3(256), lds32, st, tp, tc, s.mb_a,
                s.aux, s.stats, metrics, mb, inv_mb, hp.clip_range, hp.entropy_coef, hp.critic_coef, s.valid_rows, gs, both, which);
    RLX_LAUNCH_CHECK();
    return RLX_OK;
  }
#define RLX_TAIL_LAUNCH(ACTV)                                                                                        \
  {                                                                                                                  \
    static AttrOnce attr_set;                                                                                          \
    if (!attr_set.done()) {                                                                                                 \
      RLX_HIP_TRY(hipFuncSetAttribute(reinterpret_cast<const void*>(k_tail_bx<ACTV>),                                \
                                      hipFuncAttributeMaxDynamicSharedMemorySize, 160 * 1024));                      \
      attr_set.mark();                                                                                                 \
    }                                                                                                                \
    RLX_PLAUNCH((k_tail_bx<ACTV>), dim3((unsigned)(mb / HEAD_ROWS), both ? 2 : 1), dim3(256), lds, st, tp, tc, s.mb_a, s.aux,   \
                s.stats, metrics, mb, N2, inv_mb, hp.clip_range, hp.entropy_coef, hp.critic_coef, s.valid_rows, gs, both,      \
                which);                                                                                              \
  }
  if (act == RLX_ACT_ELU) RLX_TAIL_LAUNCH(RLX_ACT_ELU)
  else if (act == RLX_ACT_TANH) RLX_TAIL_LAUNCH(RLX_ACT_TANH)
  else RLX_TAIL_LAUNCH(RLX_ACT_RELU)
#undef RLX_TAIL_LAUNCH
  RLX_LAUNCH_CHECK();
  return RLX_OK;
}

template <bool POLICY>
static int launch_head_loss(float* H, const float* W, const float* b, const float* logstd, const MbScratch& s, float* metrics,
                            int64_t mb, int K, int A, int PS, float inv_mb, const rlx_ppo_hparams& hp, int act, hipStream_t st,
                            rlx_ctx* prof_ctx = nullptr) {
  const int nb = div_up(mb, HEAD_ROWS);
  ProfScope prof(s.valid_rows ? nullptr : prof_ctx, PK_HEAD_LOSS, 0.0, st,
                 4.0 * ((double)mb * (2 * K + A + 3) + (double)nb * PS + (double)K * A), mb, K, A, PROF_ENGINE_HBM);
  if (POLICY && hp.discrete_actions) {
    RLX_REQUIRE(A >= 2 && A <= 8, RLX_EUNSUP, "ppo: the Categorical head supports 2..8 actions");
    const size_t ldsd = ((size_t)HEAD_ROWS * (K + 1) + (size_t)K * A + 2 * (size_t)HEAD_ROWS * A + 2 * A) * sizeof(float);
    RLX_REQUIRE(ldsd <= 160 * 1024, RLX_EUNSUP, "ppo head: last hidden layer too wide for the LDS-staged head kernel");
    hipLaunchKernelGGL((k_head_loss<POLICY, true>), dim3(nb), dim3(256), ldsd, st, H, W, b, logstd, s.mb_a, s.aux, s.stats,
                       s.head_part, metrics, mb, K, A, PS, inv_mb, hp.clip_range, hp.entropy_coef, hp.critic_coef, act,
                       s.valid_rows);
    RLX_LAUNCH_CHECK();
    return RLX_OK;
  }
  if (A <= 8 && (K == 64 || K == 128 || K == 256)) {
    const int NP = 256 / K > 0 ? 256 / K : 1;
    const size_t lds = ((size_t)K * 8 + 2 * HEAD_ROWS * 8 + (size_t)HEAD_ROWS * (K + 1) + (size_t)NP * K * 8 + 16) * sizeof(float);
#define RLX_HL_FAST(KQV)                                                                                        \
  {                                                                                                             \
    static AttrOnce attr_set;                                                                                     \
    if (!attr_set.done()) {                                                                                            \
      RLX_HIP_TRY(hipFuncSetAttribute(reinterpret_cast<const void*>(k_head_loss_fast<POLICY, KQV>),              \
                                      hipFuncAttributeMaxDynamicSharedMemorySize, 160 * 1024));                 \
      attr_set.mark();                                                                                            \
    }                                                                                                           \
    RLX_PLAUNCH((k_head_loss_fast<POLICY, KQV>), dim3(nb), dim3(256), lds, st, H, W, b, logstd, s.mb_a, s.aux,          \
                s.stats, s.head_part, metrics, mb, A, PS, inv_mb, hp.clip_range, hp.entropy_coef, hp.critic_coef,        \
                act, s.valid_rows);                                                                             \
  }
    if (K == 64) RLX_HL_FAST(16)
    else if (K == 128) RLX_HL_FAST(32)
    else RLX_HL_FAST(64)
#undef RLX_HL_FAST
    RLX_LAUNCH_CHECK();
    return RLX_OK;
  }
  const size_t lds = ((size_t)HEAD_ROWS * (K + 1) + (size_t)K * A + 2 * (size_t)HEAD_ROWS * A + 2 * A) * sizeof(float);
  RLX_REQUIRE(lds <= 160 * 1024, RLX_EUNSUP, "ppo head: last hidden layer too wide for the LDS-staged head kernel");
  hipLaunchKernelGGL(k_head_loss<POLICY>, dim3(nb), dim3(256), lds, st, H, W, b, logstd, s.mb_a, s.aux, s.stats, s.head_part,
                     metrics, mb, K, A, PS, inv_mb, hp.clip_range, hp.entropy_coef, hp.critic_coef, act, s.valid_rows);
  RLX_LAUNCH_CHECK();
  return RLX_OK;
}

template <bool POLICY>
static int net_fwd_bwd(rlx_ctx* ctx, const rlx_mlp_desc& d, const float* params, float* grads, float* metrics,
                       const MbScratch& s, int64_t mb, int mb_global, const rlx_ppo_hparams& hp, float* sumsq,
                       int* n_sumsq, hipStream_t st, hipEvent_t ev_after_fwd = nullptr) {
  const MlpLayout L = make_layout(d);
  const bool kept = ctx->bx_keep[ctx->bank] && ctx->bx_n[ctx->bank] > 0 && d.n_hidden >= 2 &&
                    ctx->bx_img[ctx->bank][0].W == params + L.layer[1].W;
  int rc = (mb >= 4096 && !kept) ? bx_prepare_mlp(ctx, d, L, params, true, st) : RLX_OK;
  if (rc) return rc;
  struct BxScope { rlx_ctx* c; ~BxScope() { if (!c->bx_keep[c->bank]) bx_release(c); } } bx_scope{ctx};
  const float* x_in = (!POLICY && s.mb_xc) ? s.mb_xc : s.mb_x;
  const int K = L.head.in, A = L.head.out;
  const int PS = K * A + 2 * A + 8;
  int nb = div_up(mb, HEAD_ROWS);
  const float inv_mb = 1.0f / (float)mb_global;
  const bool discrete = POLICY && hp.discrete_actions != 0;
  const void *w3f = nullptr, *w3t = nullptr;
  float* dz2 = nullptr;
  if (tail_shape_ok(ctx, d, mb, hp)) {
    const LayerOff& o3 = L.layer[2];
    w3f = bx_lookup(ctx, params + o3.W, 0, o3.in, o3.out);
    w3t = bx_lookup(ctx, params + o3.W, 1, o3.out, o3.in);
    if (w3f && w3t) dz2 = (float*)scratch(ctx, SL_DACT_0, (size_t)mb * o3.in * sizeof(float));
  }
  const bool tail = dz2 != nullptr;
  if (tail) nb = (int)(mb / tail_rows(ctx, L.layer[2].in, d.act, mb));
  XmaxScope xscope(ctx, ctx->xmax_slot[(!POLICY && s.mb_xc) ? 1 : 0]);
  struct L12Scope { rlx_ctx* c; ~L12Scope() { c->l12_stats = nullptr; c->l12_ran = false; } } l12scope{ctx};
  ctx->l12_ran = false;
  ctx->l12_stats = nullptr;
  if (ctx->dw_recompute && tail && ctx->l12_fused && l12fwd_supported(d) && dw_merge_ok(ctx, d, L, mb) && d.hidden[0] == 512 &&
      d.act == RLX_ACT_ELU && grads) {
    ctx->l12_stats = (float*)scratch(ctx, SL_LN_P, (size_t)2 * mb * sizeof(float));
    if (!ctx->l12_stats) return RLX_ENOMEM;
  }
  rc = mlp_trunk_fwd(ctx, d, L, params, x_in, s.acts, mb, st, 0, false, nullptr, tail ? d.n_hidden - 1 : -1);
  if (rc) return rc;
  if (ev_after_fwd) RLX_HIP_TRY(hipEventRecord(ev_after_fwd, st));
  if (tail) {
    const LayerOff& o3 = L.layer[2];
    const TailNet tn{s.acts[1], (const u32x4*)w3f, (const u32x4*)w3t, params + o3.b, params + L.head.W, params + L.head.b,
                     POLICY ? params + L.logstd : nullptr, s.acts[2], dz2, s.head_part, A, PS};
    rc = launch_tail(ctx, POLICY ? &tn : nullptr, POLICY ? nullptr : &tn, s, metrics, mb, o3.in, mb_global, hp, d.act, st);
  } else {
    rc = launch_head_loss<POLICY>(s.acts[d.n_hidden - 1], params + L.head.W, params + L.head.b,
                                  (POLICY && !discrete) ? params + L.logstd : nullptr, s, metrics, mb, K, A, PS, inv_mb, hp,
                                  d.act, st, ctx);
  }
  if (rc) return rc;
  ReduceSeg extra[8];
  int ne = 0;
  extra[ne++] = ReduceSeg{s.head_part, grads + L.head.W, (int64_t)K * A, (int64_t)PS, nb, 0, 1.f, 0.f, 1};
  extra[ne++] = ReduceSeg{s.head_part + K * A, grads + L.head.b, (int64_t)A, (int64_t)PS, nb, 0, 1.f, 0.f, 1};
  if (POLICY) {
    if (!discrete)
      extra[ne++] = ReduceSeg{s.head_part + K * A + A, grads + L.logstd, (int64_t)A, (int64_t)PS, nb, 0, 1.f, 0.f, 1};
    else
      extra[ne++] = ReduceSeg{s.head_part + K * A + 2 * A + 3, metrics + 2, 1, (int64_t)PS, nb, 0, inv_mb, 0.f, 0};
    extra[ne++] = ReduceSeg{s.head_part + K * A + 2 * A + 0, metrics + 0, 1, (int64_t)PS, nb, 0, inv_mb, 0.f, 0};
    extra[ne++] = ReduceSeg{s.head_part + K * A + 2 * A + 1, metrics + 3, 1, (int64_t)PS, nb, 0, inv_mb, 0.f, 0};
    extra[ne++] = ReduceSeg{s.head_part + K * A + 2 * A + 2, metrics + 4, 1, (int64_t)PS, nb, 0, inv_mb, 0.f, 0};
  } else {
    extra[ne++] = ReduceSeg{s.head_part + K * A + 2 * A + 0, metrics + 1, 1, (int64_t)PS, nb, 0, inv_mb, 0.f, 0};
  }
  GradScaleScope gscope(ctx, bx_grad_scale(mb_global));
  TrunkOpts topt;
  topt.dz_below_last = dz2;
  return mlp_trunk_bwd(ctx, d, L, params, x_in, s.acts, grads, mb, extra, ne, sumsq, n_sumsq, st, tail ? &topt : nullptr);
}

struct XmaxCall {
  rlx_ctx* c;
  explicit XmaxCall(rlx_ctx* ctx) : c(ctx) {}
  int set(const float* states, int64_t n, const float* cstates, int64_t nc, hipStream_t st) {
    if (!c->gemm_bx) return RLX_OK;
    int rc = x_max_update(c, states, n, 0, st, &c->xmax_slot[0]);
    if (!rc && cstates) rc = x_max_update(c, cstates, nc, 1, st, &c->xmax_slot[1]);
    return rc;
  }
  ~XmaxCall() { c->xmax_slot[0] = c->xmax_slot[1] = nullptr; }
};

static bool twin_shapes_ok(const rlx_ctx* ctx, const rlx_mlp_desc& pd, const rlx_mlp_desc& cd, const rlx_ppo_hparams& hp,
                           int64_t mb) {
  if (ctx->ppo_twin == 0 || (ctx->ppo_twin < 0 && mb > 16384)) return false;
  if (ctx->ppo_twin < 0 && mb < 6144 && ctx->gather_records && ctx->gather_group_rows > mb && !hp.critic_states &&
      pd.in_dim + (hp.discrete_actions ? 1 : pd.out_dim) + 3 <= 128)
    return false;
  if (ctx->ppo_twin < 0 && ctx->comm && ctx->world > 1) return false;
  if (!ctx->gemm_bx || !ctx->adam_emit || ctx->disable_l1fused || !ctx->l1fwd_mfma || hp.discrete_actions || hp.critic_states)
    return false;
  if (pd.n_hidden != cd.n_hidden || pd.n_hidden < 2 || pd.in_dim != cd.in_dim || pd.act != cd.act ||
      pd.ln_first != cd.ln_first || !pd.has_logstd || cd.out_dim != 1 || pd.out_dim > 8)
    return false;
  for (int l = 0; l < pd.n_hidden; ++l)
    if (pd.hidden[l] != cd.hidden[l] || (l >= 1 && pd.hidden[l] % 4 != 0)) return false;
  const int K = pd.hidden[pd.n_hidden - 1];
  if (!(K == 64 || K == 128 || K == 256)) return false;
  if (mb < 4096 || !l1fwd_mfma_supported(pd) || !l1fused_supported(pd)) return false;
  for (int l = 1; l < pd.n_hidden; ++l)
    if (!bx_dw_usable(ctx, mb, pd.hidden[l - 1], pd.hidden[l - 1], pd.hidden[l])) return false;
  return true;
}

struct TwinImages {
  const void* f[4][2];
  const void* t[4][2];
  const void* w2x[2];
  const void* w1x[2];
};

static int twin_images(rlx_ctx* ctx, const rlx_mlp_desc& pd, const MlpLayout& LP, const float* pparams, const rlx_mlp_desc& cd,
                       const MlpLayout& LC, const float* cparams, hipStream_t st, TwinImages* im, bool* ok) {
  *ok = false;
  const rlx_mlp_desc* dd[2] = {&pd, &cd};
  const MlpLayout* LL[2] = {&LP, &LC};
  const float* pp[2] = {pparams, cparams};
  const int bank0 = ctx->bank;
  for (int q = 0; q < 2; ++q) {
    ctx->bank = q;
    const bool kept = ctx->bx_keep[q] && ctx->bx_n[q] > 0 && ctx->bx_img[q][0].W == pp[q] + LL[q]->layer[1].W;
    if (!kept) {
      const int rc = bx_prepare_mlp(ctx, *dd[q], *LL[q], pp[q], true, st);
      if (rc) { ctx->bank = bank0; return rc; }
    }
    bool all = l1fused_bx_images(ctx, *LL[q], pp[q], &im->w2x[q], &im->w1x[q]);
    for (int l = 1; l < dd[q]->n_hidden && all; ++l) {
      const LayerOff& o = LL[q]->layer[l];
      im->f[l][q] = bx_lookup(ctx, pp[q] + o.W, 0, o.in, o.out);
      im->t[l][q] = bx_lookup(ctx, pp[q] + o.W, 1, o.out, o.in);
      all = im->f[l][q] && im->t[l][q];
    }
    if (!all) { ctx->bank = bank0; return RLX_OK; }
  }
  ctx->bank = bank0;
  *ok = true;
  return RLX_OK;
}

static int twin_fwd_bwd(rlx_ctx* ctx, const rlx_mlp_desc& pd, const MlpLayout& LP, const float* pparams, float* pg,
                        const rlx_mlp_desc& cd, const MlpLayout& LC, const float* cparams, float* cg, const TwinImages& im,
                        float* met, const MbScratch& sp, const MbScratch& sc, int64_t mb, int mb_global,
                        const rlx_ppo_hparams& hp, float* sq, int* npb, int* ncb, hipStream_t st) {
  const int nh = pd.n_hidden, last = nh - 1;
  Twin t;
  XmaxScope xscope(ctx, ctx->xmax_slot[0]);
  int rc;
  int l_first = 1;
  float* stats2[2] = {nullptr, nullptr};
  const bool l12 = ctx->l12_fused && l12fwd_supported(pd) && im.w1x[0] && im.w1x[1];
  if (l12 && ctx->dw_recompute && ctx->dw_merge && nh == 3 && tail_shape_ok(ctx, pd, mb, hp) && pd.hidden[0] == 512 &&
      pd.act == RLX_ACT_ELU) {
    const int b0 = ctx->bank;
    for (int q = 0; q < 2; ++q) {
      ctx->bank = q;
      stats2[q] = (float*)scratch(ctx, SL_LN_P, (size_t)2 * mb * sizeof(float));
    }
    ctx->bank = b0;
    if (!stats2[0] || !stats2[1]) return RLX_ENOMEM;
  }
  if (l12) {
    L12Twin tw{cparams, sc.acts[0], sc.acts[1], im.w1x[1], im.f[1][1]};
    tw.stats = stats2[1];
    rc = launch_l12fwd(ctx, pd, LP, pparams, sp.mb_x, sp.acts[0], sp.acts[1], im.w1x[0], im.f[1][0], mb, st, &tw, stats2[0]);
    l_first = 2;
  } else {
    rc = launch_l1fwd_mfma(pd, LP, pparams, sp.mb_x, sp.acts[0], mb, ctx->num_cus, st, nullptr, ctx, cparams, sc.acts[0]);
  }
  if (rc) return rc;
  float* dz2[2] = {nullptr, nullptr};
  const float* dzb[4][2];
  for (int l = 0; l < 4; ++l) { dzb[l][0] = sp.acts[l]; dzb[l][1] = sc.acts[l]; }
  if (tail_shape_ok(ctx, pd, mb, hp)) {
    const int bank0_ = ctx->bank;
    for (int q = 0; q < 2; ++q) {
      ctx->bank = q;
      dz2[q] = (float*)scratch(ctx, SL_DACT_0, (size_t)mb * LP.layer[2].in * sizeof(float));
    }
    ctx->bank = bank0_;
    if (!dz2[0] || !dz2[1]) return RLX_ENOMEM;
    dzb[1][0] = dz2[0];
    dzb[1][1] = dz2[1];
  }
  const bool tail = dz2[0] != nullptr;
  for (int l = l_first; l < (tail ? nh - 1 : nh); ++l) {
    const LayerOff& o = LP.layer[l];
    t.p[0] = sc.acts[l - 1]; t.p[1] = im.f[l][1]; t.p[2] = cparams + LC.layer[l].b; t.p[3] = sc.acts[l];
    rc = bx_launch_fwd(ctx, sp.acts[l - 1], im.f[l][0], pparams + o.b, sp.acts[l], mb, o.out, o.in, pd.act, st, 0, nullptr, &t);
    if (rc) return rc;
  }
  const int K = LP.head.in, A = LP.head.out;
  const int PSp = K * A + 2 * A + 8, PSc = K + 2 + 8;
  const int nb = tail ? (int)(mb / tail_rows(ctx, LP.layer[2].in, pd.act, mb)) : div_up(mb, HEAD_ROWS);
  const float inv_mb = 1.0f / (float)mb_global;
  if (tail) {
    const LayerOff& o3 = LP.layer[2];
    const TailNet tp{sp.acts[1], (const u32x4*)im.f[2][0], (const u32x4*)im.t[2][0], pparams + o3.b, pparams + LP.head.W,
                     pparams + LP.head.b, pparams + LP.logstd, sp.acts[2], dz2[0], sp.head_part, A, PSp};
    const TailNet tc{sc.acts[1], (const u32x4*)im.f[2][1], (const u32x4*)im.t[2][1], cparams + LC.layer[2].b, cparams + LC.head.W,
                     cparams + LC.head.b, nullptr, sc.acts[2], dz2[1], sc.head_part, 1, PSc};
    rc = launch_tail(ctx, &tp, &tc, sp, met, mb, o3.in, mb_global, hp, pd.act, st);
    if (rc) return rc;
  } else {
    const HeadNet hn_p{sp.acts[last], pparams + LP.head.W, pparams + LP.head.b, pparams + LP.logstd, sp.head_part, A, PSp};
    const HeadNet hn_c{sc.acts[last], cparams + LC.head.W, cparams + LC.head.b, nullptr, sc.head_part, 1, PSc};
    rc = launch_head_loss_pc(hn_p, hn_c, sp, met, mb, K, inv_mb, hp, pd.act, st);
    if (rc) return rc;
  }
  GradScaleScope gscope(ctx, bx_grad_scale(mb_global));
  const int cus = ctx->num_cus / 2 > 0 ? ctx->num_cus / 2 : 1;
  int S[4] = {0, 0, 0, 0};
  int64_t Mc[4] = {0, 0, 0, 0};
  size_t per_net = 0;
  for (int l = 1; l < nh; ++l) {
    const LayerOff& o = LP.layer[l];
    Mc[l] = choose_mc(mb, div_up(o.in, G_BM) * div_up(o.out, G_BN), cus, &S[l]);
  }
// ... 964 lines not shown
```

Before: 7.828 million.

## Fold early gradient-reduction segments into the merged dW GEMM launch

Splits the per-layer gradient reduction into early and late parts. Segments that are already final (layer-1 fused output, the last layer's dW/db, and the head extras) are reduced by extra workgroups appended to the final merged dW kernel grid, so they overlap with GEMM work. Only the remaining segments are handled by a smaller trailing reduce launch. The shared reduction body is moved into a header so both kernels can use it. This adds grid and LDS complexity to the dW kernel and is disabled when distributed training is active.

```diff
diff --git a/rl-x_amd/csrc/common.h b/rl-x_amd/csrc/common.h
--- a/rl-x_amd/csrc/common.h
+++ b/rl-x_amd/csrc/common.h
@@ -35,6 +35,9 @@
   RLX_HIP_TRY(hipGetLastError())
 
 constexpr int WAVE = 64;
+#ifndef RLX_EARLY_REDUCE_DEFAULT
+#define RLX_EARLY_REDUCE_DEFAULT 1
+#endif
 
 struct Scratch {
   void* ptr = nullptr;
@@ -107,6 +110,7 @@
   float* l12_stats = nullptr;
   bool l12_ran = false;
   bool dw_merge = true;
+  int early_reduce = RLX_EARLY_REDUCE_DEFAULT;
   void* dbg_stamps = nullptr;
   bool fwd2h = true;
   int gather_group_rows = 524288;
diff --git a/rl-x_amd/csrc/core.hip b/rl-x_amd/csrc/core.hip
--- a/rl-x_amd/csrc/core.hip
+++ b/rl-x_amd/csrc/core.hip
@@ -224,6 +224,7 @@
   if (std::string(name) == "lf_idle_cus") { ctx->lf_idle_cus = value < 0 ? 0 : value; return RLX_OK; }
   if (std::string(name) == "dw_recompute") { ctx->dw_recompute = value != 0; return RLX_OK; }
   if (std::string(name) == "dw_merge") { ctx->dw_merge = value != 0; return RLX_OK; }
+  if (std::string(name) == "early_reduce") { ctx->early_reduce = value < 0 ? 0 : (value > 2 ? 2 : value); return RLX_OK; }
   if (std::string(name) == "fwd2h") { ctx->fwd2h = value != 0; return RLX_OK; }
   if (std::string(name) == "l12_fused") { ctx->l12_fused = value != 0; return RLX_OK; }
   if (std::string(name) == "gather_group_rows") { ctx->gather_group_rows = value; return RLX_OK; }
diff --git a/rl-x_amd/csrc/gemm_bx.hip b/rl-x_amd/csrc/gemm_bx.hip
--- a/rl-x_amd/csrc/gemm_bx.hip
+++ b/rl-x_amd/csrc/gemm_bx.hip
@@ -3,6 +3,7 @@
 #define RLX_WS_MIN_WAVES 2
 #endif
 #include "mlp.h"
+#include "reduce_body.h"
 
 namespace rlx {
 
@@ -204,13 +205,17 @@
   BxDwRecompute rc;
 };
 template <bool TWIN, bool REC = false>
-__global__ __launch_bounds__(XW_THREADS, 2) void k_gemm_dw_bx(DwArgs a, DwArgs b, int nb0, float sg, float so) {
+__global__ __launch_bounds__(XW_THREADS, 2) void k_gemm_dw_bx(DwArgs a, DwArgs b, int nb0, int nbg, float sg, float so, ReduceEarly early) {
   extern __shared__ __attribute__((aligned(16))) char lds[];
+  if ((int)blockIdx.x >= nbg) {
+    reduce_early_workgroup(early, ((int)blockIdx.x - nbg) * (int)gridDim.y + (int)blockIdx.y, lds);
+    return;
+  }
   int bid = blockIdx.x, nblk = nb0;
   if (bid >= nb0) {
     a = b;
     bid -= nb0;
-    nblk = gridDim.x - nb0;
+    nblk = nbg - nb0;
   }
   const float* __restrict__ Hp = a.Hp;
   const float* __restrict__ dZ = a.dZ;
@@ -820,15 +825,16 @@
   const DwArgs a = dw_args(Hp, dZ, pW, pB, M, Kd, ldh, N, Mc, ntk, ntn, tw);
   const int nb = S * ntk * ntn;
   if (tw) {
-    RLX_PLAUNCH(k_gemm_dw_bx<true>, dim3(nb, 2), dim3(XW_THREADS), 4 * X_OPER, st, a, a, nb, gs, X_AINV / gs);
+    RLX_PLAUNCH(k_gemm_dw_bx<true>, dim3(nb, 2), dim3(XW_THREADS), 4 * X_OPER, st, a, a, nb, nb, gs, X_AINV / gs, ReduceEarly{});
   } else {
-    RLX_PLAUNCH(k_gemm_dw_bx<false>, dim3(nb), dim3(XW_THREADS), 4 * X_OPER, st, a, a, nb, gs, X_AINV / gs);
+    RLX_PLAUNCH(k_gemm_dw_bx<false>, dim3(nb), dim3(XW_THREADS), 4 * X_OPER, st, a, a, nb, nb, gs, X_AINV / gs, ReduceEarly{});
   }
   RLX_LAUNCH_CHECK();
   return RLX_OK;
 }
 
-int bx_launch_dw2(rlx_ctx* ctx, const BxDwJob& j0, const BxDwJob& j1, int64_t M, hipStream_t st, const Twin* tw0, const Twin* tw1) {
+int bx_launch_dw2(rlx_ctx* ctx, const BxDwJob& j0, const BxDwJob& j1, int64_t M, hipStream_t st, const Twin* tw0, const Twin* tw1,
+                  const ReduceEarly* early) {
   int rc = dw_attr();
   if (rc) return rc;
   RLX_REQUIRE((tw0 == nullptr) == (tw1 == nullptr), RLX_EINVAL, "bx_launch_dw2: both jobs or neither must have a twin");
@@ -845,13 +851,17 @@
   }
   const int nb0 = j0.S * j0.ntk * j0.ntn, nb1 = j1.S * j1.ntk * j1.ntn;
   const size_t lds = 4 * X_OPER + (j0.rc ? DW_REC_LDS : 0);
+  const ReduceEarly et = early ? *early : ReduceEarly{};
+  const int ny = tw0 ? 2 : 1;
+  const int nbe = div_up(et.nblocks, 2 * ny);
+  const int nbg = nb0 + nb1;
   if (j0.rc) {
-    if (tw0) { RLX_PLAUNCH((k_gemm_dw_bx<true, true>), dim3(nb0 + nb1, 2), dim3(XW_THREADS), lds, st, a, b, nb0, gs, X_AINV / gs); }
-    else { RLX_PLAUNCH((k_gemm_dw_bx<false, true>), dim3(nb0 + nb1), dim3(XW_THREADS), lds, st, a, b, nb0, gs, X_AINV / gs); }
+    if (tw0) { RLX_PLAUNCH((k_gemm_dw_bx<true, true>), dim3(nbg + nbe, 2), dim3(XW_THREADS), lds, st, a, b, nb0, nbg, gs, X_AINV / gs, et); }
+    else { RLX_PLAUNCH((k_gemm_dw_bx<false, true>), dim3(nbg + nbe), dim3(XW_THREADS), lds, st, a, b, nb0, nbg, gs, X_AINV / gs, et); }
   } else if (tw0) {
-    RLX_PLAUNCH(k_gemm_dw_bx<true>, dim3(nb0 + nb1, 2), dim3(XW_THREADS), lds, st, a, b, nb0, gs, X_AINV / gs);
+    RLX_PLAUNCH(k_gemm_dw_bx<true>, dim3(nbg + nbe, 2), dim3(XW_THREADS), lds, st, a, b, nb0, nbg, gs, X_AINV / gs, et);
   } else {
-    RLX_PLAUNCH(k_gemm_dw_bx<false>, dim3(nb0 + nb1), dim3(XW_THREADS), lds, st, a, b, nb0, gs, X_AINV / gs);
+    RLX_PLAUNCH(k_gemm_dw_bx<false>, dim3(nbg + nbe), dim3(XW_THREADS), lds, st, a, b, nb0, nbg, gs, X_AINV / gs, et);
   }
   RLX_LAUNCH_CHECK();
   return RLX_OK;
diff --git a/rl-x_amd/csrc/mlp.h b/rl-x_amd/csrc/mlp.h
--- a/rl-x_amd/csrc/mlp.h
+++ b/rl-x_amd/csrc/mlp.h
@@ -17,10 +17,20 @@
   float bias;
   int in_norm;
   int vec;
+  int blk0;
+  int early;
 };
 struct ReduceTable {
   int n;
   ReduceSeg seg[REDUCE_MAX_SEGS];
+};
+enum ReducePart { REDUCE_ALL = 0, REDUCE_EARLY = 1, REDUCE_LATE = 2 };
+constexpr int REDUCE_MAX_EARLY = 12;
+struct ReduceEarly {
+  int n = 0;
+  int nblocks = 0;
+  float* sumsq = nullptr;
+  ReduceSeg seg[REDUCE_MAX_EARLY];
 };
 
 struct TrunkOpts {
@@ -42,6 +52,10 @@
 int64_t choose_mc(int64_t M, int tiles, int num_cus, int* S_out);
 int64_t choose_mc_fit(int64_t M, int tiles, int num_cus, int* S_out);
 int launch_reduce_segments(ReduceTable& tab, float* sumsq_partials, int* n_blocks_out, hipStream_t st, rlx_ctx* prof_ctx = nullptr);
+int reduce_plan(ReduceTable& tab, int* total_out, int cap = REDUCE_MAX_BLOCKS);
+bool reduce_early_table(const ReduceTable& tab, float* sumsq_partials, ReduceEarly* out);
+int launch_reduce_part(const ReduceTable& tab, ReducePart part, float* sumsq_partials, hipStream_t st, rlx_ctx* prof_ctx = nullptr);
+int early_reduce_mode(const rlx_ctx* ctx);
 int mlp_trunk_fwd(rlx_ctx* ctx, const rlx_mlp_desc& d, const MlpLayout& L, const float* params, const float* x,
                   float* const* acts, int64_t M, hipStream_t st, int ldx = 0, bool gemm_l0 = false,
                   const int32_t* m_dev = nullptr, int n_layers = -1);
@@ -181,7 +195,7 @@
   const BxDwRecompute* rc = nullptr;
 };
 int bx_launch_dw2(rlx_ctx* ctx, const BxDwJob& j0, const BxDwJob& j1, int64_t M, hipStream_t st, const Twin* tw0 = nullptr,
-                  const Twin* tw1 = nullptr);
+                  const Twin* tw1 = nullptr, const ReduceEarly* early = nullptr);
 
 
 struct BxEmitLayer {
diff --git a/rl-x_amd/csrc/mlp.hip b/rl-x_amd/csrc/mlp.hip
--- a/rl-x_amd/csrc/mlp.hip
+++ b/rl-x_amd/csrc/mlp.hip
@@ -1,4 +1,6 @@
 #include "mlp.h"
+#include "reduce_body.h"
+#include "dist.h"
 #include "ln_kernels.h"
 
 namespace rlx {
@@ -720,148 +722,18 @@
   } while (0)
 
 __global__ __launch_bounds__(256) void k_reduce_segments(ReduceTable tab, float* __restrict__ sumsq_partials) {
-  __shared__ float4 s_acc[4][64];
+  __shared__ float4 s_acc[256];
   __shared__ float s_buf[4];
   int seg = 0;
-  int blk = blockIdx.x;
-  while (seg < tab.n - 1 && blk >= tab.seg[seg].nblocks) {
-    blk -= tab.seg[seg].nblocks;
-    ++seg;
-  }
+  const int blk = reduce_locate(tab.seg, tab.n, blockIdx.x, &seg);
   const ReduceSeg sg = tab.seg[seg];
-  float sq = 0.f;
-  if (sg.vec == 2) {
-    const int x = threadIdx.x & 15, y = threadIdx.x >> 4;
-    const int64_t i = (int64_t)blk * 64 + 4 * x;
-    float4 a = make_float4(0.f, 0.f, 0.f, 0.f);
-    if (i < sg.len) {
-      const float* p = sg.src + i;
-      int sidx = y;
-      for (; sidx + 240 < sg.S; sidx += 256) {
-        float4 v[16];
-#pragma unroll
-        for (int q = 0; q < 16; ++q) v[q] = *reinterpret_cast<const float4*>(p + (int64_t)(sidx + 16 * q) * sg.stride);
-#pragma unroll
-        for (int q = 0; q < 16; q += 4) {
-          a.x += (v[q].x + v[q + 1].x) + (v[q + 2].x + v[q + 3].x);
-          a.y += (v[q].y + v[q + 1].y) + (v[q + 2].y + v[q + 3].y);
-          a.z += (v[q].z + v[q + 1].z) + (v[q + 2].z + v[q + 3].z);
-          a.w += (v[q].w + v[q + 1].w) + (v[q + 2].w + v[q + 3].w);
-        }
-      }
-      for (; sidx < sg.S; sidx += 64) {
-        float4 r[4];
-#pragma unroll
-        for (int q = 0; q < 4; ++q) {
-          const int si = sidx + 16 * q;
-          r[q] = *reinterpret_cast<const float4*>(p + (int64_t)(si < sg.S ? si : sg.S - 1) * sg.stride);
-        }
-#pragma unroll
-        for (int q = 0; q < 4; ++q)
-          if (sidx + 16 * q < sg.S) { a.x += r[q].x; a.y += r[q].y; a.z += r[q].z; a.w += r[q].w; }
-      }
-    }
-    float4* sred4 = &s_acc[0][0];
-    sred4[y * 16 + x] = a;
-    __syncthreads();
-    if (y == 0 && i < sg.len) {
-      float4 v = a;
-#pragma unroll
-      for (int q = 1; q < 16; ++q) {
-        const float4 b = sred4[q * 16 + x];
-        v.x += b.x; v.y += b.y; v.z += b.z; v.w += b.w;
-      }
-      v.x = v.x * sg.scale + sg.bias;
-      v.y = v.y * sg.scale + sg.bias;
-      v.z = v.z * sg.scale + sg.bias;
-      v.w = v.w * sg.scale + sg.bias;
-      sg.dst[i] = v.x; sg.dst[i + 1] = v.y; sg.dst[i + 2] = v.z; sg.dst[i + 3] = v.w;
-      if (sg.in_norm) sq = v.x * v.x + v.y * v.y + v.z * v.z + v.w * v.w;
-    }
-  } else if (sg.vec) {
-    const int x = threadIdx.x & 63, y = threadIdx.x >> 6;
-    const int64_t i = (int64_t)blk * 256 + 4 * x;
-    float4 a = make_float4(0.f, 0.f, 0.f, 0.f);
-    if (i < sg.len) {
-      const float* p = sg.src + i;
-      int sidx = y;
-      for (; sidx + 60 < sg.S; sidx += 64) {
-        float4 v[16];
-#pragma unroll
-        for (int q = 0; q < 16; ++q) v[q] = *reinterpret_cast<const float4*>(p + (int64_t)(sidx + 4 * q) * sg.stride);
-#pragma unroll
-        for (int q = 0; q < 16; q += 4) {
-          a.x += (v[q].x + v[q + 1].x) + (v[q + 2].x + v[q + 3].x);
-          a.y += (v[q].y + v[q + 1].y) + (v[q + 2].y + v[q + 3].y);
-          a.z += (v[q].z + v[q + 1].z) + (v[q + 2].z + v[q + 3].z);
-          a.w += (v[q].w + v[q + 1].w) + (v[q + 2].w + v[q + 3].w);
-        }
-      }
-      for (; sidx + 12 < sg.S; sidx += 16) {
-        const float4 v0 = *reinterpret_cast<const float4*>(p + (int64_t)sidx * sg.stride);
-        const float4 v1 = *reinterpret_cast<const float4*>(p + (int64_t)(sidx + 4) * sg.stride);
-        const float4 v2 = *reinterpret_cast<const float4*>(p + (int64_t)(sidx + 8) * sg.stride);
-        const float4 v3 = *reinterpret_cast<const float4*>(p + (int64_t)(sidx + 12) * sg.stride);
-        a.x += (v0.x + v1.x) + (v2.x + v3.x);
-        a.y += (v0.y + v1.y) + (v2.y + v3.y);
-        a.z += (v0.z + v1.z) + (v2.z + v3.z);
-        a.w += (v0.w + v1.w) + (v2.w + v3.w);
-      }
-      {
-        float4 r[3];
-#pragma unroll
-        for (int q = 0; q < 3; ++q) {
-          const int si = sidx + 4 * q;
-          r[q] = *reinterpret_cast<const float4*>(p + (int64_t)(si < sg.S ? si : sg.S - 1) * sg.stride);
-        }
-#pragma unroll
-        for (int q = 0; q < 3; ++q) {
-          if (sidx + 4 * q < sg.S) { a.x += r[q].x; a.y += r[q].y; a.z += r[q].z; a.w += r[q].w; }
-        }
-      }
-    }
-    s_acc[y][x] = a;
-    __syncthreads();
-    if (y == 0 && i < sg.len) {
-      const float4 b1 = s_acc[1][x], b2 = s_acc[2][x], b3 = s_acc[3][x];
-      float4 v;
-      v.x = ((a.x + b1.x) + (b2.x + b3.x)) * sg.scale + sg.bias;
-      v.y = ((a.y + b1.y) + (b2.y + b3.y)) * sg.scale + sg.bias;
-      v.z = ((a.z + b1.z) + (b2.z + b3.z)) * sg.scale + sg.bias;
-      v.w = ((a.w + b1.w) + (b2.w + b3.w)) * sg.scale + sg.bias;
-      sg.dst[i] = v.x; sg.dst[i + 1] = v.y; sg.dst[i + 2] = v.z; sg.dst[i + 3] = v.w;
-      if (sg.in_norm) sq = v.x * v.x + v.y * v.y + v.z * v.z + v.w * v.w;
-    }
-  } else {
-    const int x = threadIdx.x & 15, y = threadIdx.x >> 4;
-    const int64_t i = (int64_t)blk * 16 + x;
-    float a = 0.f;
-    if (i < sg.len) {
-      const float* p = sg.src + i;
-      int sidx = y;
-      for (; sidx + 48 < sg.S; sidx += 64) {
-        const float v0 = p[(int64_t)sidx * sg.stride], v1 = p[(int64_t)(sidx + 16) * sg.stride];
-        const float v2 = p[(int64_t)(sidx + 32) * sg.stride], v3 = p[(int64_t)(sidx + 48) * sg.stride];
-        a += (v0 + v1) + (v2 + v3);
-      }
-      for (; sidx < sg.S; sidx += 16) a += p[(int64_t)sidx * sg.stride];
-    }
-    float* sred = reinterpret_cast<float*>(&s_acc[0][0]);
-    sred[y * 16 + x] = a;
-    __syncthreads();
-    if (y == 0 && i < sg.len) {
-      float v = 0.f;
-#pragma unroll
-      for (int q = 0; q < 16; ++q) v += sred[q * 16 + x];
-      v = v * sg.scale + sg.bias;
-      sg.dst[i] = v;
-      if (sg.in_norm) sq = v * v;
-    }
-  }
+  const float4 a = reduce_block_load(sg, blk, threadIdx.x, s_acc);
+  __syncthreads();
+  float sq = reduce_block_store(sg, blk, threadIdx.x, s_acc, a);
   sq = wave_sum(sq);
   if ((threadIdx.x & 63) == 0) s_buf[threadIdx.x >> 6] = sq;
   __syncthreads();
-  if (threadIdx.x == 0 && sumsq_partials) sumsq_partials[blockIdx.x] = s_buf[0] + s_buf[1] + s_buf[2] + s_buf[3];
+  if (threadIdx.x == 0 && sumsq_partials) sumsq_partials[sg.blk0 + blk] = s_buf[0] + s_buf[1] + s_buf[2] + s_buf[3];
 }
 
 static int check_desc(const rlx_mlp_desc& d) {
@@ -1134,7 +1006,11 @@
     const int rcf = launch_l1fused(ctx, d, L, params, x, dz[1], lf_arena, lf_grid, grads, M, &tab, st);
     if (rcf) return rcf;
     l1_done = true;
-  }
+    for (int i = 0; i < tab.n; ++i) tab.seg[i].early = 1;
+  }
+  const int early_mode = (dw_merge && l1_done) ? early_reduce_mode(ctx) : 0;
+  bool early_done = false;
+  int early_total = 0;
   for (int l = d.n_hidden - 1; l >= 1; --l) {
     const LayerOff& o = L.layer[l];
     float* pW = cur; cur += (size_t)S_l[l] * o.in * o.out;
@@ -1150,8 +1026,27 @@
           rcd.be = params + o0.be; rcd.stats = ctx->l12_stats; rcd.xmax = ctx->l1_xmax; rcd.O = o0.in; rcd.NT1 = o0.out / 32;
           job.rc = &rcd;
         }
-        const int rcw = bx_launch_dw2(ctx, job, dw_job3, M, st);
+        ReduceEarly etab;
+        if (early_mode) {
+          RLX_REQUIRE(tab.n + 2 + n_extra <= REDUCE_MAX_SEGS, RLX_EUNSUP, "mlp bwd: too many reduction segments");
+          ReduceTable plan = tab;
+          plan.seg[plan.n++] = ReduceSeg{pW, grads + o.W, (int64_t)o.in * o.out, (int64_t)o.in * o.out, S_l[l], 0, 1.f, 0.f, 1};
+          plan.seg[plan.n++] = ReduceSeg{pB, grads + o.b, (int64_t)o.out, (int64_t)o.out, S_l[l], 0, 1.f, 0.f, 1};
+          for (int e = 0; e < n_extra; ++e) plan.seg[plan.n++] = extra[e];
+          reduce_plan(plan, &early_total);
+          if (early_total <= REDUCE_MAX_BLOCKS && reduce_early_table(plan, sumsq_partials, &etab)) {
+            tab = plan;
+            early_done = true;
+            if (early_mode == 2) {
+              const int rce = launch_reduce_part(tab, REDUCE_EARLY, sumsq_partials, st, ctx);
+              if (rce) return rce;
+            }
+          }
+        }
+        const int rcw = bx_launch_dw2(ctx, job, dw_job3, M, st, nullptr, nullptr,
+                                      early_done && early_mode == 1 ? &etab : nullptr);
         if (rcw) return rcw;
+        if (early_done) break;
       }
       tab.seg[tab.n++] = ReduceSeg{pW, grads + o.W, (int64_t)o.in * o.out, (int64_t)o.in * o.out, S_l[l], 0, 1.f, 0.f, 1};
       tab.seg[tab.n++] = ReduceSeg{pB, grads + o.b, (int64_t)o.out, (int64_t)o.out, S_l[l], 0, 1.f, 0.f, 1};
@@ -1260,30 +1155,74 @@
     if (n_sumsq_blocks) *n_sumsq_blocks = 0;
     return RLX_OK;
   }
+  if (early_done) {
+    if (n_sumsq_blocks) *n_sumsq_blocks = early_total;
+    return launch_reduce_part(tab, REDUCE_LATE, sumsq_partials, st, ctx);
+  }
   for (int e = 0; e < n_extra; ++e) tab.seg[tab.n++] = extra[e];
   return launch_reduce_segments(tab, sumsq_partials, n_sumsq_blocks, st, ctx);
 }
 
-int launch_reduce_segments(ReduceTable& tab, float* sumsq_partials, int* n_blocks_out, hipStream_t st, rlx_ctx* prof_ctx) {
-  int total_blocks = 0;
+int reduce_plan(ReduceTable& tab, int* total_out, int cap) {
+  int total = 0;
+  for (int pass = 0; pass < 2; ++pass) {
+    total = 0;
+    for (int i = 0; i < tab.n; ++i) {
+      ReduceSeg& g = tab.seg[i];
+      g.vec = (g.len % 4 == 0 && g.stride % 4 == 0 && (reinterpret_cast<uintptr_t>(g.src) & 15) == 0 && g.len >= 256) ? 1 : 0;
+      if (pass == 0 && g.vec && g.S >= 128) g.vec = 2;
+      g.nblocks = g.vec == 2 ? div_up(g.len, 64) : (g.vec ? div_up(g.len, 256) : div_up(g.len, 16));
+      g.blk0 = total;
+      total += g.nblocks;
+    }
+    if (cap <= 0 || total <= cap) break;
+  }
+  if (total_out) *total_out = total;
+  return RLX_OK;
+}
+
+bool reduce_early_table(const ReduceTable& tab, float* sumsq_partials, ReduceEarly* out) {
+  out->n = 0;
+  out->nblocks = 0;
+  out->sumsq = sumsq_partials;
+  for (int i = 0; i < tab.n; ++i) {
+    if (!tab.seg[i].early) continue;
+    if (out->n == REDUCE_MAX_EARLY) return false;
+    out->seg[out->n++] = tab.seg[i];
+    out->nblocks += tab.seg[i].nblocks;
+  }
+  return out->n > 0;
+}
+
+int early_reduce_mode(const rlx_ctx* ctx) { return (ctx->gemm_bx && !dist_active(ctx)) ? ctx->early_reduce : 0; }
+
+int launch_reduce_part(const ReduceTable& tab, ReducePart part, float* sumsq_partials, hipStream_t st, rlx_ctx* prof_ctx) {
+  ReduceTable sub;
+  sub.n = 0;
+  int blocks = 0;
   double bytes = 0.0;
   int64_t outputs = 0;
   for (int i = 0; i < tab.n; ++i) {
-    bytes += 4.0 * (double)tab.seg[i].len * (tab.seg[i].S + 1);
-    outputs += tab.seg[i].len;
-  }
-  ProfScope prof(prof_ctx, PK_REDUCE, 0.0, st, bytes, outputs, tab.n, 0, PROF_ENGINE_HBM);
-  for (int i = 0; i < tab.n; ++i) {
-    ReduceSeg& g = tab.seg[i];
-    g.vec = (g.len % 4 == 0 && g.stride % 4 == 0 && (reinterpret_cast<uintptr_t>(g.src) & 15) == 0 && g.len >= 256)
-                ? 1 : 0;
-    if (g.vec && g.S >= 128) g.vec = 2;
-    g.nblocks = g.vec == 2 ? div_up(g.len, 64) : (g.vec ? div_up(g.len, 256) : div_up(g.len, 16));
-    total_blocks += g.nblocks;
-  }
+    const ReduceSeg& g = tab.seg[i];
+    if ((part == REDUCE_EARLY && !g.early) || (part == REDUCE_LATE && g.early)) continue;
+    sub.seg[sub.n++] = g;
+    blocks += g.nblocks;
+    bytes += 4.0 * (double)g.len * (g.S + 1);
+    outputs += g.len;
+  }
+  if (sub.n == 0) return RLX_OK;
+  ProfScope prof(prof_ctx, PK_REDUCE, 0.0, st, bytes, outputs, sub.n, 0, PROF_ENGINE_HBM);
+  RLX_PLAUNCH(k_reduce_segments, dim3(blocks), dim3(256), 0, st, sub, sumsq_partials);
+  RLX_LAUNCH_CHECK();
+  return RLX_OK;
+}
+
+int launch_reduce_segments(ReduceTable& tab, float* sumsq_partials, int* n_blocks_out, hipStream_t st, rlx_ctx* prof_ctx) {
+  int total_blocks = 0;
+  reduce_plan(tab, &total_blocks);
   RLX_REQUIRE(total_blocks <= REDUCE_MAX_BLOCKS, RLX_EUNSUP, "mlp bwd: too many reduction blocks");
-  RLX_PLAUNCH(k_reduce_segments, dim3(total_blocks), dim3(256), 0, st, tab, sumsq_partials);
-  RLX_LAUNCH_CHECK();
+  const int rc = launch_reduce_part(tab, REDUCE_ALL, sumsq_partials, st, prof_ctx);
+  if (rc) return rc;
   if (n_blocks_out) *n_blocks_out = total_blocks;
   return RLX_OK;
 }
@@ -1334,13 +1273,7 @@
 
 static int reduce_launch(rlx_ctx* ctx, ReduceTable& tab, float* sumsq, int* nsq, hipStream_t st) {
   int total = 0;
-  for (int i = 0; i < tab.n; ++i) {
-    ReduceSeg& g = tab.seg[i];
-    g.vec = (g.len % 4 == 0 && g.stride % 4 == 0 && (reinterpret_cast<uintptr_t>(g.src) & 15) == 0 && g.len >= 256) ? 1 : 0;
-    if (g.vec && g.S >= 128) g.vec = 2;
-    g.nblocks = g.vec == 2 ? div_up(g.len, 64) : (g.vec ? div_up(g.len, 256) : div_up(g.len, 16));
-    total += g.nblocks;
-  }
+  reduce_plan(tab, &total, nsq ? REDUCE_MAX_BLOCKS - *nsq : 0);
   RLX_REQUIRE(!nsq || *nsq + total <= REDUCE_MAX_BLOCKS, RLX_EUNSUP, "stage reduce: norm partial array exhausted");
   hipLaunchKernelGGL(k_reduce_segments, dim3(total), dim3(256), 0, st, tab, sumsq ? sumsq + (nsq ? *nsq : 0) : nullptr);
   RLX_LAUNCH_CHECK();
@@ -1508,13 +1441,7 @@
     tab.seg[tab.n++] = ReduceSeg{pW, C, (int64_t)K * N, (int64_t)K * N, S, 0, 1.f, 0.f, 0};
     if (aux) tab.seg[tab.n++] = ReduceSeg{pB, aux, (int64_t)N, (int64_t)N, S, 0, 1.f, 0.f, 0};
     int total = 0;
-    for (int i = 0; i < tab.n; ++i) {
-      ReduceSeg& g = tab.seg[i];
-      g.vec = (g.len % 4 == 0 && g.stride % 4 == 0 && (reinterpret_cast<uintptr_t>(g.src) & 15) == 0 && g.len >= 256) ? 1 : 0;
-      if (g.vec && g.S >= 128) g.vec = 2;
-      g.nblocks = g.vec == 2 ? div_up(g.len, 64) : (g.vec ? div_up(g.len, 256) : div_up(g.len, 16));
-      total += g.nblocks;
-    }
+    reduce_plan(tab, &total, 0);
     hipLaunchKernelGGL(k_reduce_segments, dim3(total), dim3(256), 0, st, tab, (float*)nullptr);
     RLX_LAUNCH_CHECK();
     return RLX_OK;
diff --git a/rl-x_amd/csrc/ppo.hip b/rl-x_amd/csrc/ppo.hip
--- a/rl-x_amd/csrc/ppo.hip
+++ b/rl-x_amd/csrc/ppo.hip
@@ -1392,6 +1392,7 @@
   } else {
     extra[ne++] = ReduceSeg{s.head_part + K * A + 2 * A + 0, metrics + 1, 1, (int64_t)PS, nb, 0, inv_mb, 0.f, 0};
   }
+  for (int e = 0; e < ne; ++e) extra[e].early = 1;
   GradScaleScope gscope(ctx, bx_grad_scale(mb_global));
   TrunkOpts topt;
   topt.dz_below_last = dz2;
diff --git a/rl-x_amd/csrc/reduce_body.h b/rl-x_amd/csrc/reduce_body.h
--- /dev/null
+++ b/rl-x_amd/csrc/reduce_body.h
@@ -0,0 +1,182 @@
+#pragma once
+#include "common.h"
+#include "mlp.h"
+
+namespace rlx {
+
+__device__ __forceinline__ int reduce_locate(const ReduceSeg* __restrict__ segs, int n, int rel, int* seg_out) {
+  int seg = 0;
+  int blk = rel;
+  while (seg < n - 1 && blk >= segs[seg].nblocks) {
+    blk -= segs[seg].nblocks;
+    ++seg;
+  }
+  *seg_out = seg;
+  return blk;
+}
+
+__device__ __forceinline__ float4 reduce_block_load(const ReduceSeg& sg, int blk, int tid, float4* __restrict__ s_acc) {
+  float4 a = make_float4(0.f, 0.f, 0.f, 0.f);
+  if (sg.vec == 2) {
+    const int x = tid & 15, y = tid >> 4;
+    const int64_t i = (int64_t)blk * 64 + 4 * x;
+    if (i < sg.len) {
+      const float* p = sg.src + i;
+      int sidx = y;
+      for (; sidx + 240 < sg.S; sidx += 256) {
+        float4 v[16];
+#pragma unroll
+        for (int q = 0; q < 16; ++q) v[q] = *reinterpret_cast<const float4*>(p + (int64_t)(sidx + 16 * q) * sg.stride);
+#pragma unroll
+        for (int q = 0; q < 16; q += 4) {
+          a.x += (v[q].x + v[q + 1].x) + (v[q + 2].x + v[q + 3].x);
+          a.y += (v[q].y + v[q + 1].y) + (v[q + 2].y + v[q + 3].y);
+          a.z += (v[q].z + v[q + 1].z) + (v[q + 2].z + v[q + 3].z);
+          a.w += (v[q].w + v[q + 1].w) + (v[q + 2].w + v[q + 3].w);
+        }
+      }
+      for (; sidx < sg.S; sidx += 64) {
+        float4 r[4];
+#pragma unroll
+        for (int q = 0; q < 4; ++q) {
+          const int si = sidx + 16 * q;
+          r[q] = *reinterpret_cast<const float4*>(p + (int64_t)(si < sg.S ? si : sg.S - 1) * sg.stride);
+        }
+#pragma unroll
+        for (int q = 0; q < 4; ++q)
+          if (sidx + 16 * q < sg.S) { a.x += r[q].x; a.y += r[q].y; a.z += r[q].z; a.w += r[q].w; }
+      }
+    }
+    s_acc[y * 16 + x] = a;
+  } else if (sg.vec) {
+    const int x = tid & 63, y = tid >> 6;
+    const int64_t i = (int64_t)blk * 256 + 4 * x;
+    if (i < sg.len) {
+      const float* p = sg.src + i;
+      int sidx = y;
+      for (; sidx + 60 < sg.S; sidx += 64) {
+        float4 v[16];
+#pragma unroll
+        for (int q = 0; q < 16; ++q) v[q] = *reinterpret_cast<const float4*>(p + (int64_t)(sidx + 4 * q) * sg.stride);
+#pragma unroll
+        for (int q = 0; q < 16; q += 4) {
+          a.x += (v[q].x + v[q + 1].x) + (v[q + 2].x + v[q + 3].x);
+          a.y += (v[q].y + v[q + 1].y) + (v[q + 2].y + v[q + 3].y);
+          a.z += (v[q].z + v[q + 1].z) + (v[q + 2].z + v[q + 3].z);
+          a.w += (v[q].w + v[q + 1].w) + (v[q + 2].w + v[q + 3].w);
+        }
+      }
+      for (; sidx + 12 < sg.S; sidx += 16) {
+        const float4 v0 = *reinterpret_cast<const float4*>(p + (int64_t)sidx * sg.stride);
+        const float4 v1 = *reinterpret_cast<const float4*>(p + (int64_t)(sidx + 4) * sg.stride);
+        const float4 v2 = *reinterpret_cast<const float4*>(p + (int64_t)(sidx + 8) * sg.stride);
+        const float4 v3 = *reinterpret_cast<const float4*>(p + (int64_t)(sidx + 12) * sg.stride);
+        a.x += (v0.x + v1.x) + (v2.x + v3.x);
+        a.y += (v0.y + v1.y) + (v2.y + v3.y);
+        a.z += (v0.z + v1.z) + (v2.z + v3.z);
+        a.w += (v0.w + v1.w) + (v2.w + v3.w);
+      }
+      {
+        float4 r[3];
+#pragma unroll
+        for (int q = 0; q < 3; ++q) {
+          const int si = sidx + 4 * q;
+          r[q] = *reinterpret_cast<const float4*>(p + (int64_t)(si < sg.S ? si : sg.S - 1) * sg.stride);
+        }
+#pragma unroll
+        for (int q = 0; q < 3; ++q) {
+          if (sidx + 4 * q < sg.S) { a.x += r[q].x; a.y += r[q].y; a.z += r[q].z; a.w += r[q].w; }
+        }
+      }
+    }
+    s_acc[y * 64 + x] = a;
+  } else {
+    const int x = tid & 15, y = tid >> 4;
+    const int64_t i = (int64_t)blk * 16 + x;
+    float s = 0.f;
+    if (i < sg.len) {
+      const float* p = sg.src + i;
+      int sidx = y;
+      for (; sidx + 48 < sg.S; sidx += 64) {
+        const float v0 = p[(int64_t)sidx * sg.stride], v1 = p[(int64_t)(sidx + 16) * sg.stride];
+        const float v2 = p[(int64_t)(sidx + 32) * sg.stride], v3 = p[(int64_t)(sidx + 48) * sg.stride];
+        s += (v0 + v1) + (v2 + v3);
+      }
+      for (; sidx < sg.S; sidx += 16) s += p[(int64_t)sidx * sg.stride];
+    }
+    reinterpret_cast<float*>(s_acc)[y * 16 + x] = s;
+    a.x = s;
+  }
+  return a;
+}
+
+__device__ __forceinline__ float reduce_block_store(const ReduceSeg& sg, int blk, int tid, const float4* __restrict__ s_acc,
+                                                    const float4 a) {
+  float sq = 0.f;
+  if (sg.vec == 2) {
+    const int x = tid & 15, y = tid >> 4;
+    const int64_t i = (int64_t)blk * 64 + 4 * x;
+    if (y == 0 && i < sg.len) {
+      float4 v = a;
+#pragma unroll
+      for (int q = 1; q < 16; ++q) {
+        const float4 b = s_acc[q * 16 + x];
+        v.x += b.x; v.y += b.y; v.z += b.z; v.w += b.w;
+      }
+      v.x = v.x * sg.scale + sg.bias;
+      v.y = v.y * sg.scale + sg.bias;
+      v.z = v.z * sg.scale + sg.bias;
+      v.w = v.w * sg.scale + sg.bias;
+      sg.dst[i] = v.x; sg.dst[i + 1] = v.y; sg.dst[i + 2] = v.z; sg.dst[i + 3] = v.w;
+      if (sg.in_norm) sq = v.x * v.x + v.y * v.y + v.z * v.z + v.w * v.w;
+    }
+  } else if (sg.vec) {
+    const int x = tid & 63, y = tid >> 6;
+    const int64_t i = (int64_t)blk * 256 + 4 * x;
+    if (y == 0 && i < sg.len) {
+      const float4 b1 = s_acc[64 + x], b2 = s_acc[128 + x], b3 = s_acc[192 + x];
+      float4 v;
+      v.x = ((a.x + b1.x) + (b2.x + b3.x)) * sg.scale + sg.bias;
+      v.y = ((a.y + b1.y) + (b2.y + b3.y)) * sg.scale + sg.bias;
+      v.z = ((a.z + b1.z) + (b2.z + b3.z)) * sg.scale + sg.bias;
+      v.w = ((a.w + b1.w) + (b2.w + b3.w)) * sg.scale + sg.bias;
+      sg.dst[i] = v.x; sg.dst[i + 1] = v.y; sg.dst[i + 2] = v.z; sg.dst[i + 3] = v.w;
+      if (sg.in_norm) sq = v.x * v.x + v.y * v.y + v.z * v.z + v.w * v.w;
+    }
+  } else {
+    const int x = tid & 15, y = tid >> 4;
+    const int64_t i = (int64_t)blk * 16 + x;
+    if (y == 0 && i < sg.len) {
+      const float* sred = reinterpret_cast<const float*>(s_acc);
+      float v = 0.f;
+#pragma unroll
+      for (int q = 0; q < 16; ++q) v += sred[q * 16 + x];
+      v = v * sg.scale + sg.bias;
+      sg.dst[i] = v;
+      if (sg.in_norm) sq = v * v;
+    }
+  }
+  return sq;
+}
+
+__device__ __forceinline__ void reduce_early_workgroup(const ReduceEarly& E, int wg, char* smem) {
+  const int half = threadIdx.x >> 8, tid = threadIdx.x & 255;
+  float4* s_acc = reinterpret_cast<float4*>(smem) + half * 256;
+  float* s_buf = reinterpret_cast<float*>(smem + 2 * 256 * sizeof(float4)) + half * 4;
+  const int rel = 2 * wg + half;
+  const bool live = rel < E.nblocks;
+  int seg = 0, blk = 0;
+  if (live) blk = reduce_locate(E.seg, E.n, rel, &seg);
+  const ReduceSeg sg = E.seg[seg];
+  float4 a = make_float4(0.f, 0.f, 0.f, 0.f);
+  if (live) a = reduce_block_load(sg, blk, tid, s_acc);
+  __syncthreads();
+  float sq = 0.f;
+  if (live) sq = reduce_block_store(sg, blk, tid, s_acc, a);
+  sq = wave_sum(sq);
+  if ((tid & 63) == 0) s_buf[tid >> 6] = sq;
+  __syncthreads();
+  if (live && tid == 0 && E.sumsq) E.sumsq[sg.blk0 + blk] = s_buf[0] + s_buf[1] + s_buf[2] + s_buf[3];
+}
+
+}
```

Result: no change. 7.821 million (-0.1%).
